# MAPieschl/PointCloudProcessing

Measured on AMD Instinct MI355X. Metric: points/sec PointNet fwd+bwd N=1024 B=32 at 1/2/4/8 MI355X vs CPU ref, higher is better.
Workload: dtype bf16; 1 GPU; PointNet-cls training step (fwd + losses + bwd + grad all-reduce + Adam), N=1024 points, batch 32 per GPU, profile classification_pretrain, 23 classes / 12 parts, random-init weights; global_batch=32, points_per_cloud=1024, parallelism=dp1, launch=hipgraph

## Files before the change

### include/pointnet_hip.h

```cpp
#ifndef POINTNET_HIP_H
#define POINTNET_HIP_H

#include <stddef.h>
#include <stdint.h>

#ifdef __cplusplus
extern "C" {
#endif

#define PN_ABI_VERSION 6

typedef enum {
  PN_OK = 0,
  PN_ERR_INVALID_ARGUMENT = -1,
  PN_ERR_LAUNCH = -2,
  PN_ERR_UNSUPPORTED = -3,
  PN_ERR_WORKSPACE = -4
} pn_status;

#define PN_PREC_BF16 1
#define PN_PREC_BF16X3 3
#define PN_STORE_BF16 0x100
#define PN_IO_KEEP_ACTIVATIONS 1

// ... 183 lines not shown

typedef struct pn_slot_info {
  char name[64];
  int64_t offset;
  int32_t rows, cols, kind, block;
} pn_slot_info;

#define PN_NUM_BLOCKS 15

typedef struct pn_model_io {
  const float* pc;
  int32_t B, N;
  float* params;
  float* grads;
  const uint8_t* trainable;
  int32_t training;
  int32_t zero_grads_in_forward;
  const uint8_t* keep1;
  const uint8_t* keep2;
  const int32_t* labels_cls;
  const int32_t* labels_seg;
  const float* se3;
  float loss_weights[3];
  float pad2_;
  float* out_cls;
  float* out_seg;
  float* out_R;
  float* scalars;
  void* workspace;
  size_t workspace_bytes;
  void** prof_events;
  void* aux_stream;
  int32_t bwd_phase;
  int32_t flags;
  uint64_t dropout_seed;
  uint32_t* dropout_step;
  int32_t sync_rank;
  int32_t pad3_;
  int (*sync_hook)(void* ctx, int op, const void* src, void* dst, int64_t n, int dtype, void* stream);
  void* sync_ctx;
} pn_model_io;

int pn_model_num_slots(const pn_model_desc* d);
int64_t pn_model_param_floats(const pn_model_desc* d);
int pn_model_slot_info(const pn_model_desc* d, int i, pn_slot_info* out);
size_t pn_model_workspace_bytes(const pn_model_desc* d, int B, int N, int training);
int pn_model_ws_lookup(const pn_model_desc* d, int B, int N, int training, const char* name, int64_t* offset, int64_t* bytes);

int pn_model_ws_entry(const pn_model_desc* d, int B, int N, int training, int index, char* name_out, int name_cap,
                      int64_t* offset, int64_t* bytes);

int64_t pn_model_plan_count(int which);
int64_t pn_model_wgrad_fused_count(void);

int pn_model_forward(const pn_model_desc* d, const pn_model_io* io, pn_stream stream);
int pn_model_backward(const pn_model_desc* d, const pn_model_io* io, const float* d_cls, const float* d_seg,
                      const float* d_R, pn_stream stream);

int pn_dropout_masks(uint8_t* keep1, int64_t n1, uint8_t* keep2, int64_t n2, float rate, uint64_t seed, uint32_t* step,
                     pn_stream stream);

int pn_adam_prepare(const int32_t* iterations, float* alpha_scratch, double lr0, double decay_rate, double decay_steps, double beta1,
                    double beta2, pn_stream stream);
int pn_adam_step(float* params, const float* grads, float* m, float* v, int64_t n, int32_t* iterations,
                 float* alpha_scratch, double lr0, double decay_rate, double decay_steps, double beta1, double beta2,
                 double eps, float grad_scale, pn_stream stream);

#ifdef __cplusplus
}
#endif
#endif
```

### pointcloudprocessing_amd/_lib.py

```python
from __future__ import annotations

import ctypes as C
import os
import subprocess

_HERE = os.path.dirname(os.path.abspath(__file__))
LIB_PATH = os.path.join(_HERE, "libpointnet_hip.so")
CSRC = os.path.join(_HERE, "csrc")

PN_PREC_BF16 = 1
PN_PREC_BF16X3 = 3
PN_STORE_BF16 = 0x100
PN_IO_KEEP_ACTIVATIONS = 1
ABI_VERSION = 6
PN_NUM_BLOCKS = 15
PREC = {"bf16": PN_PREC_BF16 | PN_STORE_BF16, "bf16_f32act": PN_PREC_BF16, "bf16x3": PN_PREC_BF16X3}

BLOCK_NAMES = ["input_transform", "mlp_1_1", "mlp_1_2", "feature_transform", "mlp_2_1", "mlp_2_2", "mlp_2_3",
               "mlp_cls_1", "mlp_cls_2", "mlp_cls_3", "mlp_seg_1", "mlp_seg_2", "mlp_seg_3", "mlp_seg_4",
               "mlp_seg_5"]


class PointNetHipError(RuntimeError):
    pass
# ... 70 lines not shown
    "pn_conv_bwd_data_wgrad": (_I, [_OP, _P, _I64, _I, _I, _I, _I, _P, _P, _P, _P, _P, _P, _OP, _I, _I, _P, _I, _P]),
    "pn_slab_reduce": (_I, [_P, _I, _I, _I64, _P, _P]),
    "pn_bn_finalize": (_I, [_P, _I, _I, _I64, _P, _P, _P, _P, _F, _F, _I, _I, _P, _P, _P, _P, _P]),
    "pn_bn_bwd_finalize": (_I, [_P, _I, _I, _I64, _P, _P, _P, _I, _P, _P, _P, _P, _P, _P]),
    "pn_sign": (_I, [_P, _I, _P, _P]),
    "pn_max_finalize": (_I, [_P, _P, _I, _I, _I, _P, _P, _P, _P, _P, _P, _P]),
    "pn_dense_workspace_floats": (C.c_size_t, [_I, _I, _I]),
    "pn_dense_layer": (_I, [_P, _I, _P, _I, _I, _I, _I, _I, _P, _P, _P, _P, _P, _P, _P, _F, _F, _I, _I, _P, _F, _P, _P, _P, _P, _P]),
    "pn_dense_bwd_step": (_I, [_P, _I, _P, _I, _I, _I, _I, _P, _P, _P, _P, _P]),
    "pn_dense_wgrad_batch": (_I, [_P, _I, _P]),
    "pn_dense_bwd": (_I, [_P, _P, _P, _I, _I, _I, _I, _P, _P, _P, _P, _I, _I, _P, _F, _P, _P, _P, _P, _P, _P]),
    "pn_softmax_xent": (_I, [_P, _I, _I, _P, _F, _P, _P, _P, _P, _P]),
    "pn_argmax_rows": (_I, [_P, _I64, _I, _P, _P]),
    "pn_seg_out_part_stride": (_I, []),
    "pn_seg_out_part_rows": (_I, []),
    "pn_seg_out_fwd": (_I, [_OP, _P, _P, _I64, _I, _I, _P, _F, _P, _P, _P, _P]),
    "pn_bmm": (_I, [_P, _P, _I, _I, _I, _P, _I, _P]),
    "pn_dropout_masks": (_I, [_P, _I64, _P, _I64, _F, C.c_uint64, _P, _P]),
    "pn_count_nonfinite": (_I, [_P, _I64, _I, _P, _P]),
    "pn_fps_workspace_bytes": (C.c_size_t, [_I, _I]),
    "pn_fps": (_I, [_P, _I, _I, _I, _I, _P, _P, _P, C.c_size_t, _P]),
    "pn_voxel_workspace_bytes": (C.c_size_t, [_I]),
    "pn_voxel_downsample": (_I, [_P, _P, _I, C.POINTER(C.c_float), C.POINTER(C.c_float), _I, _P, _P, _P, _P, _P,
                                 C.c_size_t, _P]),
    "pn_knn_propagate": (_I, [_P, _P, _I, _I, _I, _I, _P, _I, _P, _P, _P, _P, _P]),
    "pn_icp_workspace_bytes": (C.c_size_t, [_I, _I, _I, _I]),
    "pn_icp_correspond": (_I, [_P, _P, _I, _I, _P, C.POINTER(C.c_int32), _I, _I, _P, _F, _P, _P, _P, _P, C.c_size_t, _P]),
    "pn_icp_solve": (_I, [_P, _I, _P, _P, _P, _P]),
    "pn_semantic_icp": (_I, [_P, _P, _I, _I, _P, C.POINTER(C.c_int32), _I, _I, _P, _I, _F, _D, _D, _P, _P, _P, _P, _P, _P,
                             C.c_size_t, _P]),
    "pn_icp_normals": (_I, [_P, C.POINTER(C.c_int32), _I, _I, _I, _P, _P, _P, _P]),
    "pn_icp_plane_workspace_bytes": (C.c_size_t, [_I, _I, _I, _I]),
    "pn_icp_plane_sums": (_I, [_P, _P, _I, _I, _P, C.POINTER(C.c_int32), _I, _I, _P, _F, _P, _P, _P, _P, _P, _P, C.c_size_t, _P]),
    "pn_icp_plane_solve": (_I, [_P, _I, _P, _P, _P, _P]),
    "pn_semantic_icp_plane": (_I, [_P, _P, _I, _I, _P, C.POINTER(C.c_int32), _I, _I, _P, _I, _F, _D, _D, _P, _P, _P, _P, _P, _P, _P,
                                   C.c_size_t, _P]),
    "pn_icp_mesh_workspace_bytes": (C.c_size_t, [_I, _I, _I, _I]),
    "pn_icp_mesh_correspond": (_I, [_P, _P, _I, _I, _P, C.POINTER(C.c_int32), _I, _I, _P, _F, _I, _P, _P, _P, _P, _P, _P, _P, C.c_size_t,
                                    _P]),
    "pn_semantic_icp_mesh": (_I, [_P, _P, _I, _I, _P, C.POINTER(C.c_int32), _I, _I, _P, _I, _P, _I, _F, _D, _D, _P, _P, _P, _P, _P, _P,
                                  C.c_size_t, _P]),
    "pn_part_moments_workspace_bytes": (C.c_size_t, [_I, _I]),
    "pn_part_moments": (_I, [_P, _P, _I, _I, _I, _P, _P, C.c_size_t, _P]),
    "pn_icp_seed_poses": (_I, [_P, _P, _I, _I, _P, _I, _P, _P]),
    "pn_icp_score_workspace_bytes": (C.c_size_t, [_I, _I, _I]),
    "pn_icp_score_poses": (_I, [_P, _P, _I, _I, _P, C.POINTER(C.c_int32), _I, _I, _P, _I, _I, _F, _P, _P, _P, C.c_size_t, _P]),
    "pn_model_num_slots": (_I, [_DESC]),
    "pn_model_param_floats": (_I64, [_DESC]),
    "pn_model_slot_info": (_I, [_DESC, _I, C.POINTER(pn_slot_info)]),
    "pn_model_workspace_bytes": (C.c_size_t, [_DESC, _I, _I, _I]),
    "pn_model_ws_lookup": (_I, [_DESC, _I, _I, _I, C.c_char_p, C.POINTER(C.c_int64), C.POINTER(C.c_int64)]),
    "pn_model_ws_entry": (_I, [_DESC, _I, _I, _I, _I, C.c_char_p, _I, C.POINTER(C.c_int64), C.POINTER(C.c_int64)]),
    "pn_model_plan_count": (_I64, [_I]),
    "pn_model_wgrad_fused_count": (_I64, []),
    "pn_model_forward": (_I, [_DESC, _IO, _P]),
    "pn_model_backward": (_I, [_DESC, _IO, _P, _P, _P, _P]),
    "pn_adam_prepare": (_I, [_P, _P, _D, _D, _D, _D, _D, _P]),
    "pn_adam_step": (_I, [_P, _P, _P, _P, _I64, _P, _P, _D, _D, _D, _D, _D, _D, _F, _P]),
}

_lib = None


def build(verbose: bool = False) -> str:
    res = subprocess.run(["make", "-C", CSRC, "-j", str(min(8, os.cpu_count() or 1))], capture_output=True, text=True)
    if verbose or res.returncode != 0:
        print(res.stdout[-4000:])
        print(res.stderr[-4000:])
    if res.returncode != 0:
        raise PointNetHipError("building libpointnet_hip.so failed")
    return LIB_PATH


def lib():
    global _lib
    if _lib is None:
        if not os.path.exists(LIB_PATH):
            raise PointNetHipError(
                f"{LIB_PATH} is missing: run `python -c 'import __graft_entry__ as g; g.build()'` "
                f"(or `make -C {CSRC}`).  There is no CPU fallback for the PointNet hot path.")
        import torch
        try:
            l = C.CDLL(LIB_PATH)
        except OSError as e:
            raise PointNetHipError(f"cannot load {LIB_PATH}: {e}") from e
        for name, (res, args) in SIGNATURES.items():
            fn = getattr(l, name)
            fn.restype = res
            fn.argtypes = args
        if l.pn_abi_version() != ABI_VERSION:
            raise PointNetHipError("libpointnet_hip.so ABI version mismatch")
        _lib = l
    return _lib


def check(rc: int, what: str = "") -> None:
    if rc != 0:
        msg = lib().pn_last_error()
        raise PointNetHipError(f"{what} failed ({rc}): {msg.decode() if msg else ''}")


def ptr(t):
    if t is None:
        return None
    return C.c_void_p(t.data_ptr())

# ... 33 lines not shown
```

### pointcloudprocessing_amd/csrc/pn_dense.hip

```cpp
#include "pn_common.h"
#include "pn_dense_wgrad.h"
#include "pn_internal.h"
#include "pn_loss_bodies.h"
#include "pn_maxbwd_bodies.h"

namespace pn {

typedef __attribute__((ext_vector_type(8))) __bf16 bf16x8;
typedef __attribute__((ext_vector_type(16))) float f32x16;

constexpr int DL_COLS = 32;
constexpr int DL_SLICES = 8;
constexpr int DL_KPS = 16;
constexpr int DL_KSTEP = DL_SLICES * DL_KPS;
constexpr int DL_ROWS = 32;
constexpr int DL_MAX_SPLITS = 8;

struct DenseArgs {
  const float* x; int ldx;
  const float* w; int ldw;
  int R, K, C, split_len, nsplit;
  float* partial;
  unsigned* counters;
  const float *bias, *gamma, *beta;
  float *mm, *mv;
  float momentum, eps;
  int bn_mode, act;
  const unsigned char* keep; float keep_scale;
  float *z_out, *a_out, *mean_o, *invstd_o;
  const float *bt_z, *bt_gamma, *bt_beta, *bt_mean, *bt_invstd;
  const unsigned char* bt_keep; float bt_keep_scale;
  int bt_mode, bt_act;
  float *bt_dz, *bt_dgamma, *bt_dbeta, *bt_dbias;
};

static inline int dl_ksplit_env() {
  static const int v = (getenv("PN_DENSE_KSPLIT") && atoi(getenv("PN_DENSE_KSPLIT")) >= 1) ? atoi(getenv("PN_DENSE_KSPLIT")) : 0;
  return v;
}
static inline int dl_nsplit(int K) {
  const int env = dl_ksplit_env();
  const int per_split = env ? env : DL_KSTEP;
  const int s = cdiv(K, per_split);
  return s < 1 ? 1 : (s > DL_MAX_SPLITS ? DL_MAX_SPLITS : s);
}
static inline int dl_split_len(int K) { return cdiv(cdiv(K, dl_nsplit(K)), DL_KSTEP) * DL_KSTEP; }

template <bool TRANS, int DEPTH, bool VEC, bool CARRY = false>
__device__ __forceinline__ bool dense_layer_body(const DenseArgs& a, const unsigned bxi, const int ks, float* zr_out = nullptr) {
  __shared__ __attribute__((aligned(16))) float lds[4 * DL_ROWS * DL_COLS + 16 * 32 + 4];
  float* red = lds;
  float* fin = lds + 4 * DL_ROWS * DL_COLS;
  unsigned* flag = reinterpret_cast<unsigned*>(fin + 16 * 32);
  const int tid = threadIdx.x, c = tid & 31, s = tid >> 5;
  const int j = bxi * DL_COLS + c;
  const int jc = j < a.C ? j : a.C - 1;
  const int kbeg = ks * a.split_len, kend = min(a.K, kbeg + a.split_len);
  const bool single = a.nsplit == 1;
  const bool small = a.R <= DL_ROWS;
  float own[DL_ROWS / DL_SLICES];
  float pf_g = 1.f, pf_b = 0.f, pf_mm = 0.f, pf_mv = 1.f;
  const float pf_bias = a.bias ? a.bias[jc] : 0.f;
  unsigned char pf_kb[DL_ROWS / DL_SLICES] = {1, 1, 1, 1};
  if (a.bn_mode) { pf_g = a.gamma[jc]; pf_b = a.beta[jc]; pf_mm = a.mm[jc]; pf_mv = a.mv[jc]; }
  if (a.keep && a.a_out && a.R <= DL_ROWS) {
#pragma unroll
    for (int i = 0; i < DL_ROWS / DL_SLICES; ++i) pf_kb[i] = a.keep[(long long)min(s + DL_SLICES * i, a.R - 1) * a.C + jc];
  }
  float bt_zz[DL_ROWS / DL_SLICES], bt_mu = 0.f, bt_is = 1.f, bt_g = 1.f, bt_b = 0.f;
  unsigned char bt_kb[DL_ROWS / DL_SLICES] = {1, 1, 1, 1};
  if (TRANS && a.bt_dz) {
#pragma unroll
    for (int i = 0; i < DL_ROWS / DL_SLICES; ++i) bt_zz[i] = a.bt_z[(long long)min(s + DL_SLICES * i, a.R - 1) * a.C + jc];
    if (a.bt_keep) {
#pragma unroll
      for (int i = 0; i < DL_ROWS / DL_SLICES; ++i) bt_kb[i] = a.bt_keep[(long long)min(s + DL_SLICES * i, a.R - 1) * a.C + jc];
    }
    if (a.bt_mode) { bt_mu = a.bt_mean[jc]; bt_is = a.bt_invstd[jc]; bt_g = a.bt_gamma[jc]; bt_b = a.bt_beta[jc]; }
  }

  const int lane = tid & 63, wv = tid >> 6;
  const int lr = lane & 31, lg = lane >> 5;
  const int jw = bxi * DL_COLS + lr;
  const int jwc = jw < a.C ? jw : a.C - 1;
  for (int rc = 0; rc < a.R; rc += DL_ROWS) {
    const int nr = min(DL_ROWS, a.R - rc);
    f32x16 acc;
#pragma unroll
    for (int e = 0; e < 16; ++e) acc[e] = 0.f;
    const int xr = rc + (lr < nr ? lr : nr - 1);
    float xa[DEPTH][8], wb[DEPTH][8];
    auto issue = [&](float (&xv)[8], float (&wv_)[8], int k0) {
      const int kk = k0 + 8 * lg;
      if constexpr (VEC) {
        const int kc = min(kk, kend - 8);
        const float4 t0 = *reinterpret_cast<const float4*>(a.x + (long long)xr * a.ldx + kc);
        const float4 t1 = *reinterpret_cast<const float4*>(a.x + (long long)xr * a.ldx + kc + 4);
        xv[0] = t0.x; xv[1] = t0.y; xv[2] = t0.z; xv[3] = t0.w; xv[4] = t1.x; xv[5] = t1.y; xv[6] = t1.z; xv[7] = t1.w;
        if constexpr (TRANS) {
          const float4 u0 = *reinterpret_cast<const float4*>(a.w + (long long)jwc * a.ldw + kc);
          const float4 u1 = *reinterpret_cast<const float4*>(a.w + (long long)jwc * a.ldw + kc + 4);
          wv_[0] = u0.x; wv_[1] = u0.y; wv_[2] = u0.z; wv_[3] = u0.w; wv_[4] = u1.x; wv_[5] = u1.y; wv_[6] = u1.z; wv_[7] = u1.w;
        } else {
#pragma unroll
          for (int e = 0; e < 8; ++e) wv_[e] = a.w[(long long)(kc + e) * a.ldw + jwc];
        }
      } else {
#pragma unroll
        for (int e = 0; e < 8; ++e) {
          const int k = kk + e;
          const long long kc = k < kend ? k : kend - 1;
          xv[e] = a.x[(long long)xr * a.ldx + kc];
          wv_[e] = TRANS ? a.w[(long long)jwc * a.ldw + kc] : a.w[kc * a.ldw + jwc];
        }
      }
    };
    const int kw = kbeg + 16 * wv;
    const int nsteps = kw < kend ? (kend - kw + 63) / 64 : 0;
    for (int base = 0; base < nsteps; base += DEPTH) {
#pragma unroll
      for (int d = 0; d < DEPTH; ++d)
        if (base + d < nsteps) issue(xa[d], wb[d], kw + 64 * (base + d));
#pragma unroll
      for (int d = 0; d < DEPTH; ++d) {
        const int i = base + d;
        if (i >= nsteps) break;
        const int k0 = kw + 64 * i;
        bf16x8 ah, al, bh, bl;
#pragma unroll
        for (int e = 0; e < 8; ++e) {
          const bool kv = k0 + 8 * lg + e < kend;
          const float xv = (kv && lr < nr) ? xa[d][e] : 0.f;
          const float wvv = (kv && jw < a.C) ? wb[d][e] : 0.f;
          ah[e] = (__bf16)xv;
          al[e] = (__bf16)(xv - (float)ah[e]);
          bh[e] = (__bf16)wvv;
          bl[e] = (__bf16)(wvv - (float)bh[e]);
        }
        acc = __builtin_amdgcn_mfma_f32_32x32x16_bf16(al, bh, acc, 0, 0, 0);
        acc = __builtin_amdgcn_mfma_f32_32x32x16_bf16(ah, bl, acc, 0, 0, 0);
        acc = __builtin_amdgcn_mfma_f32_32x32x16_bf16(ah, bh, acc, 0, 0, 0);
      }
    }
    __syncthreads();
#pragma unroll
    for (int e = 0; e < 16; ++e) red[(wv * DL_ROWS + (e & 3) + 8 * (e >> 2) + 4 * lg) * DL_COLS + lr] = acc[e];
    __syncthreads();
#pragma unroll
    for (int i = 0; i < DL_ROWS / DL_SLICES; ++i) {
      const int r = s + DL_SLICES * i;
      const float t = (red[(0 * DL_ROWS + r) * DL_COLS + c] + red[(1 * DL_ROWS + r) * DL_COLS + c]) +
                      (red[(2 * DL_ROWS + r) * DL_COLS + c] + red[(3 * DL_ROWS + r) * DL_COLS + c]);
      own[i] = t;
      if (!(single && small) && r < nr && j < a.C)
        __hip_atomic_store(&a.partial[((long long)ks * a.R + rc + r) * a.C + j], t, __ATOMIC_RELAXED, __HIP_MEMORY_SCOPE_AGENT);
    }
  }

  if (!single) {
    asm volatile("s_waitcnt vmcnt(0)" ::: "memory");
    __syncthreads();
    if (tid == 0) {
      const unsigned t = __hip_atomic_fetch_add(a.counters + bxi, 1u, __ATOMIC_RELAXED, __HIP_MEMORY_SCOPE_AGENT);
      const unsigned last = (t == (unsigned)a.nsplit - 1u) ? 1u : 0u;
      if (last) __hip_atomic_store(a.counters + bxi, 0u, __ATOMIC_RELAXED, __HIP_MEMORY_SCOPE_AGENT);
      *flag = last;
    }
    __syncthreads();
    if (*flag == 0u) return false;
  } else {
    __syncthreads();
  }

  const int R = a.R, C = a.C, nks = a.nsplit;
  const int tx = c, ty = s;
  constexpr int RP = DL_SLICES;
  const bool jv = j < C;
  const float b = jv ? pf_bias : 0.f;
  float zr[DL_ROWS / RP];
  float s1 = 0.f;
  if (small && single) {
#pragma unroll
    for (int i = 0; i < DL_ROWS / RP; ++i) {
      const int r = ty + RP * i;
      const float z = own[i] + b;
      zr[i] = z;
      if (jv && r < R) {
        a.z_out[(long long)r * C + j] = z;
        s1 += z;
      }
    }
  } else if (small) {
    float pv[DL_ROWS / RP][DL_MAX_SPLITS];
#pragma unroll
    for (int i = 0; i < DL_ROWS / RP; ++i) {
      const int r = min(ty + RP * i, R - 1);
#pragma unroll
      for (int q = 0; q < DL_MAX_SPLITS; ++q)
        pv[i][q] = __hip_atomic_load(&a.partial[((long long)min(q, nks - 1) * R + r) * C + jc], __ATOMIC_RELAXED, __HIP_MEMORY_SCOPE_AGENT);
    }
#pragma unroll
    for (int i = 0; i < DL_ROWS / RP; ++i) {
      float z0 = 0.f, z1 = 0.f;
#pragma unroll
      for (int q = 0; q < DL_MAX_SPLITS; q += 2) {
        z0 += (q < nks) ? pv[i][q] : 0.f;
        z1 += (q + 1 < nks) ? pv[i][q + 1] : 0.f;
      }
      const int r = ty + RP * i;
      const float z = (z0 + z1) + b;
      zr[i] = z;
      if (jv && r < R) {
        a.z_out[(long long)r * C + j] = z;
        s1 += z;
      }
    }
  } else if (jv) {
    for (int r = ty; r < R; r += RP) {
      float z0 = 0.f, z1 = 0.f;
      int q = 0;
      for (; q + 1 < nks; q += 2) {
        z0 += __hip_atomic_load(&a.partial[((long long)q * R + r) * C + j], __ATOMIC_RELAXED, __HIP_MEMORY_SCOPE_AGENT);
        z1 += __hip_atomic_load(&a.partial[((long long)(q + 1) * R + r) * C + j], __ATOMIC_RELAXED, __HIP_MEMORY_SCOPE_AGENT);
      }
      if (q < nks) z0 += __hip_atomic_load(&a.partial[((long long)q * R + r) * C + j], __ATOMIC_RELAXED, __HIP_MEMORY_SCOPE_AGENT);
      const float z = (z0 + z1) + b;
      a.z_out[(long long)r * C + j] = z;
      s1 += z;
    }
  }
  float sc = 1.f, sh = 0.f;
  if (a.bn_mode) {
    float mean = 0.f, var = 1.f;
    if (a.bn_mode == 1) {
      __syncthreads();
      fin[ty * 32 + tx] = s1;
      __syncthreads();
      float t = 0.f;
      for (int q = 0; q < RP; ++q) t += fin[q * 32 + tx];
      mean = t / (float)R;
      float s2 = 0.f;
      if (small) {
#pragma unroll
        for (int i = 0; i < DL_ROWS / RP; ++i) {
          const float d = zr[i] - mean;
          s2 = (jv && ty + RP * i < R) ? fmaf(d, d, s2) : s2;
        }
      } else if (jv) {
        for (int r = ty; r < R; r += RP) {
          const float d = a.z_out[(long long)r * C + j] - mean;
          s2 = fmaf(d, d, s2);
        }
      }
      fin[(8 + ty) * 32 + tx] = s2;
      __syncthreads();
      t = 0.f;
      for (int q = 0; q < RP; ++q) t += fin[(8 + q) * 32 + tx];
      var = t / (float)R;
      if (ty == 0 && jv) {
        a.mm[j] = pf_mm * a.momentum + mean * (1.f - a.momentum);
        a.mv[j] = pf_mv * a.momentum + var * (1.f - a.momentum);
      }
    } else if (jv) {
      mean = pf_mm;
      var = pf_mv;
    }
    const float invstd = 1.0f / sqrtf(var + a.eps);
    if (jv) {
      sc = pf_g * invstd;
      sh = pf_b - mean * sc;
      if (ty == 0) {
        if (a.mean_o) a.mean_o[j] = mean;
        if (a.invstd_o) a.invstd_o[j] = invstd;
      }
    }
  }
  if (TRANS && a.bt_dz) {
    float bsc = 1.f, bsh = 0.f;
    const float mu = bt_mu, is = bt_is;
    if (a.bt_mode) {
      bsc = bt_g * is;
      bsh = bt_b - mu * bsc;
    }
    const float kscale = a.bt_keep ? a.bt_keep_scale : 1.f;
    float v[DL_ROWS / RP], zh[DL_ROWS / RP];
    const float (&zz)[DL_ROWS / DL_SLICES] = bt_zz;
    float S1 = 0.f, S2 = 0.f;
#pragma unroll
    for (int i = 0; i < DL_ROWS / RP; ++i) {
      const int r = ty + RP * i;
      float d = bt_kb[i] ? zr[i] * kscale : 0.f;
      if (a.bt_act == 1 && !(fmaf(bsc, zz[i], bsh) > 0.f)) d = 0.f;
      if (r >= R || !jv) d = 0.f;
      zh[i] = (zz[i] - mu) * is;
      v[i] = d;
      S1 += d;
      S2 = fmaf(d, zh[i], S2);
    }
    __syncthreads();
    fin[ty * 32 + tx] = S1;
    fin[(8 + ty) * 32 + tx] = S2;
    __syncthreads();
    S1 = 0.f; S2 = 0.f;
#pragma unroll
    for (int q = 0; q < RP; ++q) { S1 += fin[q * 32 + tx]; S2 += fin[(8 + q) * 32 + tx]; }
    const float invR = 1.f / (float)R;
    const float m1 = S1 * invR, m2 = S2 * invR;
#pragma unroll
    for (int i = 0; i < DL_ROWS / RP; ++i) {
      const int r = ty + RP * i;
      float d = v[i];
      if (a.bt_mode == 1) d = bsc * (d - m1 - zh[i] * m2);
      else if (a.bt_mode == 2) d *= bsc;
      if (jv && r < R) a.bt_dz[(long long)r * C + j] = d;
    }
    if (ty == 0 && jv) {
      if (a.bt_mode == 1) {
        if (a.bt_dgamma) a.bt_dgamma[j] = S2;
        if (a.bt_dbeta) a.bt_dbeta[j] = S1;
      } else if (a.bt_mode == 0 && a.bt_dbias) {
        a.bt_dbias[j] = S1;
      }
    }
  }
  if (a.a_out && jv) {
    if (small) {
#pragma unroll
      for (int i = 0; i < DL_ROWS / RP; ++i) {
        const int r = ty + RP * i;
        if (r < R) {
          float y = fmaf(sc, zr[i], sh);
          if (a.act == 1) y = clamp_lo(y, 0.f);
          if (a.keep) y = pf_kb[i] ? y * a.keep_scale : 0.f;
          a.a_out[(long long)r * C + j] = y;
        }
      }
    } else {
      for (int r = ty; r < R; r += RP) {
        float y = fmaf(sc, a.z_out[(long long)r * C + j], sh);
        if (a.act == 1) y = clamp_lo(y, 0.f);
        if (a.keep) y = a.keep[(long long)r * C + j] ? y * a.keep_scale : 0.f;
        a.a_out[(long long)r * C + j] = y;
      }
    }
  }
  if constexpr (CARRY) {
#pragma unroll
    for (int i = 0; i < DL_ROWS / RP; ++i) zr_out[i] = zr[i];
  }
  return true;
}

template <bool TRANS, int DEPTH, bool VEC>
__global__ __launch_bounds__(256) void dense_layer_kernel(const DenseArgs a0, const DenseArgs a1) {
  (void)dense_layer_body<TRANS, DEPTH, VEC>(blockIdx.z ? a1 : a0, blockIdx.x, blockIdx.y);
}

template <int NT>
__global__ __launch_bounds__(256) void dense_prep_carry_kernel(const DenseArgs a, int ncb, int n_dense, const PrepArgs pa, const pn_operand x,
                                                               const __bf16* __restrict__ wf_hi, const __bf16* __restrict__ wf_lo,
                                                               const int* __restrict__ argq, int N, int K, int C, int quarters_per_cloud,
                                                               int* __restrict__ arg) {
  const int lin = (int)blockIdx.x;
  if (lin >= n_dense) {
    max_resolve_body<NT>(x, wf_hi, wf_lo, argq, N, K, C, quarters_per_cloud, arg, lin - n_dense);
    return;
  }
  const int ks = lin / ncb, bx = lin - ks * ncb;
  PrepPre pre;
  maxbwd_prep_preload(pa, bx, pre);
  float zr[DL_ROWS / DL_SLICES];
  if (!dense_layer_body<true, 2, true, true>(a, (unsigned)bx, ks, zr)) return;
  maxbwd_prep_body<true>(pa, bx, &pre, zr);
}


struct LossCarryArgs {
  const int* labels; float grad_scale; float *probs, *dlogits, *loss_sum, *correct;
  const float* part; int n, stride, n_sum; float* sum_out;
  const float *Rm, *T; int n_mse; float* mse_out;
  float* scratch;
};
__global__ __launch_bounds__(256) void dense_loss_carry_kernel(const DenseArgs a, const DenseArgs t, const LossCarryArgs lc, int ncb) {
  __shared__ float rl[32], rc[32];
  __shared__ double wsum[16];
  int bx = blockIdx.x;
  if (bx >= ncb) {
    bx -= ncb;
    if (bx < lc.n_sum) { sum_partials_body_as1024(lc.part, lc.n, lc.stride, bx, lc.sum_out, wsum); return; }
    bx -= lc.n_sum;
    if (bx == 0 && lc.mse_out) mse_body(lc.Rm, lc.T, lc.n_mse, 0.f, nullptr, lc.mse_out, rl);
    return;
  }
  float *lg = a.z_out, *pr = lc.probs, *dl = lc.dlogits, *ls = lc.loss_sum, *cr = lc.correct;
  if (bx > 0) {
    const long long rc_ = (long long)a.R * a.C;
    lg = lc.scratch + (long long)(bx - 1) * 3 * rc_; pr = lg + rc_; dl = pr + rc_; ls = nullptr; cr = nullptr;
  }
  DenseArgs a2 = a, t2 = t;
  a2.z_out = lg;
  t2.x = dl;
  (void)dense_layer_body<false, 4, true>(a2, 0u, 0);
  __syncthreads();
  softmax_xent_rows_body<true>(lg, a.R, a.C, lc.labels, lc.grad_scale, pr, dl, ls, cr, rl, rc);
  __syncthreads();
  (void)dense_layer_body<true, 2, false>(t2, (unsigned)bx, 0);
}

constexpr int DB_TPW = 2;
constexpr int DB_KG = 4 * DB_TPW * 32;

__global__ __launch_bounds__(256) void dense_bwd_fused_kernel(const float* __restrict__ da, const float* __restrict__ z,
                                                              const float* __restrict__ x, int ldx, int R, int K, int C,
                                                              const float* __restrict__ gamma, const float* __restrict__ beta,
                                                              const float* __restrict__ mean, const float* __restrict__ invstd,
                                                              int bn_mode, int act, const unsigned char* __restrict__ keep,
                                                              float keep_scale, float* __restrict__ dz, float* __restrict__ dgamma,
                                                              float* __restrict__ dbeta, float* __restrict__ dbias,
                                                              float* __restrict__ dw) {
  const int lane = threadIdx.x & 63, wave = threadIdx.x >> 6;
  const int lr = lane & 31, lg = lane >> 5;
  const int j = blockIdx.x * 32 + lr;
  const bool jv = j < C;
  const int jc = jv ? j : C - 1;
  float sc = 1.f, sh = 0.f, mu = 0.f, is = 1.f;
  if (bn_mode) {
    mu = mean[jc]; is = invstd[jc];
    sc = gamma[jc] * is;
    sh = beta[jc] - mu * sc;
  }
  float d[16], zh[16];
  unsigned kmask = 0xffffu;
#pragma unroll
  for (int q = 0; q < 16; ++q) {
    const int r = (q >> 3) * 16 + 8 * lg + (q & 7);
    const long long o = (long long)min(r, R - 1) * C + jc;
    d[q] = da[o];
    zh[q] = z[o];
  }
  if (keep) {
    kmask = 0u;
#pragma unroll
    for (int q = 0; q < 16; ++q) {
      const int r = (q >> 3) * 16 + 8 * lg + (q & 7);
      kmask |= (keep[(long long)min(r, R - 1) * C + jc] ? 1u : 0u) << q;
    }
  }
  const int kbase = blockIdx.y * DB_KG + wave * (DB_TPW * 32);
  float xa[16];
  auto issue_x = [&](int k0) {
    const int kk = min(k0 + lr, K - 1);
#pragma unroll
    for (int q = 0; q < 16; ++q) {
      const int r = (q >> 3) * 16 + 8 * lg + (q & 7);
      xa[q] = x[(long long)min(r, R - 1) * ldx + kk];
    }
  };
  if (dw && kbase < K) issue_x(kbase);
  const float kscale = keep ? keep_scale : 1.f;
// ... 220 lines not shown
__global__ __launch_bounds__(1024) void softmax_xent_rows_kernel(const float* __restrict__ logits, int R, int C,
                                                                const int* __restrict__ labels, float grad_scale,
                                                                float* __restrict__ probs, float* __restrict__ dlogits,
                                                                float* __restrict__ loss_sum, float* __restrict__ correct) {
  __shared__ float rl[32], rc[32];
  softmax_xent_rows_body(logits, R, C, labels, grad_scale, probs, dlogits, loss_sum, correct, rl, rc);
}

__global__ __launch_bounds__(256) void softmax_bwd_rows_kernel(const float* __restrict__ probs, const float* __restrict__ dprobs,
                                                               long long R, int C, float* __restrict__ dlogits) {
  const long long r = (long long)blockIdx.x * 256 + threadIdx.x;
  if (r >= R) return;
  const float* p = probs + r * C;
  const float* dp = dprobs + r * C;
  float dot = 0.f;
  for (int c = 0; c < C; ++c) dot = fmaf(p[c], dp[c], dot);
  float* d = dlogits + r * C;
  for (int c = 0; c < C; ++c) d[c] = p[c] * (dp[c] - dot);
}

__global__ __launch_bounds__(256) void argmax_rows_kernel(const float* __restrict__ v, long long R, int C, int* __restrict__ out) {
  const long long r = (long long)blockIdx.x * 256 + threadIdx.x;
  if (r >= R) return;
  const float* p = v + r * C;
  float best = p[0];
  int bi = 0;
  for (int c = 1; c < C; ++c) {
    const float x = p[c];
    if (x > best) { best = x; bi = c; }
  }
  out[r] = bi;
}

size_t dense_partial_floats(int R, int K, int C) { return (size_t)dl_nsplit(K) * R * C; }

static int dense_args(DenseArgs& a, const float* x, int ldx, const float* w, int ldw, int R, int K, int C, float* partial, unsigned* counters,
                      const float* bias, const float* gamma, const float* beta, float* mm, float* mv, float momentum, float eps, int bn_mode,
                      int act, const unsigned char* keep, float keep_scale, float* z_out, float* a_out, float* mean_o, float* invstd_o) {
  PN_CHECK_ARG(x && w && partial && counters && z_out && R > 0 && K > 0 && C > 0, "dense_layer: bad arguments");
  PN_CHECK_ARG(cdiv(C, DL_COLS) <= DENSE_MAX_COUNTERS, "dense_layer: C=%d needs more than %d counters", C, DENSE_MAX_COUNTERS);
  PN_CHECK_ARG(!bn_mode || (gamma && beta && mm && mv), "dense_layer: BatchNormalization needs gamma/beta/moving statistics");
  a.x = x; a.ldx = ldx; a.w = w; a.ldw = ldw; a.R = R; a.K = K; a.C = C;
  a.nsplit = dl_nsplit(K); a.split_len = dl_split_len(K);
  if (cdiv(C, DL_COLS) == 1 && K <= 512) { a.nsplit = 1; a.split_len = cdiv(K, DL_KSTEP) * DL_KSTEP; }
  a.partial = partial; a.counters = counters;
  a.bias = bias; a.gamma = gamma; a.beta = beta; a.mm = mm; a.mv = mv; a.momentum = momentum; a.eps = eps;
  a.bn_mode = bn_mode; a.act = act; a.keep = keep; a.keep_scale = keep_scale;
  a.z_out = z_out; a.a_out = a_out; a.mean_o = mean_o; a.invstd_o = invstd_o;
  a.bt_z = a.bt_gamma = a.bt_beta = a.bt_mean = a.bt_invstd = nullptr;
  a.bt_keep = nullptr; a.bt_keep_scale = 1.f; a.bt_mode = 0; a.bt_act = 0;
  a.bt_dz = a.bt_dgamma = a.bt_dbeta = a.bt_dbias = nullptr;
  return PN_OK;
}
template <bool TRANS>
static void launch_dense(const DenseArgs& a, const DenseArgs& b, dim3 grid, hipStream_t st) {
  const int steps = cdiv(a.split_len, 64);
  const int depth = steps <= 2 ? 2 : (steps <= 4 ? 4 : 8);
  auto aligned = [](const DenseArgs& q) {
    return q.K % 16 == 0 && q.ldx % 4 == 0 && (reinterpret_cast<uintptr_t>(q.x) & 15) == 0 &&
           (!TRANS || (q.ldw % 4 == 0 && (reinterpret_cast<uintptr_t>(q.w) & 15) == 0));
  };
  const bool vec = aligned(a) && aligned(b);
#define PN_DENSE_CASE(D, V) hipLaunchKernelGGL((dense_layer_kernel<TRANS, D, V>), grid, dim3(256), 0, st, a, b)
  if (vec) { if (depth == 2) PN_DENSE_CASE(2, true); else if (depth == 4) PN_DENSE_CASE(4, true); else PN_DENSE_CASE(8, true); }
  else PN_DENSE_CASE(2, false);
#undef PN_DENSE_CASE
}

int dense_layer(const float* x, int ldx, const float* w, int ldw, bool trans, int R, int K, int C, float* partial, unsigned* counters,
                const float* bias, const float* gamma, const float* beta, float* mm, float* mv, float momentum, float eps, int bn_mode,
                int act, const unsigned char* keep, float keep_scale, float* z_out, float* a_out, float* mean_o, float* invstd_o,
                hipStream_t st) {
  DenseArgs a;
  PN_TRY(dense_args(a, x, ldx, w, ldw, R, K, C, partial, counters, bias, gamma, beta, mm, mv, momentum, eps, bn_mode, act, keep, keep_scale,
                    z_out, a_out, mean_o, invstd_o));
  const dim3 grid(cdiv(C, DL_COLS), a.nsplit);
  if (trans) launch_dense<true>(a, a, grid, st);
  else launch_dense<false>(a, a, grid, st);
  PN_CHECK_LAUNCH();
  return PN_OK;
}
int dense_layer_with_plain(const float* x, int ldx, const float* w, int ldw, int R, int K, int C, float* partial, unsigned* counters,
                           const float* bias, const float* gamma, const float* beta, float* mm, float* mv, float momentum, float eps,
                           int bn_mode, int act, const unsigned char* keep, float keep_scale, float* z_out, float* a_out, float* mean_o,
                           float* invstd_o, const float* w2, int ldw2, float* out2, hipStream_t st) {
  PN_CHECK_ARG(2 * cdiv(C, DL_COLS) <= DENSE_MAX_COUNTERS, "dense_layer_with_plain: C=%d needs more than %d counters", C, DENSE_MAX_COUNTERS);
  DenseArgs a, b;
  PN_TRY(dense_args(a, x, ldx, w, ldw, R, K, C, partial, counters, bias, gamma, beta, mm, mv, momentum, eps, bn_mode, act, keep, keep_scale,
                    z_out, a_out, mean_o, invstd_o));
  PN_TRY(dense_args(b, x, ldx, w2, ldw2, R, K, C, partial + dense_partial_floats(R, K, C), counters + cdiv(C, DL_COLS), nullptr, nullptr, nullptr,
                    nullptr, nullptr, 0.f, 0.f, 0, 0, nullptr, 1.f, out2, nullptr, nullptr, nullptr));
  launch_dense<false>(a, b, dim3(cdiv(C, DL_COLS), a.nsplit, 2), st);
  PN_CHECK_LAUNCH();
  return PN_OK;
}

int dense_trans_tail(const float* dz, int lddz, const float* w, int ldw, int R, int K, int C, float* partial, unsigned* counters, float* dx,
                     const DenseTail* tail, hipStream_t st) {
  DenseArgs a;
  PN_TRY(dense_args(a, dz, lddz, w, ldw, R, K, C, partial, counters, nullptr, nullptr, nullptr, nullptr, nullptr, 0.f, 0.f, 0, 0, nullptr, 1.f,
                    dx, nullptr, nullptr, nullptr));
  if (tail) {
    PN_CHECK_ARG(R <= DL_ROWS, "dense_trans_tail: the backward tail needs R <= %d (R=%d)", DL_ROWS, R);
    PN_CHECK_ARG(tail->z && tail->dz, "dense_trans_tail: null pointer in the tail");
    PN_CHECK_ARG(!tail->mode || (tail->gamma && tail->beta && tail->mean && tail->invstd), "dense_trans_tail: BatchNormalization needs gamma/beta/mean/invstd");
    a.bt_z = tail->z; a.bt_gamma = tail->gamma; a.bt_beta = tail->beta; a.bt_mean = tail->mean; a.bt_invstd = tail->invstd;
    a.bt_keep = tail->keep; a.bt_keep_scale = tail->keep_scale; a.bt_mode = tail->mode; a.bt_act = tail->act;
    a.bt_dz = tail->dz; a.bt_dgamma = tail->dgamma; a.bt_dbeta = tail->dbeta; a.bt_dbias = tail->dbias;
  }
  launch_dense<true>(a, a, dim3(cdiv(C, DL_COLS), a.nsplit), st);
  PN_CHECK_LAUNCH();
  return PN_OK;
}

int dense_trans_prep_carry(const float* dz, int lddz, const float* w, int ldw, int R, int K, int C, float* partial, unsigned* counters, float* dx,
                           const PrepCarry* pc, hipStream_t st, bool* carried) {
  *carried = false;
  DenseArgs a;
  PN_TRY(dense_args(a, dz, lddz, w, ldw, R, K, C, partial, counters, nullptr, nullptr, nullptr, nullptr, nullptr, 0.f, 0.f, 0, 0, nullptr, 1.f,
                    dx, nullptr, nullptr, nullptr));
  const int prec = pc ? (pc->prec & ~PN_STORE_BF16) : 0;
  const bool vec = K % 16 == 0 && lddz % 4 == 0 && ldw % 4 == 0 && (reinterpret_cast<uintptr_t>(dz) & 15) == 0 && (reinterpret_cast<uintptr_t>(w) & 15) == 0;
  const bool fits = pc && R <= DL_ROWS && cdiv(a.split_len, 64) <= 2 && vec && C % 32 == 0 && pc->W && pc->Wt && pc->We && pc->K <= RS_KMAX &&
                    pc->K % 16 == 0 && (!pc->pm_slabs || pc->K == 128) && pc->x.s1 && !pc->x.s2 && (reinterpret_cast<uintptr_t>(pc->x.s1) & 15) == 0 &&
                    pc->x.ld % (pc->x.h16 ? 8 : 4) == 0 && (prec == PN_PREC_BF16 || (prec == PN_PREC_BF16X3 && pc->wf_lo)) && pc->N > 0;
  if (!fits) {
    launch_dense<true>(a, a, dim3(cdiv(C, DL_COLS), a.nsplit), st);
    PN_CHECK_LAUNCH();
    return PN_OK;
  }
  PN_CHECK_ARG(pc->g && pc->zstar && pc->mean && pc->invstd && pc->scale && pc->hs && pc->e && pc->nege && pc->f && pc->wf_hi && pc->argq && pc->arg,
               "dense_trans_prep_carry: null pointer");
  const PrepArgs pa = make_prep(dx, pc->dg2, pc->g, pc->zstar, R, C, pc->mean, pc->invstd, pc->scale, pc->batch_stats, pc->count, pc->hs, pc->e, pc->nege,
                                pc->f, pc->dgamma, pc->dbeta, pc->W, pc->K, pc->Wt, pc->We, pc->pm_slabs);
  const int ncb = cdiv(C, DL_COLS), n_dense = ncb * a.nsplit, qpc = cdiv(pc->N, 32);
  const __bf16* wh = reinterpret_cast<const __bf16*>(pc->wf_hi);
  const __bf16* wl = reinterpret_cast<const __bf16*>(pc->wf_lo);
  if (prec == PN_PREC_BF16X3)
    hipLaunchKernelGGL((dense_prep_carry_kernel<2>), dim3(n_dense + R * qpc), dim3(256), 0, st, a, ncb, n_dense, pa, pc->x, wh, wl, pc->argq, pc->N, pc->K, C, qpc, pc->arg);
  else
    hipLaunchKernelGGL((dense_prep_carry_kernel<1>), dim3(n_dense + R * qpc), dim3(256), 0, st, a, ncb, n_dense, pa, pc->x, wh, wl, pc->argq, pc->N, pc->K, C, qpc, pc->arg);
  PN_CHECK_LAUNCH();
  *carried = true;
  return PN_OK;
}

bool dense_loss_carry_fits(const float* x, int ldx, int R, int K, int C, int C2) {
  if (R < 1 || R > DL_ROWS || C < 1 || C2 < 1 || cdiv(C, DL_COLS) != 1 || K > 512 || K % 16 != 0 || ldx % 4 != 0 || (reinterpret_cast<uintptr_t>(x) & 15) != 0) return false;
  const int steps_a = cdiv(cdiv(K, DL_KSTEP) * DL_KSTEP, 64);
  if (steps_a <= 2 || steps_a > 4) return false;
  if (C % 16 == 0 || dl_nsplit(C) != 1 || cdiv(dl_split_len(C), 64) > 2) return false;
  return cdiv(C2, DL_COLS) <= DENSE_MAX_COUNTERS;
}
int dense_loss_carry(const float* x, int ldx, const float* w, int ldw, int R, int K, int C, const float* bias, float* logits, float* partial,
                     unsigned* counters, const LossCarry* lc, int C2, float* dx, const DenseTail* tail, hipStream_t st) {
  PN_CHECK_ARG(dense_loss_carry_fits(x, ldx, R, K, C, C2), "dense_loss_carry: shapes do not fit the carried launch (R=%d K=%d C=%d C2=%d)", R, K, C, C2);
  PN_CHECK_ARG(lc && lc->labels && lc->probs && lc->dlogits && dx && tail && tail->z && tail->dz, "dense_loss_carry: null pointer");
  PN_CHECK_ARG(!tail->mode || (tail->gamma && tail->beta && tail->mean && tail->invstd), "dense_loss_carry: BatchNormalization needs gamma/beta/mean/invstd");
  PN_CHECK_ARG(lc->n_sum == 0 || (lc->part && lc->sum_out && lc->n > 0), "dense_loss_carry: bad partial-sum arguments");
  PN_CHECK_ARG(!lc->mse_out || (lc->Rm && lc->T && lc->n_mse > 0), "dense_loss_carry: bad rotation-loss arguments");
  DenseArgs a, t;
  PN_TRY(dense_args(a, x, ldx, w, ldw, R, K, C, partial, counters, bias, nullptr, nullptr, nullptr, nullptr, 0.f, 0.f, 0, 0, nullptr, 1.f, logits,
                    nullptr, nullptr, nullptr));
  PN_TRY(dense_args(t, lc->dlogits, C, w, ldw, R, C, C2, partial, counters, nullptr, nullptr, nullptr, nullptr, nullptr, 0.f, 0.f, 0, 0, nullptr, 1.f,
                    dx, nullptr, nullptr, nullptr));
  PN_CHECK_ARG(a.nsplit == 1 && t.nsplit == 1, "dense_loss_carry: both products must be single splits");
  t.bt_z = tail->z; t.bt_gamma = tail->gamma; t.bt_beta = tail->beta; t.bt_mean = tail->mean; t.bt_invstd = tail->invstd;
  t.bt_keep = tail->keep; t.bt_keep_scale = tail->keep_scale; t.bt_mode = tail->mode; t.bt_act = tail->act;
  t.bt_dz = tail->dz; t.bt_dgamma = tail->dgamma; t.bt_dbeta = tail->dbeta; t.bt_dbias = tail->dbias;
  const int ncb = cdiv(C2, DL_COLS);
  PN_CHECK_ARG(dense_partial_floats(R, 1024, C2) >= (size_t)(ncb - 1) * 3 * R * C, "dense_loss_carry: the partial-tile buffer is too small for the copies");
  const LossCarryArgs la{lc->labels, lc->grad_scale, lc->probs, lc->dlogits, lc->loss_sum, lc->correct, lc->part, lc->n, lc->stride, lc->n_sum,
                         lc->sum_out, lc->Rm, lc->T, lc->n_mse, lc->mse_out, partial};
  hipLaunchKernelGGL(dense_loss_carry_kernel, dim3(ncb + lc->n_sum + (lc->mse_out ? 1 : 0)), dim3(256), 0, st, a, t, la, ncb);
  PN_CHECK_LAUNCH();
  return PN_OK;
}

__global__ __launch_bounds__(256) void dense_wgrad_batch_kernel(const DenseWgradBatch b) {
  __shared__ float xs[16][32];
  dense_wgrad_batch_body(b, (int)blockIdx.x, xs);
}
int dense_wgrad_batch(const DenseWgradJob* jobs, int n, hipStream_t st) {
  DenseWgradBatch b;
  int blocks = 0;
  PN_TRY(make_dense_wgrad_batch(jobs, n, b, blocks));
  hipLaunchKernelGGL(dense_wgrad_batch_kernel, dim3(blocks), dim3(256), 0, st, b);
  PN_CHECK_LAUNCH();
  return PN_OK;
}

// ... 68 lines not shown
```

### pointcloudprocessing_amd/csrc/pn_internal.h

```cpp
#pragma once
#include "pn_common.h"

namespace pn {

int conv_fwd(const pn_operand* x, const float* w, long long wcs, int B, int N, int K, int C, const float* cloud_bias, float* z,
             float* stat_partials, int prec, hipStream_t st, const void* w16 = nullptr);
int conv_fwd_max(const pn_operand* x, const float* w, int B, int N, int K, int C, const float* sgn, float* pmax, int* pidx,
                 float* stat_partials, int prec, hipStream_t st);
struct WgradFuse {
  pn_operand a;
  int Ci, slab_rows;
  float* slabs;
};
int conv_bwd_data(const pn_operand* dz, const float* w, long long wcs, int B, int N, int K, int C, const float* addend,
                  const float* zmask, const float* msc, const float* msh, float* out, float* stat_partials, int prec,
                  hipStream_t st, const void* w16 = nullptr, const float* col_bias = nullptr,
                  const WgradFuse* wf = nullptr);
int conv_bwd_data_reduce(const pn_operand* dz, const float* w, long long wcs, int B, int N, int K, int C, float* out, int prec, hipStream_t st,
                         const float* slabs, int n_slabs, int per_group, long long elems, float* red_out, bool* rode);
struct WgradDesc {
  pn_operand a, b;
  int B, N, Ci, Cj, slab_rows;
  float* slabs;
  int prec, colsum;
// ... 47 lines not shown
  long long elems;
  int n_slabs;
};
int slab_reduce_batch(const SlabJob* jobs, int n_jobs, hipStream_t st);
int slab_reduce_q(const float* slabs, int n_slabs, long long elems, float* out, const float* w, const float* f, int K, int C, float* q,
                  hipStream_t st);
int bn_finalize(const float* part, int n_tiles, int C, long long count, const float* gamma, const float* beta, float* mm,
                float* mv, float momentum, float eps, int use_batch, int update, float* mean, float* invstd, float* scale,
                float* shift, hipStream_t st);
int bn_bwd_finalize(const float* part, int n_tiles, int C, long long count, const float* gamma, const float* mean,
                    const float* invstd, int batch_stats, float* dgamma, float* dbeta, float* ca, float* cb, float* cc,
                    hipStream_t st);
int sign_of(const float* gamma, int C, float* sgn, hipStream_t st);
int max_finalize(const float* pmax, const int* pidx, int B, int tpc, int C, int n_rows, const float* sgn, const float* scale,
                 const float* shift, float* g, float* zstar, int* arg, hipStream_t st);

constexpr int DENSE_MAX_COUNTERS = 256;
size_t dense_partial_floats(int R, int K, int C);
int dense_layer(const float* x, int ldx, const float* w, int ldw, bool trans, int R, int K, int C, float* partial, unsigned* counters,
                const float* bias, const float* gamma, const float* beta, float* mm, float* mv, float momentum, float eps, int bn_mode,
                int act, const unsigned char* keep, float keep_scale, float* z_out, float* a_out, float* mean_o, float* invstd_o,
                hipStream_t st);
int dense_layer_with_plain(const float* x, int ldx, const float* w, int ldw, int R, int K, int C, float* partial, unsigned* counters,
                           const float* bias, const float* gamma, const float* beta, float* mm, float* mv, float momentum, float eps,
                           int bn_mode, int act, const unsigned char* keep, float keep_scale, float* z_out, float* a_out, float* mean_o,
                           float* invstd_o, const float* w2, int ldw2, float* out2, hipStream_t st);
int dense_bwd_fused(const float* da, const float* z, const float* x, int ldx, int R, int K, int C, const float* gamma, const float* beta,
                    const float* mean, const float* invstd, int bn_mode, int act, const unsigned char* keep, float keep_scale, float* dz,
                    float* dgamma, float* dbeta, float* dbias, float* dw, hipStream_t st);
int dense_bwd_pre(const float* da, const float* z, int R, int C, const float* gamma, const float* beta, const float* mean,
                  const float* invstd, int bn_mode, int act, const unsigned char* keep, float keep_scale, float* dz, float* dgamma,
                  float* dbeta, float* dbias, hipStream_t st);
int dense_wgrad(const float* x, int ldx, const float* dz, int R, int K, int C, float* dw, hipStream_t st, float* db = nullptr);
struct DenseTail {
  const float *z, *gamma, *beta, *mean, *invstd;
  const unsigned char* keep; float keep_scale;
  int mode, act;
  float *dz, *dgamma, *dbeta, *dbias;
};
static_assert(sizeof(DenseTail) == sizeof(pn_dense_tail), "DenseTail mirrors pn_dense_tail");
int dense_trans_tail(const float* dz, int lddz, const float* w, int ldw, int R, int K, int C, float* partial, unsigned* counters, float* dx,
                     const DenseTail* tail, hipStream_t st);
struct PrepCarry {
  const float *dg2, *g, *zstar, *mean, *invstd, *scale;
  int batch_stats; long long count;
  float *hs, *e, *nege, *f, *dgamma, *dbeta;
  const float* W; int K;
  float *Wt, *We;
  pn_operand x;
  const void *wf_hi, *wf_lo;
  int prec;
  const int* argq; int N; int* arg;
  float* pm_slabs;
};
int dense_trans_prep_carry(const float* dz, int lddz, const float* w, int ldw, int R, int K, int C, float* partial, unsigned* counters, float* dx,
                           const PrepCarry* pc, hipStream_t st, bool* carried);
struct LossCarry {
  const int* labels; float grad_scale; float *probs, *dlogits, *loss_sum, *correct;
  const float* part; int n, stride, n_sum; float* sum_out;
  const float *Rm, *T; int n_mse; float* mse_out;
};
bool dense_loss_carry_fits(const float* x, int ldx, int R, int K, int C, int C2);
int dense_loss_carry(const float* x, int ldx, const float* w, int ldw, int R, int K, int C, const float* bias, float* logits, float* partial,
                     unsigned* counters, const LossCarry* lc, int C2, float* dx, const DenseTail* tail, hipStream_t st);
constexpr int DENSE_WGRAD_MAX_JOBS = 12;
struct DenseWgradJob { const float* x; int ldx; const float* dz; int R, K, C; float* dw; float* db; };
static_assert(sizeof(DenseWgradJob) == sizeof(pn_dense_wgrad_job), "DenseWgradJob mirrors pn_dense_wgrad_job");
int dense_wgrad_batch(const DenseWgradJob* jobs, int n, hipStream_t st);
int transpose(const float* in, int R, int C, float* out, hipStream_t st);
int transpose2(const float* in, int R, int C, const float* rowscale, float* out, float* out2, hipStream_t st);
int softmax_xent_rows(const float* logits, int R, int C, const int* labels, float grad_scale, float* probs, float* dlogits,
                      float* loss_sum, float* correct, hipStream_t st);
int softmax_bwd_rows(const float* probs, const float* dprobs, long long R, int C, float* dlogits, hipStream_t st);
int argmax_rows(const float* values, long long R, int C, int* index, hipStream_t st);

int bmm3(const float* x, const float* R, int B, int N, float* out, hipStream_t st);

int seg_out_fwd(const pn_operand* x, const float* w, const float* bias, long long M, int K, int C, const int* labels,
                float grad_scale, float* probs, float* dlogits, float* part, hipStream_t st);
int seg_head_fused_rows();
int seg_head_fused(const pn_operand* x, const float* gb, const void* w1t, const void* w2t, const void* w3t, const void* w4t, const float* sc1,
                   const float* sh1, const float* sc2, const float* sh2, const float* sc3, const float* sh3, const float* sc4, const float* sh4,
                   const float* w5, const float* b5, int B, int N, int C, int s16, const int* labels, float grad_scale, float* probs,
                   float* dlogits, float* part, hipStream_t st);
int seg_out_part_stride();
int seg_out_part_rows();
int seg_out_bwd(const pn_operand* x, const float* w, const float* dlogits, int B, int N, int K, int C, float* dyhat, float* stat_part,
                float* wslab, hipStream_t st, int store16 = 0);
int sum_partials(const float* part, int n, int stride, int elems, float* out, hipStream_t st);
int loss_tail(const float* logits, int R, int C, const int* labels, float grad_scale, float* probs, float* dlogits, float* loss_sum,
              float* correct, const float* part, int n, int stride, int n_sum, float* sum_out, const float* Rm, const float* T, int n_mse,
              float* mse_out, hipStream_t st);

int maxbwd_prep(const float* dg, const float* dg2, const float* g, const float* zstar, int B, int C, const float* mean, const float* invstd,
                const float* scale, int batch_stats, long long count, float* hs, float* e, float* nege, float* f, float* dgamma,
                float* dbeta, const float* W, int K, float* Wt, float* We, hipStream_t st, float* pm_slabs = nullptr);
int colsum_lazy(const pn_operand* x, int B, int N, int C, float* part, hipStream_t st);
struct DwJob {
  pn_operand x;
  const int* arg;
  const float* hs;
  const float* a1;
  const float* f;
  const float* e;
  const float* GW;
  float* dW;
};
int maxbwd_dw_batch(const DwJob* jobs, int n_jobs, int B, int N, int K, int C, hipStream_t st);
int maxbwd_dw(const pn_operand* x, const int* arg, const float* hs, int B, int N, int K, int C, const float* a1, const float* f,
              const float* e, const float* GW, float* dW, hipStream_t st);
int maxbwd_q(const float* w, const float* f, int K, int C, float* q, hipStream_t st);
int maxbwd_scatter(const int* arg, const float* hs, const float* wt, const float* q, int B, int N, int K, int C, float* D,
                   int store16, hipStream_t st);
int maxbwd_scatter_reduce(const int* arg, const float* hs, const float* wt, int B, int N, int K, int C, float* D, int store16,
                          const float* slabs, int n_slabs, long long elems, float* pm, const float* w, const float* f, float* q, hipStream_t st);
int maxbwd_prep_resolve(const float* dg, const float* dg2, const float* g, const float* zstar, int B, int C, const float* mean,
                        const float* invstd, const float* scale, int batch_stats, long long count, float* hs, float* e, float* nege,
                        float* f, float* dgamma, float* dbeta, const float* W, int K, float* Wt, float* We, const pn_operand* x,
                        const void* wf_hi, const void* wf_lo, int prec, const int* argq, int N, int* arg, hipStream_t st, float* pm_slabs = nullptr);
int max_resolve(const pn_operand* x, const void* wf_hi, const void* wf_lo, int prec, const int* argq, int B, int N, int K, int C, int* arg,
                hipStream_t st);

size_t fps_workspace_bytes(int B, int N);
int fps(const float* xyz, int B, int N, int M, int start_idx, int* idx_out, float* mindist, void* ws, size_t ws_bytes,
        hipStream_t st);
size_t voxel_workspace_bytes(int N);
int voxel_downsample(const float* xyz, const int* labels, int N, const float* leaf, const float* origin, int n_labels,
                     float* centroids, int* counts, int* majority, int* n_out, void* ws, size_t ws_bytes, hipStream_t st);
int knn_propagate(const float* query, const float* ref, int B, int Nq, int M, int k, const float* values, int C, int* idx_out,
                  float* d2_out, float* values_out, int* arg_out, hipStream_t st);
size_t icp_workspace_bytes(int B, int N, int M, int n_parts);
int icp_correspond(const float* scan, const int* labels, int B, int N, const float* ref, const int* ref_seg, int M, int n_parts,
                   const float* pose32, float max_d2, int* idx_out, float* d2_out, double* sums_out, void* ws, size_t ws_bytes,
                   hipStream_t st);
int icp_solve(const double* sums, int B, double* pose, double* rmse, int* status, hipStream_t st);
int semantic_icp(const float* scan, const int* labels, int B, int N, const float* ref, const int* ref_seg, int M, int n_parts,
                 const double* init_pose, int max_iters, float max_d2, double tol_rot, double tol_t, double* pose_out,
// ... 59 lines not shown
```

### pointcloudprocessing_amd/csrc/pn_model.hip

```cpp
#include <algorithm>
#include <atomic>
#include <cstdlib>
#include <functional>
#include <cstring>
#include <string>
#include <vector>
#include "pn_internal.h"

namespace pn {

static std::atomic<long long> g_plan_count[3];
static std::atomic<long long> g_wgrad_fused_count;

enum { BLK_IT = 0, BLK_M11, BLK_M12, BLK_FT, BLK_M21, BLK_M22, BLK_M23, BLK_C1, BLK_C2, BLK_C3, BLK_S1, BLK_S2, BLK_S3, BLK_S4,
       BLK_S5, N_BLOCKS };

struct Slot {
  std::string name;
  long long off;
  int rows, cols, kind, block;
};
struct LRef {
  long long kernel = -1, gamma = -1, beta = -1, mm = -1, mv = -1, bias = -1;
  int cin = 0, cout = 0, block = 0;
  bool has_bn = false;
};
struct TRef {
  LRef c1, c2, c3, d1, d2;
  long long w = -1, b = -1;
  int K = 0;
};
struct Layout {
  std::vector<Slot> slots;
  TRef iT, fT;
  LRef m11, m12, m21, m22, m23, c1, c2, c3, s1, s2, s3, s4, s5;
  long long total = 0;
};

static long long add_slot(Layout& L, const std::string& name, int rows, int cols, int kind, int block) {
  Slot s;
  s.name = name; s.rows = rows; s.cols = cols; s.kind = kind; s.block = block;
  s.off = L.total;
  L.total += ((long long)rows * cols + 63) / 64 * 64;
  L.slots.push_back(s);
  return s.off;
}
static LRef add_layer(Layout& L, const std::string& prefix, int cin, int cout, bool has_bn, int block) {
  LRef r;
  r.cin = cin; r.cout = cout; r.block = block; r.has_bn = has_bn;
  r.kernel = add_slot(L, prefix + ".kernel", cin, cout, 0, block);
  if (has_bn) {
    r.gamma = add_slot(L, prefix + ".bn.gamma", 1, cout, 1, block);
    r.beta = add_slot(L, prefix + ".bn.beta", 1, cout, 2, block);
    r.mm = add_slot(L, prefix + ".bn.moving_mean", 1, cout, 3, block);
    r.mv = add_slot(L, prefix + ".bn.moving_var", 1, cout, 4, block);
  } else {
    r.bias = add_slot(L, prefix + ".bias", 1, cout, 5, block);
  }
  return r;
}
static TRef add_tnet(Layout& L, const std::string& name, int K, int block) {
  TRef t;
  t.K = K;
  t.c1 = add_layer(L, name + ".conv1", K, 64, true, block);
// ... 7 lines not shown
}

static Layout make_layout(const pn_model_desc& d) {
  Layout L;
  if (!d.vanilla) L.iT = add_tnet(L, "input_transform", 3, BLK_IT);
  L.m11 = add_layer(L, "mlp_1_1", 3, 64, true, BLK_M11);
  L.m12 = add_layer(L, "mlp_1_2", 64, 64, true, BLK_M12);
  if (!d.vanilla) L.fT = add_tnet(L, "feature_transform", 64, BLK_FT);
  L.m21 = add_layer(L, "mlp_2_1", 64, 64, true, BLK_M21);
  L.m22 = add_layer(L, "mlp_2_2", 64, 128, true, BLK_M22);
  L.m23 = add_layer(L, "mlp_2_3", 128, 1024, true, BLK_M23);
  L.c1 = add_layer(L, "mlp_cls_1", 1024, 512, true, BLK_C1);
  L.c2 = add_layer(L, "mlp_cls_2", 512, 256, true, BLK_C2);
  L.c3 = add_layer(L, "mlp_cls_3", 256, d.ccls, false, BLK_C3);
  L.s1 = add_layer(L, "mlp_seg_1", 1088, 512, true, BLK_S1);
  L.s2 = add_layer(L, "mlp_seg_2", 512, 256, true, BLK_S2);
  L.s3 = add_layer(L, "mlp_seg_3", 256, 128, true, BLK_S3);
  L.s4 = add_layer(L, "mlp_seg_4", 128, 128, true, BLK_S4);
  L.s5 = add_layer(L, "mlp_seg_5", 128, d.cseg, false, BLK_S5);
  return L;
}

struct Arena {
  char* base = nullptr;
  size_t off = 0;
  size_t guard = ws_guard_bytes();
  std::vector<std::pair<std::string, std::pair<size_t, size_t>>>* dir = nullptr;
  static size_t ws_guard_bytes() {
    const char* e = getenv("PN_WS_GUARD");
    return e ? ((size_t)atoll(e) + 255) & ~(size_t)255 : 0;
  }
  template <class T>
  T* get(const char* name, size_t count) {
    const size_t bytes = ((count * sizeof(T) + 255) & ~(size_t)255) + guard;
    const size_t o = off;
    off += bytes;
    if (dir) dir->push_back({name, {o, count * sizeof(T)}});
    return base ? reinterpret_cast<T*>(base + o) : nullptr;
  }
};

struct CL {
  float *Z = nullptr, *part = nullptr, *mean = nullptr, *invstd = nullptr, *scale = nullptr, *shift = nullptr;
  float *ca = nullptr, *cb = nullptr, *cc = nullptr, *dy = nullptr;
  unsigned short *w16 = nullptr, *wt16 = nullptr;
  int C = 0, K = 0;
};
struct ML {
  long long* pa1;
  float *g_all = nullptr, *zstar_all = nullptr;
  float *pmax, *sumsq, *g, *zstar, *hs, *e, *nege, *f, *a1part, *a1, *gram, *GW, *Pm, *q, *D, *Wt, *We, *dG;
  float* gram_slabs = nullptr;
  int gram_rows = 0, gram_spc = 0;
  int *pq, *argq, *arg;
  unsigned short *wb_hi, *wb_lo;
  int T64, tpc64, rows;
};
struct DLs {
  float *z, *a, *mean, *invstd, *dz, *din;
  int K, C;
};
struct TN {
  CL c1, c2, c3;
  ML m3;
  DLs d1, d2;
  float *R, *dR, *da2;
};

struct WS {
  float *pcn, *cent, *scl;
  TN iT, fT;
  CL m11, m12, m21, m22, m23, s1, s2, s3, s4;
  ML mm23;
  DLs c1, c2, c3;
  float *Weff1, *dWeff1, *X64, *dX64, *tmpA12, *gb, *dgb, *dGseg, *dGcls;
  float *cls_logits, *cls_dlogits, *seg_dlogits, *seg_part, *dense_part, *slabs, *slabs_main, *bpart, *s5slab, *R3eye, *regpart;
  float* sync_part = nullptr;
  float* pm_slabs = nullptr;
  size_t slab_floats, slab_main_floats;
  float* slab_pool;
  size_t slab_pool_floats;
  unsigned* dcount;
};

static long long wgrad_slab_rows(int B, int N, int Ci, int Cj, int* spc_out, int target_override = 0) {
  const int bm = (Ci % 128 == 0 && Cj % 128 == 0) ? 128 : 64, bn = (Cj % 128 == 0) ? 128 : 64;
  const int n_out = (Ci / bm) * (Cj / bn);
  static const int target_blocks = getenv("PN_WGRAD_TARGET") ? atoi(getenv("PN_WGRAD_TARGET")) : 256;
  int target = (target_override > 0 ? target_override : target_blocks) / n_out;
  if (target < 1) target = 1;
  int spc = cdiv(target, B);
  const int max_spc = cdiv(N, 64);
  if (spc > max_spc) spc = max_spc;
  if (spc < 1) spc = 1;
  int rows = cdiv(cdiv(N, spc), 64) * 64;
  spc = cdiv(N, rows);
  *spc_out = spc;
  return rows;
}
static size_t wgrad_slab_floats(int B, int N, int Ci, int Cj) {
  int spc;
  wgrad_slab_rows(B, N, Ci, Cj, &spc);
  return (size_t)B * spc * Ci * Cj;
}

static float* plan_act(Arena& A, const std::string& name, size_t elems, bool s16) {
// ... 356 lines not shown
  }
  bool gram_rides(const ML& m, const LRef& r) const {
    static const bool on = getenv("PN_GRAM_RIDE") && atoi(getenv("PN_GRAM_RIDE")) == 1;
    return on && training && tr(r.block) && G && W == 1 && !aux && m.gram_slabs && r.cin == 128 && s16 && (prec & ~PN_STORE_BF16) == PN_PREC_BF16;
  }
  int fwd_max(CL& l, ML& m, const LRef& r, const pn_operand& x, int prof_slot) {
    const int ub = bn_batch(r.block) ? 1 : 0;
    void** ev = io.prof_events;
    if (ev && ev[2 * prof_slot]) (void)hipEventRecord(reinterpret_cast<hipEvent_t>(ev[2 * prof_slot]), st);
    PN_TRY(conv_fwd_max_panel(&x, m.wb_hi, m.wb_lo, B, N, r.cin, r.cout, m.pmax, m.pq, ub ? m.sumsq : nullptr, ub ? m.pa1 : nullptr, prec, st));
    if (ev && ev[2 * prof_slot + 1]) (void)hipEventRecord(reinterpret_cast<hipEvent_t>(ev[2 * prof_slot + 1]), st);
    if (W > 1 && ub) {
      PN_TRY(sync_sum(m.sumsq, m.sumsq, (long long)m.T64 * r.cout));
      PN_TRY(sync_sum(m.pa1, m.pa1, (long long)B * r.cin * ((prec & ~PN_STORE_BF16) == PN_PREC_BF16X3 ? 2 : 1), 1));
    }
    WgradDesc gram{x, x, B, N, r.cin, r.cin, m.gram_rows, m.gram_slabs, prec, 1, 0};
    PN_TRY(panel_finalize(m.pmax, m.pq, m.sumsq, m.pa1, m.wb_hi, m.wb_lo, prec, B, N, r.cin, r.cout, p(r.gamma), p(r.beta), p(r.mm), p(r.mv), d.bn_momentum, d.bn_eps, ub,
                          ub, l.mean, l.invstd, l.scale, l.shift, W > 1 ? loc(m.g_all, r.cout) : m.g, W > 1 ? loc(m.zstar_all, r.cout) : m.zstar, m.argq, st, W,
                          gram_rides(m, r) ? &gram : nullptr));
    if (W > 1) {
      PN_TRY(sync_gather_rows(m.g_all, (long long)B * r.cout));
      PN_TRY(sync_gather_rows(m.zstar_all, (long long)B * r.cout));
    }
    return PN_OK;
  }
  const float* pooled(const ML& m) const { return W > 1 ? m.g_all : m.g; }
  const float* pooled_local(const ML& m, int C) const { return W > 1 ? loc(m.g_all, C) : m.g; }
  const float* zstar_local(const ML& m, int C) const { return W > 1 ? loc(m.zstar_all, C) : m.zstar; }
  bool fused_chain(const CL& c2) const {
    static const bool on = !(getenv("PN_CHAIN_FUSE") && atoi(getenv("PN_CHAIN_FUSE")) == 0);
    return on && !training && s16 && (prec & ~PN_STORE_BF16) == PN_PREC_BF16 && !(io.flags & PN_IO_KEEP_ACTIVATIONS) && c2.wt16 != nullptr;
  }
  int fwd_chain(const pn_operand* x, const float* w1f, CL& c1, CL& c2, CL& c3, ML& m, const LRef& r3) {
    PN_TRY(chain_fwd_max(x, x ? nullptr : w.pcn, w1f, x ? c1.wt16 : nullptr, c1.scale, c1.shift, c2.wt16, c2.scale, c2.shift, m.wb_hi, B, N,
                         m.pmax, m.pq, st));
    return panel_finalize(m.pmax, m.pq, nullptr, nullptr, m.wb_hi, m.wb_lo, prec, B, N, r3.cin, r3.cout, p(r3.gamma), p(r3.beta), p(r3.mm), p(r3.mv),
                          d.bn_momentum, d.bn_eps, 0, 0, c3.mean, c3.invstd, c3.scale, c3.shift, m.g, m.zstar, m.argq, st);
  }
  int dense_plain(const float* x, int ldx, const float* Wk, int ldw, bool trans, int K, int C, const float* bias, float* out, int rows = -1) {
    return dense_layer(x, ldx, Wk, ldw, trans, rows < 0 ? Bd : rows, K, C, w.dense_part, w.dcount, bias, nullptr, nullptr, nullptr, nullptr, 0.f, 0.f, 0, 0,
                       nullptr, 1.f, out, nullptr, nullptr, nullptr, st);
  }
  int fwd_dense(DLs& dl, const LRef& r, const float* x, int act, const unsigned char* keep) {
    const int mode = r.has_bn ? (bn_batch(r.block) ? 1 : 2) : 0;
    const float ks = 1.f / (1.f - d.dropout_rate);
    return dense_layer(x, r.cin, p(r.kernel), r.cout, false, Bd, r.cin, r.cout, w.dense_part, w.dcount, p(r.bias), p(r.gamma), p(r.beta),
                       p(r.mm), p(r.mv), d.bn_momentum, d.bn_eps, mode, act, keep, ks, dl.z, dl.a, dl.mean, dl.invstd, st);
  }
  bool loss_carries() const {
    static const bool on = getenv("PN_LOSS_CARRY") && atoi(getenv("PN_LOSS_CARRY")) == 1;
    return on && training && G && io.zero_grads_in_forward && io.labels_cls && io.loss_weights[0] != 0.f && W == 1 && chain_ok() &&
           dense_loss_carry_fits(w.c2.a, L.c3.cin, Bd, L.c3.cin, d.ccls, L.c2.cout);
  }
  struct ChainLayer { DLs* dl; const LRef* r; const float* xin; int act; const unsigned char* keep; };
  DenseTail chain_tail(const ChainLayer& cl) const {
    const DLs& dl = *cl.dl;
    const LRef& r = *cl.r;
    const int mode = r.has_bn ? (bn_batch(r.block) ? 1 : 2) : 0;
    const bool wg = tr(r.block) && G;
    DenseTail t;
    memset(&t, 0, sizeof(t));
    t.z = dl.z; t.gamma = p(r.gamma); t.beta = p(r.beta); t.mean = dl.mean; t.invstd = dl.invstd;
    t.keep = cl.keep; t.keep_scale = 1.f / (1.f - d.dropout_rate); t.mode = mode; t.act = cl.act;
    t.dz = dl.dz;
    t.dgamma = (wg && mode == 1) ? gr(r.gamma) : nullptr;
    t.dbeta = (wg && mode == 1) ? gr(r.beta) : nullptr;
    t.dbias = (wg && mode == 0) ? gr(r.bias) : nullptr;
    return t;
  }
  int fwd_tnet(TN& t, const TRef& r, const pn_operand* x) {
    if (fused_chain(t.c2) && (r.K == 3 || t.c1.wt16)) {
      PN_TRY(fwd_chain(r.K == 3 ? nullptr : x, r.K == 3 ? p(r.c1.kernel) : nullptr, t.c1, t.c2, t.c3, t.m3, r.c3));
      PN_TRY(fwd_dense(t.d1, r.d1, pooled(t.m3), 1, nullptr));
      PN_TRY(fwd_dense(t.d2, r.d2, t.d1.a, 1, nullptr));
      return dense_plain(t.d2.a, 256, p(r.w), r.K * r.K, false, 256, r.K * r.K, p(r.b), t.R);
    }
    if (r.K == 3) {
      PN_TRY(conv3_fwd(w.pcn, p(r.c1.kernel), 0, B, N, 64, t.c1.Z, bn_batch(r.c1.block) ? t.c1.part : nullptr, st, s16));
      PN_TRY(bn_fin(t.c1, r.c1));
    } else {
      PN_TRY(fwd_conv(t.c1, r.c1, *x, p(r.c1.kernel), 0, nullptr));
    }
    PN_TRY(fwd_conv(t.c2, r.c2, lazy(t.c1), p(r.c2.kernel), 0, nullptr));
    PN_TRY(fwd_max(t.c3, t.m3, r.c3, lazy(t.c2), r.K == 3 ? 0 : 1));
    PN_TRY(fwd_dense(t.d1, r.d1, pooled(t.m3), 1, nullptr));
    PN_TRY(fwd_dense(t.d2, r.d2, t.d1.a, 1, nullptr));
    return dense_plain(t.d2.a, 256, p(r.w), r.K * r.K, false, 256, r.K * r.K, p(r.b), t.R);
  }

  pn_operand x64op() const { return d.vanilla ? lazy(w.m12) : plain_act(w.X64, 64); }

  int forward() {
    {
      const bool x3 = prec == PN_PREC_BF16X3;
      const float* ws[3] = {d.vanilla ? nullptr : p(L.iT.c3.kernel), d.vanilla ? nullptr : p(L.fT.c3.kernel), p(L.m23.kernel)};
      const int Ks[3] = {128, 128, 128}, Cs[3] = {1024, 1024, 1024};
      void* his[3] = {d.vanilla ? nullptr : w.iT.m3.wb_hi, d.vanilla ? nullptr : w.fT.m3.wb_hi, w.mm23.wb_hi};
      void* los[3] = {(x3 && !d.vanilla) ? w.iT.m3.wb_lo : nullptr, (x3 && !d.vanilla) ? w.fT.m3.wb_lo : nullptr, x3 ? w.mm23.wb_lo : nullptr};
      const float* sgs[3] = {d.vanilla ? nullptr : p(L.iT.c3.gamma), d.vanilla ? nullptr : p(L.fT.c3.gamma), p(L.m23.gamma)};
      WCopyDesc wc[PN_WCOPY_MAX];
      int nwc = 0;
      bool dropped = false;
      auto add_wc = [&](const CL& l, const float* Wk, int frag = 0) {
        if (!l.w16) return;
        if (nwc < PN_WCOPY_MAX) wc[nwc++] = WCopyDesc{Wk, l.w16, l.wt16, l.K, l.C, frag};
        else dropped = true;
// ... 21 lines not shown
      if (dropped) {
        set_error("pn_model_forward: more per-point layers than fwd_prologue's tables hold (PN_WCOPY_MAX %d, PN_FROZEN_MAX %d)", PN_WCOPY_MAX,
                  PN_FROZEN_MAX);
        return PN_ERR_INVALID_ARGUMENT;
      }
      const bool zg = training && G && io.zero_grads_in_forward;
      const bool dm = training && io.dropout_step && io.keep1 && io.keep2 && d.dropout_rate > 0.f;
      PN_TRY(fwd_prologue(io.pc, B, N, w.pcn, w.cent, w.scl, ws, sgs, Ks, Cs, his, los, w.dcount, DENSE_MAX_COUNTERS + 3 * B * 512, zg ? G : nullptr,
                          zg ? L.total : 0, dm ? const_cast<unsigned char*>(io.keep1) : nullptr, dm ? (long long)Bd * 512 : 0,
                          dm ? const_cast<unsigned char*>(io.keep2) : nullptr, dm ? (long long)Bd * 256 : 0, d.dropout_rate, io.dropout_seed,
                          dm ? io.dropout_step : nullptr, wc, nwc, fz, nfz, d.bn_eps, st));
    }
    if (!d.vanilla) {
      PN_TRY(fwd_tnet(w.iT, L.iT, nullptr));
      PN_TRY(conv3_fwd(w.pcn, p(L.m11.kernel), 0, B, N, 64, w.m11.Z, bn_batch(BLK_M11) ? w.m11.part : nullptr, st, s16, loc(w.iT.R, 9), w.Weff1,
                       io.out_R));
    } else {
      PN_TRY(conv3_fwd(w.pcn, p(L.m11.kernel), 0, B, N, 64, w.m11.Z, bn_batch(BLK_M11) ? w.m11.part : nullptr, st, s16));
    }
    PN_TRY(bn_fin(w.m11, L.m11));
    PN_TRY(fwd_conv(w.m12, L.m12, lazy(w.m11), p(L.m12.kernel), 0, nullptr));
    if (!d.vanilla) {
      const pn_operand a12 = lazy(w.m12);
      PN_TRY(fwd_tnet(w.fT, L.fT, &a12));
      PN_TRY(conv_fwd(&a12, loc(w.fT.R, 4096), 4096, B, N, 64, 64, nullptr, w.X64, nullptr, prec, st));
    }
    const pn_operand x64 = x64op();
    if (fused_chain(w.m22) && w.m21.wt16) {
      PN_TRY(fwd_chain(&x64, nullptr, w.m21, w.m22, w.m23, w.mm23, L.m23));
    } else {
      PN_TRY(fwd_conv(w.m21, L.m21, x64, p(L.m21.kernel), 0, nullptr));
      PN_TRY(fwd_conv(w.m22, L.m22, lazy(w.m21), p(L.m22.kernel), 0, nullptr));
      PN_TRY(fwd_max(w.m23, w.mm23, L.m23, lazy(w.m22), 2));
    }
    const float* Gf = pooled(w.mm23);

    {
      const LRef& r = L.c1;
      const int mode = r.has_bn ? (bn_batch(r.block) ? 1 : 2) : 0;
      PN_TRY(dense_layer_with_plain(Gf, r.cin, p(r.kernel), r.cout, Bd, r.cin, r.cout, w.dense_part, w.dcount, p(r.bias), p(r.gamma), p(r.beta),
                                    p(r.mm), p(r.mv), d.bn_momentum, d.bn_eps, mode, 1, training ? io.keep1 : nullptr,
                                    1.f / (1.f - d.dropout_rate), w.c1.z, w.c1.a, w.c1.mean, w.c1.invstd, p(L.s1.kernel) + 64 * 512, 512, w.gb,
                                    st));
    }
    const bool lcar = loss_carries();
    const bool fused = io.labels_cls != nullptr;
    const bool fseg = io.labels_seg != nullptr;
    int seg_parts = (int)cdivll(M, seg_out_part_rows());
    auto cls_rest = [&]() -> int {
      PN_TRY(fwd_dense(w.c2, L.c2, w.c1.a, 1, training ? io.keep2 : nullptr));
      if (!lcar) PN_TRY(dense_plain(w.c2.a, 256, p(L.c3.kernel), d.ccls, false, 256, d.ccls, p(L.c3.bias), w.cls_logits));
      return PN_OK;
    };
    if (!lcar) PN_TRY(cls_rest());

    if (fused_seg_head()) {
      seg_parts = B * cdiv(N, seg_head_fused_rows());
      PN_TRY(seg_head_fused(&x64, loc(w.gb, 512), w.s1.wt16, w.s2.wt16, w.s3.wt16, w.s4.wt16, w.s1.scale, w.s1.shift, w.s2.scale, w.s2.shift, w.s3.scale,
                            w.s3.shift, w.s4.scale, w.s4.shift, p(L.s5.kernel), p(L.s5.bias), B, N, d.cseg, s16, io.labels_seg,
                            fseg ? io.loss_weights[1] / (float)M : 0.f, io.out_seg, nullptr, fseg ? w.seg_part : nullptr, st));
    } else {
    const float* Ws1 = p(L.s1.kernel);
    PN_TRY(conv_fwd(&x64, Ws1, 0, B, N, 64, 512, loc(w.gb, 512), w.s1.Z, w.s1.part, prec, st, w.s1.wt16));
    PN_TRY(bn_fin(w.s1, L.s1));
    PN_TRY(fwd_conv(w.s2, L.s2, lazy(w.s1), p(L.s2.kernel), 0, nullptr));
    PN_TRY(fwd_conv(w.s3, L.s3, lazy(w.s2), p(L.s3.kernel), 0, nullptr));
    PN_TRY(fwd_conv(w.s4, L.s4, lazy(w.s3), p(L.s4.kernel), 0, nullptr));
    const pn_operand a4 = lazy(w.s4);
    PN_TRY(seg_out_fwd(&a4, p(L.s5.kernel), p(L.s5.bias), M, 128, d.cseg, io.labels_seg, fseg ? io.loss_weights[1] / (float)M : 0.f,
                       io.out_seg, (fseg && training) ? w.seg_dlogits : nullptr, fseg ? w.seg_part : nullptr, st));
    }
    if (io.out_R) {
      if (d.vanilla) {
        PN_TRY(fill_eye3(io.out_R, B, st));
      }
    }
    if (lcar) PN_TRY(cls_rest());
    {
      const float* Rp = (io.se3 && io.scalars) ? (d.vanilla ? io.out_R : loc(w.iT.R, 9)) : nullptr;
      const bool sums = fseg && io.scalars;
      if (lcar) {
        const LossCarry lc{io.labels_cls, io.loss_weights[0] / (float)B, io.out_cls, w.cls_dlogits, io.scalars ? io.scalars + 0 : nullptr,
                           io.scalars ? io.scalars + 1 : nullptr, sums ? w.seg_part : nullptr, sums ? seg_parts : 0, seg_out_part_stride(),
                           sums ? 2 : 0, sums ? io.scalars + 2 : nullptr, Rp, io.se3, B * 9, Rp ? io.scalars + 4 : nullptr};
        const ChainLayer below{&w.c2, &L.c2, w.c1.a, 1, io.keep2};
        const DenseTail t = chain_tail(below);
        PN_TRY(dense_loss_carry(w.c2.a, 256, p(L.c3.kernel), d.ccls, Bd, 256, d.ccls, p(L.c3.bias), w.cls_logits, w.dense_part, w.dcount, &lc,
                                L.c2.cout, w.c3.din, &t, st));
        ++g_plan_count[1];
      } else
      PN_TRY(loss_tail(loc(w.cls_logits, d.ccls), B, d.ccls, io.labels_cls, fused ? io.loss_weights[0] / (float)B : 0.f, io.out_cls,
                       (fused && training) ? loc(w.cls_dlogits, d.ccls) : nullptr, io.scalars ? io.scalars + 0 : nullptr,
                       io.scalars ? io.scalars + 1 : nullptr, sums ? w.seg_part : nullptr, sums ? seg_parts : 0,
                       seg_out_part_stride(), sums ? 2 : 0, sums ? io.scalars + 2 : nullptr, Rp, io.se3, B * 9, Rp ? io.scalars + 4 : nullptr,
                       st));
    }
    if (io.scalars && !d.vanilla) {
      if (d.reg_in) {
        PN_TRY(orth_reg(loc(w.iT.R, 9), B, 3, 1e-3f, nullptr, w.regpart, st));
        PN_TRY(sum_partials(w.regpart, B, 1, 1, io.scalars + 5, st));
      }
      if (d.reg_feat) {
        PN_TRY(orth_reg(loc(w.fT.R, 4096), B, 64, 1e-3f, nullptr, w.regpart + B, st));
        PN_TRY(sum_partials(w.regpart + B, B, 1, 1, io.scalars + 6, st));
      }
    }
    return PN_OK;
  }

  int wgrad_to(const pn_operand& a, const pn_operand& b, int Ci, int Cj, float* out, bool per_cloud, bool deferrable = false) {
    return wgrad_general(a, b, B, N, Ci, Cj, out, per_cloud, prec, false, deferrable);
  }
  int wgrad3_to(const pn_operand& dz, float* out) {
    float* sl = pool_take((size_t)T * 3 * 64);
    if (sl) {
      PN_TRY(conv3_wgrad(w.pcn, &dz, B, N, 64, sl, st));
      jobs.push_back(SlabJob{sl, out, 3 * 64, T});
      return PN_OK;
    }
    PN_TRY(conv3_wgrad(w.pcn, &dz, B, N, 64, cur_slabs(), st));
    return slab_reduce(cur_slabs(), T, T, 3 * 64, out, st);
  }
  int wgrad_general(const pn_operand& a, const pn_operand& b, int Bq, int Nq, int Ci, int Cj, float* out, bool per_cloud, int pr,
                    bool colsum = false, bool deferrable = false) {
    static const int t_gram = getenv("PN_WGRAD_TARGET_GRAM") ? atoi(getenv("PN_WGRAD_TARGET_GRAM")) : 128;
    const int t_over = (deferrable && colsum) ? t_gram : 0;
    int spc;
    const int rows = (int)wgrad_slab_rows(Bq, Nq, Ci, Cj, &spc, t_over);
    const size_t elems = (size_t)Ci * Cj + (colsum ? Ci : 0);
    last_deferred = false;
    if (deferrable && !per_cloud) {
      if (float* ps = pool_take((size_t)Bq * spc * elems)) {
        static const bool batch_gemm = !(getenv("PN_WGRAD_BATCH") && atoi(getenv("PN_WGRAD_BATCH")) == 0);
        if (batch_gemm) wg_jobs.push_back(WgradDesc{a, b, Bq, Nq, Ci, Cj, rows, ps, pr, colsum ? 1 : 0, 0});
        else PN_TRY(conv_wgrad(&a, &b, Bq, Nq, Ci, Cj, rows, ps, pr, st, colsum ? 1 : 0));
        jobs.push_back(SlabJob{ps, out, (long long)elems, Bq * spc});
        last_deferred = true;
        return PN_OK;
      }
    }
    float* sl = cur_slabs();
    if ((size_t)Bq * spc * elems > (sl == w.slabs ? w.slab_floats : w.slab_main_floats)) {
      set_error("wgrad: slab scratch too small");
      return PN_ERR_WORKSPACE;
    }
    PN_TRY(conv_wgrad(&a, &b, Bq, Nq, Ci, Cj, rows, sl, pr, st, colsum ? 1 : 0));
    return slab_reduce(sl, Bq * spc, per_cloud ? spc : Bq * spc, (long long)elems, out, st);
  }
  bool wgrad_fuse_take(const pn_operand& a, int cin, int cout, float* out, WgradFuse& wf) {
    static const int mode = getenv("PN_WGRAD_FUSE") ? atoi(getenv("PN_WGRAD_FUSE")) : 1;
    if (mode == 0 || aux || W != 1 || !out || prec != (PN_PREC_BF16 | PN_STORE_BF16) || cin != 64 || (cout != 64 && cout != 128)) return false;
    if (!a.h16 || a.s2) return false;
    int spc;
    const int rows = (int)wgrad_slab_rows(B, N, cin, cout, &spc);
    if (rows != 64 && rows != 128) return false;
    const size_t elems = (size_t)cin * cout;
    float* ps = pool_take((size_t)B * spc * elems);
    if (!ps) return false;
    jobs.push_back(SlabJob{ps, out, (long long)elems, B * spc});
    wf = WgradFuse{a, cin, rows, ps};
    ++g_wgrad_fused_count;
    return true;
  }
  int bn_bwd_fin(const CL& l, const LRef& r, const float* part) {
    const int bs = bn_batch(r.block) ? 1 : 0;
    if (W > 1 && bs) {
      PN_TRY(sync_sum(part, w.sync_part, (long long)T * 2 * r.cout));
      part = w.sync_part;
    }
    return bn_bwd_finalize(part, T, r.cout, M * W, p(r.gamma), l.mean, l.invstd, bs, bs ? gr(r.gamma) : nullptr, bs ? gr(r.beta) : nullptr,
                           l.ca, l.cb, l.cc, st);
  }
  int bwd_step(CL& cur, const LRef& rc, CL& prev, const pn_operand& prev_act) {
    PN_TRY(bn_bwd_fin(cur, rc, w.bpart));
    const pn_operand dz = dzop(cur);
    WgradFuse wf;
    bool fz = false;
    if (tr(rc.block) && G) {
      float* out = gr(rc.kernel);
      const int ci = rc.cin, cj = rc.cout;
      fz = wgrad_fuse_take(prev_act, ci, cj, out, wf);
      if (!fz) {
        PN_TRY(side([=] { return wgrad_to(prev_act, dz, ci, cj, out, false, true); }));
        PN_TRY(flush());
      }
    }
    return conv_bwd_data(&dz, p(rc.kernel), 0, B, N, rc.cout, rc.cin, nullptr, prev.Z, prev.scale, prev.shift, prev.dy, w.bpart, prec, st,
                         cur.w16, nullptr, fz ? &wf : nullptr);
  }
  float* pm_slabs_of(int K, int C) const {
    static const bool pm_in_prep = !(getenv("PN_PM_IN_PREP") && atoi(getenv("PN_PM_IN_PREP")) == 0);
    return (pm_in_prep && K == 128 && C % 32 == 0 && C / 32 <= 32) ? w.pm_slabs : nullptr;
  }
  bool prep_carries(const LRef& r) const {
    static const bool on = !(getenv("PN_PREP_CARRY") && atoi(getenv("PN_PREP_CARRY")) == 0);
    return on && training && W == 1 && chain_ok() && r.cin == 128 && pm_slabs_of(r.cin, r.cout) != nullptr;
  }
  PrepCarry prep_carry(const CL& l, const ML& m, const LRef& r, const pn_operand& xop, const float* dG2) const {
    const bool wg = tr(r.block) && G;
    PrepCarry c;
    memset(&c, 0, sizeof(c));
    c.dg2 = dG2; c.g = m.g; c.zstar = m.zstar; c.mean = l.mean; c.invstd = l.invstd; c.scale = l.scale;
    c.batch_stats = bn_batch(r.block) ? 1 : 0; c.count = M;
    c.hs = m.hs; c.e = m.e; c.nege = m.nege; c.f = m.f; c.dgamma = wg ? gr(r.gamma) : nullptr; c.dbeta = wg ? gr(r.beta) : nullptr;
    c.W = p(r.kernel); c.K = r.cin; c.Wt = m.Wt; c.We = m.We;
    c.x = xop; c.wf_hi = m.wb_hi; c.wf_lo = m.wb_lo; c.prec = prec; c.argq = m.argq; c.N = N; c.arg = m.arg;
    c.pm_slabs = pm_slabs_of(r.cin, r.cout);
    return c;
  }
  int bwd_max(CL& l, ML& m, const LRef& r, const pn_operand& xop, CL& prev, const float* dG, const float* dG2 = nullptr, bool carried = false) {
    const int K = r.cin, C = r.cout;
    const int bs = bn_batch(r.block) ? 1 : 0;
    const bool wg = tr(r.block) && G;
    float* pms = pm_slabs_of(K, C);
    if (carried) {
      ++g_plan_count[0];
    } else if (W > 1) {
      PN_TRY(maxbwd_prep(dG, dG2, m.g_all, m.zstar_all, Bd, C, l.mean, l.invstd, l.scale, bs, M * W, m.hs, m.e, m.nege, m.f, wg ? gr(r.gamma) : nullptr,
                         wg ? gr(r.beta) : nullptr, p(r.kernel), K, m.Wt, m.We, st, pms));
      PN_TRY(max_resolve(&xop, m.wb_hi, m.wb_lo, prec, m.argq, B, N, K, C, m.arg, st));
    } else {
    PN_TRY(maxbwd_prep_resolve(dG, dG2, m.g, m.zstar, B, C, l.mean, l.invstd, l.scale, bs, M, m.hs, m.e, m.nege, m.f, wg ? gr(r.gamma) : nullptr,
                               wg ? gr(r.beta) : nullptr, p(r.kernel), K, m.Wt, m.We, &xop, m.wb_hi, m.wb_lo, prec, m.argq, N, m.arg, st, pms));
    }
    const float* hs_loc = W > 1 ? loc(m.hs, C) : m.hs;
    if (wg) {
      ML mm = m;
      mm.hs = const_cast<float*>(hs_loc);
      float* dw = gr(r.kernel);
      const float* Wk = p(r.kernel);
      PN_TRY(side([=] {
        if (gram_rides(mm, r)) {
          jobs.push_back(SlabJob{mm.gram_slabs, mm.gram, (long long)K * K + K, B * mm.gram_spc});
          last_deferred = true;
        } else
        PN_TRY(wgrad_general(xop, xop, B, N, K, K, mm.gram, false, prec, true, true));
        const WgradDesc gwd{plain(mm.gram, K), plain(Wk, C), 1, K, K, C, K, mm.GW, PN_PREC_BF16X3, 0, 1};
        auto gw_alone = [=] { return conv_wgrad_batch(&gwd, 1, st); };
        auto rest = [=] {
          PN_TRY(gw_alone());
          return maxbwd_dw(&xop, mm.arg, mm.hs, B, N, K, C, mm.a1, mm.f, mm.e, mm.GW, dw, st);
        };
        if (!last_deferred) return rest();
        if (!dw_jobs.empty() && (dw_K != K || dw_C != C)) {
          after_jobs.push_back(rest);
          return (int)PN_OK;
        }
        static const bool gw_batch = !(getenv("PN_GW_BATCH") && atoi(getenv("PN_GW_BATCH")) == 0);
        if (gw_batch) gw_jobs.push_back(gwd);
        else after_jobs.push_back(gw_alone);
        dw_K = K; dw_C = C;
        dw_jobs.push_back(DwJob{xop, mm.arg, mm.hs, mm.a1, mm.f, mm.e, mm.GW, dw});
        return (int)PN_OK;
      }));
      PN_TRY(flush());
    }
    if (pms) {
      PN_TRY(maxbwd_scatter_reduce(m.arg, hs_loc, m.Wt, B, N, K, C, m.D, s16, pms, C / 32, (long long)K * K, m.Pm, p(r.kernel), m.f, m.q, st));
      return conv_bwd_data(&xop, m.Pm, 0, B, N, K, K, m.D, prev.Z, prev.scale, prev.shift, prev.dy, w.bpart, prec, st, nullptr, m.q);
    } else {
      int spc;
      const int rows = (int)wgrad_slab_rows(1, C, K, K, &spc);
      float* sl = cur_slabs();
      if ((size_t)spc * K * K > (sl == w.slabs ? w.slab_floats : w.slab_main_floats)) {
        set_error("wgrad: slab scratch too small");
        return PN_ERR_WORKSPACE;
      }
      const pn_operand we = plain(m.We, K), wt = plain(m.Wt, K);
      static const bool pm_small = !(getenv("PN_PM_SMALL") && atoi(getenv("PN_PM_SMALL")) == 0);
      const WgradDesc pmd{we, wt, 1, C, K, K, rows, sl, PN_PREC_BF16X3, 0, pm_small ? 1 : 0};
      PN_TRY(conv_wgrad_batch(&pmd, 1, st));
      PN_TRY(slab_reduce_q(sl, spc, (long long)K * K, m.Pm, p(r.kernel), m.f, K, C, m.q, st));
    }
    PN_TRY(maxbwd_scatter(m.arg, hs_loc, m.Wt, m.q, B, N, K, C, m.D, s16, st));
    PN_TRY(conv_bwd_data(&xop, m.Pm, 0, B, N, K, K, m.D, prev.Z, prev.scale, prev.shift, prev.dy, w.bpart, prec, st));
    return PN_OK;
  }
  int bwd_dense(DLs& dl, const LRef& r, const float* xin, const float* da, int act, const unsigned char* keep, float* dx_out) {
    const int mode = r.has_bn ? (bn_batch(r.block) ? 1 : 2) : 0;
    const bool wg = tr(r.block) && G;
    const float ks = 1.f / (1.f - d.dropout_rate);
    float* dgam = (wg && mode == 1) ? gr(r.gamma) : nullptr;
    float* dbet = (wg && mode == 1) ? gr(r.beta) : nullptr;
    float* dbia = (wg && mode == 0) ? gr(r.bias) : nullptr;
    if (Bd <= 32) {
      PN_TRY(dense_bwd_fused(da, dl.z, xin, r.cin, Bd, r.cin, r.cout, p(r.gamma), p(r.beta), dl.mean, dl.invstd, mode, act, keep, ks, dl.dz,
                             dgam, dbet, dbia, wg ? gr(r.kernel) : nullptr, st));
    } else {
      PN_TRY(dense_bwd_pre(da, dl.z, Bd, r.cout, p(r.gamma), p(r.beta), dl.mean, dl.invstd, mode, act, keep, ks, dl.dz, dgam, dbet, dbia, st));
      if (wg) {
        const float* dzp = dl.dz;
        float* out = gr(r.kernel);
        const int ci = r.cin, cj = r.cout;
        const int rows = Bd;
        PN_TRY(side([=] { return dense_wgrad(xin, ci, dzp, rows, ci, cj, out, st); }));
        PN_TRY(flush());
      }
    }
    if (dx_out) PN_TRY(dense_plain(dl.dz, r.cout, p(r.kernel), r.cout, true, r.cout, r.cin, nullptr, dx_out));
    return PN_OK;
  }
  bool chain_ok() const { return Bd <= 32; }
  int bwd_chain(const float* dtop, int Ctop, const float* Wtop, const float* a_below_top, float* dWtop, float* dbtop, float* da_top,
                ChainLayer* ls, int n, float* dx_out, const PrepCarry* carry = nullptr, bool* carried = nullptr, bool top_done = false) {
    if (dWtop) dense_jobs.push_back(DenseWgradJob{a_below_top, ls[0].r->cout, dtop, Bd, ls[0].r->cout, Ctop, dWtop, dbtop});
    const float* dz_above = dtop;
    int c_above = Ctop;
    const float* w_above = Wtop;
    float* dx_above = da_top;
    for (int q = 0; q < n; ++q) {
      DLs& dl = *ls[q].dl;
      const LRef& r = *ls[q].r;
      const bool wg = tr(r.block) && G;
      const DenseTail t = chain_tail(ls[q]);
      if (!(q == 0 && top_done))
      PN_TRY(dense_trans_tail(dz_above, c_above, w_above, c_above, Bd, c_above, r.cout, w.dense_part, w.dcount, dx_above, &t, st));
      if (wg) dense_jobs.push_back(DenseWgradJob{ls[q].xin, r.cin, dl.dz, Bd, r.cin, r.cout, gr(r.kernel), nullptr});
      dz_above = dl.dz; c_above = r.cout; w_above = p(r.kernel); dx_above = dl.din;
    }
    if (carry)
      return dense_trans_prep_carry(dz_above, c_above, w_above, c_above, Bd, c_above, ls[n - 1].r->cin, w.dense_part, w.dcount, dx_out, carry, st, carried);
    return dense_trans_tail(dz_above, c_above, w_above, c_above, Bd, c_above, ls[n - 1].r->cin, w.dense_part, w.dcount, dx_out, nullptr, st);
  }
  int bwd_tnet(TN& t, const TRef& r, const pn_operand* x, WgradFuse* wf = nullptr, bool* fused = nullptr) {
    if (fused) *fused = false;
    const int KK = r.K * r.K;
    const bool wg = tr(r.c1.block) && G;
    PN_TRY(sync_gather_rows(t.dR, (long long)B * KK));
    bool prep_carried = false;
    if (chain_ok()) {
      ChainLayer ls[2] = {{&t.d2, &r.d2, t.d1.a, 1, nullptr}, {&t.d1, &r.d1, pooled(t.m3), 1, nullptr}};
      const bool pcar = prep_carries(r.c3);
      const PrepCarry pc = prep_carry(t.c3, t.m3, r.c3, lazy(t.c2), nullptr);
      PN_TRY(bwd_chain(t.dR, KK, p(r.w), t.d2.a, wg ? gr(r.w) : nullptr, wg ? gr(r.b) : nullptr, t.da2, ls, 2, t.m3.dG, pcar ? &pc : nullptr, &prep_carried));
    } else {
    if (wg) {
      const float *dR = t.dR, *a2 = t.d2.a;
      float *gb = gr(r.b), *gw = gr(r.w);
      const int rows = Bd;
      PN_TRY(side([=] {
        return dense_wgrad(a2, 256, dR, rows, 256, KK, gw, st, gb);
      }));
      PN_TRY(flush());
    }
    PN_TRY(dense_plain(t.dR, KK, p(r.w), KK, true, KK, 256, nullptr, t.da2));
    PN_TRY(bwd_dense(t.d2, r.d2, t.d1.a, t.da2, 1, nullptr, t.d2.din));
    PN_TRY(bwd_dense(t.d1, r.d1, pooled(t.m3), t.d2.din, 1, nullptr, t.m3.dG));
    }
    PN_TRY(bwd_max(t.c3, t.m3, r.c3, lazy(t.c2), t.c2, t.m3.dG, nullptr, prep_carried));
    PN_TRY(bwd_step(t.c2, r.c2, t.c1, lazy(t.c1)));
    PN_TRY(bn_bwd_fin(t.c1, r.c1, w.bpart));
    const pn_operand dz1 = dzop(t.c1);
    if (wg) {
      float* out = gr(r.c1.kernel);
      if (r.K == 3) {
        PN_TRY(side([=] { return wgrad3_to(dz1, out); }));
      } else {
        const pn_operand xin = *x;
        const bool fz = wf && fused && wgrad_fuse_take(xin, 64, 64, out, *wf);
        if (fz) *fused = true;
        else PN_TRY(side([=] { return wgrad_to(xin, dz1, 64, 64, out, false, true); }));
      }
      PN_TRY(flush());
    }
    return PN_OK;
  }

  int backward(const float* d_cls, const float* d_seg, const float* d_R) {
    const int rc = backward_body(d_cls, d_seg, d_R);
    if (rc != PN_OK) return rc;
    return flush_jobs();
  }
  int backward_body(const float* d_cls, const float* d_seg, const float* d_R) {
    if (!G) {
      set_error("pn_model_backward: grads buffer is NULL");
      return PN_ERR_INVALID_ARGUMENT;
    }
    const pn_operand x64 = x64op();
    const float* Ws1 = p(L.s1.kernel);
    const bool fused = io.labels_cls != nullptr || io.labels_seg != nullptr;
    bool has_seg = d_seg != nullptr || (io.labels_seg != nullptr && io.loss_weights[1] != 0.f);
    if (has_seg && fused_seg_head()) {
      set_error("pn_model_backward: a gradient through the segmentation head was asked for, but the forward pass ran the head fused "
                "(frozen, loss weight 0) and kept none of its activations; set PN_IO_KEEP_ACTIVATIONS in pn_model_io.flags");
      return PN_ERR_INVALID_ARGUMENT;
    }
    bool has_cls = d_cls != nullptr || (io.labels_cls != nullptr && io.loss_weights[0] != 0.f);
    (void)fused;
    const bool have_R_grad = !d.vanilla && (d_R != nullptr || (io.se3 != nullptr && io.loss_weights[2] != 0.f) || d.reg_in);
    const bool trunk = has_seg || has_cls || (!d.vanilla && d.reg_feat);
    const int phase = io.bwd_phase;
    if (phase != 2) {
    if (!io.zero_grads_in_forward) PN_TRY(zero_fill2(G, L.total, reinterpret_cast<float*>(w.dcount), DENSE_MAX_COUNTERS, st));

    bool have_dx64 = false;
    bool have_dGseg = false;
    if (has_seg) {
      if (d_seg) PN_TRY(softmax_bwd_rows(io.out_seg, d_seg, M, d.cseg, w.seg_dlogits, st));
      const pn_operand a4 = lazy(w.s4);
      PN_TRY(seg_out_bwd(&a4, p(L.s5.kernel), w.seg_dlogits, B, N, 128, d.cseg, w.s4.dy, w.bpart, w.s5slab, st, s16));
      if (tr(BLK_S5)) {
        PN_TRY(side([=] {
          if (!aux) jobs.push_back(SlabJob{w.s5slab, gr(L.s5.kernel), (long long)128 * d.cseg, T});
          else PN_TRY(slab_reduce(w.s5slab, T, T, (long long)128 * d.cseg, gr(L.s5.kernel), st));
          if (!d_seg) return sum_partials(w.seg_part + 2, (int)cdivll(M, seg_out_part_rows()), seg_out_part_stride(), d.cseg, gr(L.s5.bias), st);
          return sum_partials(w.seg_dlogits, (int)M, d.cseg, d.cseg, gr(L.s5.bias), st);
        }));
        PN_TRY(flush());
      }
      PN_TRY(bwd_step(w.s4, L.s4, w.s3, lazy(w.s3)));
      PN_TRY(bwd_step(w.s3, L.s3, w.s2, lazy(w.s2)));
      PN_TRY(bwd_step(w.s2, L.s2, w.s1, lazy(w.s1)));
      PN_TRY(bn_bwd_fin(w.s1, L.s1, w.bpart));
      const pn_operand dz1 = dzop(w.s1);
      PN_TRY(cloud_bias_grad(w.bpart, w.s1.part, B, tpc, N, 512, w.s1.ca, w.s1.cb, w.s1.cc, w.dgb, st));
      if (tr(BLK_S1)) {
        PN_TRY(side([=] {
          PN_TRY(wgrad_to(x64, dz1, 64, 512, gr(L.s1.kernel), false, true));
          return dense_wgrad(pooled_local(w.mm23, 1024), 1024, w.dgb, B, 1024, 512, gr(L.s1.kernel) + 64 * 512, st);
        }));
        PN_TRY(flush());
      }
      PN_TRY(dense_plain(w.dgb, 512, Ws1 + 64 * 512, 512, true, 512, 1024, nullptr, loc(w.dGseg, 1024), B));
      PN_TRY(sync_gather_rows(w.dGseg, (long long)B * 1024));
      have_dGseg = true;
      PN_TRY(conv_bwd_data(&dz1, Ws1, 0, B, N, 512, 64, nullptr, nullptr, nullptr, nullptr, w.dX64, nullptr, prec, st, w.s1.w16));
      have_dx64 = true;
    }

    bool have_dGcls = false, cls_prep_carried = false;
    if (has_cls) {
      if (d_cls) PN_TRY(softmax_bwd_rows(io.out_cls, d_cls, B, d.ccls, loc(w.cls_dlogits, d.ccls), st));
      PN_TRY(sync_gather_rows(w.cls_dlogits, (long long)B * d.ccls));
      if (chain_ok()) {
        const bool wg3 = tr(BLK_C3) && G;
        ChainLayer ls[2] = {{&w.c2, &L.c2, w.c1.a, 1, io.keep2}, {&w.c1, &L.c1, pooled(w.mm23), 1, io.keep1}};
        const bool pcar = prep_carries(L.m23);
        const PrepCarry pc = prep_carry(w.m23, w.mm23, L.m23, lazy(w.m22), have_dGseg ? w.dGseg : nullptr);
        PN_TRY(bwd_chain(w.cls_dlogits, d.ccls, p(L.c3.kernel), w.c2.a, wg3 ? gr(L.c3.kernel) : nullptr, wg3 ? gr(L.c3.bias) : nullptr,
                         w.c3.din, ls, 2, w.dGcls, pcar ? &pc : nullptr, &cls_prep_carried, loss_carries() && !d_cls));
      } else {
      PN_TRY(bwd_dense(w.c3, L.c3, w.c2.a, w.cls_dlogits, 0, nullptr, w.c3.din));
      PN_TRY(bwd_dense(w.c2, L.c2, w.c1.a, w.c3.din, 1, io.keep2, w.c2.din));
      PN_TRY(bwd_dense(w.c1, L.c1, pooled(w.mm23), w.c2.din, 1, io.keep1, w.dGcls));
      }
      have_dGcls = true;
    }
    const float* dGa = have_dGcls ? w.dGcls : nullptr;
    const float* dGb = have_dGseg ? w.dGseg : nullptr;

    if (!trunk && !have_R_grad) return PN_OK;

    if (has_seg || has_cls) {
      PN_TRY(bwd_max(w.m23, w.mm23, L.m23, lazy(w.m22), w.m22, dGa, dGb, cls_prep_carried));
      PN_TRY(bwd_step(w.m22, L.m22, w.m21, lazy(w.m21)));
      PN_TRY(bn_bwd_fin(w.m21, L.m21, w.bpart));
      const pn_operand dz21 = dzop(w.m21);
      WgradFuse wf21;
      bool fz21 = false;
      if (tr(BLK_M21)) {
        fz21 = wgrad_fuse_take(x64, 64, 64, gr(L.m21.kernel), wf21);
        if (!fz21) {
          PN_TRY(side([=] { return wgrad_to(x64, dz21, 64, 64, gr(L.m21.kernel), false, true); }));
          PN_TRY(flush());
        }
      }
      if (d.vanilla) {
        PN_TRY(conv_bwd_data(&dz21, p(L.m21.kernel), 0, B, N, 64, 64, have_dx64 ? w.dX64 : nullptr, w.m12.Z, w.m12.scale, w.m12.shift,
                             w.m12.dy, w.bpart, prec, st, w.m21.w16, nullptr, fz21 ? &wf21 : nullptr));
      } else {
        PN_TRY(conv_bwd_data(&dz21, p(L.m21.kernel), 0, B, N, 64, 64, have_dx64 ? w.dX64 : nullptr, nullptr, nullptr, nullptr, w.dX64,
                             nullptr, prec, st, w.m21.w16, nullptr, fz21 ? &wf21 : nullptr));
      }
    }
    if (!d.vanilla) {
      const pn_operand a12 = lazy(w.m12);
      const bool have_dx = has_seg || has_cls;
      float* fdR = loc(w.fT.dR, 4096);
      const float* fR = loc(w.fT.R, 4096);
      if (!have_dx) PN_TRY(zero_fill(fdR, (long long)B * 4096, st));
      if (have_dx) {
        const pn_operand dx = plain_act(w.dX64, 64);
        static const bool dr64_ride = !(getenv("PN_DR64_RIDE") && atoi(getenv("PN_DR64_RIDE")) == 0);
        int spc;
        const int rows = (int)wgrad_slab_rows(B, N, 64, 64, &spc);
        float* sl = cur_slabs();
        if ((size_t)B * spc * 4096 > (sl == w.slabs ? w.slab_floats : w.slab_main_floats)) {
          set_error("wgrad: slab scratch too small");
          return PN_ERR_WORKSPACE;
        }
        PN_TRY(conv_wgrad(&a12, &dx, B, N, 64, 64, rows, sl, prec, st, 0));
        bool rode = false;
        if (dr64_ride && W == 1)
// ... 99 lines not shown
}
int pn_model_slot_info(const pn_model_desc* d, int i, pn_slot_info* out) {
  PN_TRY(check_desc(d));
  const Layout L = make_layout(*d);
  PN_CHECK_ARG(out && i >= 0 && i < (int)L.slots.size(), "pn_model_slot_info: index %d out of range", i);
  const Slot& s = L.slots[i];
  memset(out, 0, sizeof(*out));
  strncpy(out->name, s.name.c_str(), sizeof(out->name) - 1);
  out->offset = s.off; out->rows = s.rows; out->cols = s.cols; out->kind = s.kind; out->block = s.block;
  return PN_OK;
}
size_t pn_model_workspace_bytes(const pn_model_desc* d, int B, int N, int training) {
  if (check_desc(d) != PN_OK || B <= 0 || N <= 0) return 0;
  Arena A;
  WS w;
  plan_ws(A, w, *d, B, N, training != 0);
  return A.off;
}
int pn_model_ws_lookup(const pn_model_desc* d, int B, int N, int training, const char* name, int64_t* offset, int64_t* bytes) {
  PN_TRY(check_desc(d));
  PN_CHECK_ARG(name && offset && bytes && B > 0 && N > 0, "pn_model_ws_lookup: bad arguments");
  Arena A;
  WS w;
  std::vector<std::pair<std::string, std::pair<size_t, size_t>>> dir;
  A.dir = &dir;
  plan_ws(A, w, *d, B, N, training != 0);
  for (auto& e : dir)
    if (e.first == name) {
      *offset = (int64_t)e.second.first;
      *bytes = (int64_t)e.second.second;
      return PN_OK;
    }
  set_error("pn_model_ws_lookup: no workspace buffer named '%s'", name);
  return PN_ERR_INVALID_ARGUMENT;
}
int pn_model_ws_entry(const pn_model_desc* d, int B, int N, int training, int index, char* name_out, int name_cap, int64_t* offset,
                      int64_t* bytes) {
  PN_TRY(check_desc(d));
  PN_CHECK_ARG(name_out && name_cap > 0 && offset && bytes && B > 0 && N > 0, "pn_model_ws_entry: bad arguments");
  Arena A;
  WS w;
  std::vector<std::pair<std::string, std::pair<size_t, size_t>>> dir;
  A.dir = &dir;
  plan_ws(A, w, *d, B, N, training != 0);
  if (index < 0 || index >= (int)dir.size()) return 1;
  strncpy(name_out, dir[index].first.c_str(), name_cap - 1);
  name_out[name_cap - 1] = 0;
  *offset = (int64_t)dir[index].second.first;
  *bytes = (int64_t)dir[index].second.second;
  return PN_OK;
}
int64_t pn_model_wgrad_fused_count(void) { return (int64_t)g_wgrad_fused_count.load(); }
int64_t pn_model_plan_count(int which) { return (which >= 0 && which < 3) ? (int64_t)g_plan_count[which].load() : -1; }
int pn_model_forward(const pn_model_desc* d, const pn_model_io* io, pn_stream stream) {
  Run* r = nullptr;
  PN_TRY(make_run(d, io, reinterpret_cast<hipStream_t>(stream), r));
  const int rc = r->forward();
  delete r;
  return rc;
}
int pn_model_backward(const pn_model_desc* d, const pn_model_io* io, const float* d_cls, const float* d_seg, const float* d_R,
                      pn_stream stream) {
  Run* r = nullptr;
  PN_TRY(make_run(d, io, reinterpret_cast<hipStream_t>(stream), r));
  int rc;
  if (!r->training) {
    set_error("pn_model_backward: the forward pass must have run with training=1");
    rc = PN_ERR_INVALID_ARGUMENT;
  } else {
    rc = r->backward(d_cls, d_seg, d_R);
    const int rj = r->join();
    if (rc == PN_OK) rc = rj;
  }
  delete r;
  return rc;
}
int pn_adam_prepare(const int32_t* iterations, float* alpha_scratch, double lr0, double decay_rate, double decay_steps, double beta1, double beta2,
                    pn_stream stream) {
  return adam_prepare(iterations, lr0, decay_rate, decay_steps, beta1, beta2, alpha_scratch, reinterpret_cast<hipStream_t>(stream));
}
int pn_adam_step(float* params, const float* grads, float* m, float* v, int64_t n, int32_t* iterations, float* alpha_scratch, double lr0,
                 double decay_rate, double decay_steps, double beta1, double beta2, double eps, float grad_scale, pn_stream stream) {
  hipStream_t st = reinterpret_cast<hipStream_t>(stream);
  PN_CHECK_ARG(iterations && alpha_scratch, "pn_adam_step: null pointer");
  return adam_fused(params, grads, m, v, n, iterations, lr0, decay_rate, decay_steps, beta1, beta2, eps, grad_scale, alpha_scratch, st);
}

}
```

### pointcloudprocessing_amd/csrc/pn_segout.hip

```cpp
#include "pn_common.h"
#include "pn_loss_bodies.h"

namespace pn {

constexpr int SEG_CM = 16;
constexpr int SEG_RPB = 128;

typedef __attribute__((ext_vector_type(8))) __bf16 seg_bf16x8;
typedef __attribute__((ext_vector_type(16))) float seg_f32x16;
constexpr int SEG_WP = 128 + 8;

__device__ __forceinline__ void seg_row_probs(const float (&acc)[SEG_CM], int C, float (&p)[SEG_CM], int& am) {
    float mx = -INFINITY;
    am = 0;
#pragma unroll
    for (int c = 0; c < SEG_CM; ++c)
      if (c < C && acc[c] > mx) { mx = acc[c]; am = c; }
    float sum = 0.f;
#pragma unroll
    for (int c = 0; c < SEG_CM; ++c) {
      p[c] = c < C ? expf(acc[c] - mx) : 0.f;
      sum += p[c];
    }
    const float inv = 1.f / sum;
#pragma unroll
    for (int c = 0; c < SEG_CM; ++c) p[c] *= inv;
}
__device__ __forceinline__ void seg_row_loss(const float (&p)[SEG_CM], int C, int y, int am, float& loss, float& corr, float& qs) {
    float py = 1.f;
    qs = 0.f;
#pragma unroll
    for (int c = 0; c < SEG_CM; ++c)
      if (c < C) {
        const float pc = clip_nan(p[c], 1e-7f, 1.f - 1e-7f);
        qs += pc;
        if (c == y) py = pc;
      }
    loss = -(logf(py) - logf(qs));
    corr = (am == y) ? 1.f : 0.f;
}
__device__ __forceinline__ void seg_row_tail(const float (&acc)[SEG_CM], int C, long long row, const int* __restrict__ labels, float grad_scale,
                                             float* __restrict__ probs, float* __restrict__ dlogits, float& loss, float& corr,
                                             float (&dl)[SEG_CM]) {
    float p[SEG_CM];
    int am;
    seg_row_probs(acc, C, p, am);
    if (probs) {
      float* po = probs + row * C;
#pragma unroll
      for (int c = 0; c < SEG_CM; ++c)
        if (c < C) po[c] = p[c];
    }
    if (labels) {
// ... 195 lines not shown
__device__ __forceinline__ float sh_bnrelu(float z, float sc, float sh, int s16) {
  const float zq = s16 ? bf16_bits_f32(f32_bf16_bits(z)) : z;
  return clamp_lo(fmaf(sc, zq, sh), 0.f);
}
struct sh_coef { float4 v[4]; };
__device__ __forceinline__ sh_coef sh_load_coef(const float* __restrict__ p, int c0, int h) {
  sh_coef c;
#pragma unroll
  for (int g = 0; g < 4; ++g) c.v[g] = *reinterpret_cast<const float4*>(p + c0 + 8 * g + 4 * h);
  return c;
}
__device__ __forceinline__ float sh_c(const sh_coef& c, int g, int q) { return q == 0 ? c.v[g].x : (q == 1 ? c.v[g].y : (q == 2 ? c.v[g].z : c.v[g].w)); }
typedef __attribute__((ext_vector_type(2))) float seg_f32x2;
typedef __attribute__((ext_vector_type(2))) __bf16 seg_bf16x2;
template <bool S16, bool BIAS>
__device__ __forceinline__ void sh_bnrelu16(const seg_f32x16& acc, const sh_coef& bias, const sh_coef& sc, const sh_coef& sh, float (&y)[16]) {
#pragma unroll
  for (int g = 0; g < 4; ++g)
#pragma unroll
    for (int q = 0; q < 4; q += 2) {
      float z0 = acc[4 * g + q], z1 = acc[4 * g + q + 1];
      if (BIAS) { z0 += sh_c(bias, g, q); z1 += sh_c(bias, g, q + 1); }
      if (S16) {
        const seg_f32x2 zz = {z0, z1};
        const unsigned u = __builtin_bit_cast(unsigned, __builtin_convertvector(zz, seg_bf16x2));
        z0 = __builtin_bit_cast(float, u << 16);
        z1 = __builtin_bit_cast(float, u & 0xffff0000u);
      }
      y[4 * g + q] = clamp_lo(fmaf(sh_c(sc, g, q), z0, sh_c(sh, g, q)), 0.f);
      y[4 * g + q + 1] = clamp_lo(fmaf(sh_c(sc, g, q + 1), z1, sh_c(sh, g, q + 1)), 0.f);
    }
}
__device__ __forceinline__ void sh_store16(__bf16* img, int pitch, int row, int c0, int h, const float (&y)[16]) {
#pragma unroll
  for (int g = 0; g < 4; ++g) {
    const seg_f32x2 a = {y[4 * g], y[4 * g + 1]}, b = {y[4 * g + 2], y[4 * g + 3]};
    uint2 w;
    w.x = __builtin_bit_cast(unsigned, __builtin_convertvector(a, seg_bf16x2));
    w.y = __builtin_bit_cast(unsigned, __builtin_convertvector(b, seg_bf16x2));
    *reinterpret_cast<uint2*>(img + row * pitch + c0 + 8 * g + 4 * h) = w;
  }
}
#define SH_KEEP_ABOVE() asm volatile("" ::: "memory")
#define SH_BARRIER() asm volatile("s_waitcnt lgkmcnt(0)\n\ts_barrier" ::: "memory")
#define SH_STAMP(i) do { if (DBG) stamp[i] = (unsigned)__builtin_amdgcn_s_memtime(); } while (0)
constexpr int SH_CO_GB = 0, SH_CO_SC1 = 512, SH_CO_SH1 = 1024, SH_CO_SC2 = 1536, SH_CO_SH2 = 1792, SH_CO_SC3 = 2048, SH_CO_SH3 = 2176, SH_CO_SC4 = 2304,
              SH_CO_SH4 = 2432, SH_CO_B5 = 2560, SH_CO_FLOATS = 2560 + SEG_CM;
constexpr int sh_region_c(int) { return 2 * SEG_CM * SEG_WP * 2; }
static_assert((32 - SEG_CM) * SEG_WP * 2 <= SH_CO_FLOATS * 4, "the unused class rows of the lo image stay inside the allocation");
constexpr int sh_region_d() { return SH_CO_FLOATS * 4; }
constexpr int sh_lds_bytes(int rows) { return sh_region_a(rows) + sh_region_b(rows) + sh_region_c(rows) + sh_region_d(); }
static_assert(sh_lds_bytes(128) <= 160 * 1024 && 2 * sh_lds_bytes(64) <= 160 * 1024, "one 128-row workgroup or two 64-row workgroups per CU");
template <int MB, bool S16, bool DBG = false>
__global__ __launch_bounds__(256, MB == 2 ? 2 : 1) void seg_head_fused_kernel(const SegHeadArgs a) {
  constexpr int ROWS = 32 * MB, SH_REGION_A = sh_region_a(ROWS), SH_REGION_B = sh_region_b(ROWS), SH_REGION_C = sh_region_c(ROWS);
  unsigned stamp[DBG ? 24 : 1];
  SH_STAMP(0);
  extern __shared__ __attribute__((aligned(16))) unsigned char sh_sm[];
  __bf16* Ain = reinterpret_cast<__bf16*>(sh_sm);
  __bf16* S1c = Ain + ROWS * SH_P64;
  __bf16* S3 = reinterpret_cast<__bf16*>(sh_sm);
  __bf16* S2 = reinterpret_cast<__bf16*>(sh_sm + SH_REGION_A);
  float* S4f = reinterpret_cast<float*>(sh_sm + SH_REGION_A);
  float* prob_s = reinterpret_cast<float*>(sh_sm + SH_REGION_A);
  __bf16* W5hi = reinterpret_cast<__bf16*>(sh_sm + SH_REGION_A + SH_REGION_B);
  __bf16* W5lo = W5hi + SEG_CM * SEG_WP;
  float* lgt = reinterpret_cast<float*>(sh_sm);
  float* coef = reinterpret_cast<float*>(sh_sm + SH_REGION_A + SH_REGION_B + SH_REGION_C);
  const int tid = threadIdx.x, lane = tid & 63, wave = tid >> 6;
  const int r = lane & 31, h = lane >> 5;
  const int cloud = blockIdx.x / a.tiles_per_cloud, tin = blockIdx.x - cloud * a.tiles_per_cloud;
  const int r0 = tin * ROWS, nrows = min(ROWS, a.N - r0);
  const long long row0 = (long long)cloud * a.N + r0;

  auto afrag = [&](const __bf16* img, int pitch, int m, int k0) {
    return *reinterpret_cast<const seg_bf16x8*>(img + (m * 32 + r) * pitch + k0 + 8 * h);
  };
  auto bfrag = [&](const unsigned short* wt, int K, int cb, int ks) {
    return __builtin_bit_cast(seg_bf16x8, *reinterpret_cast<const uint4*>(wt + (((long long)cb * (K >> 4) + ks) * 64 + lane) * 8));
  };

  seg_bf16x8 b1[4], b2[8][2];
#pragma unroll
  for (int ks = 0; ks < 4; ++ks) { b1[ks] = bfrag(a.w1t, 64, wave, ks); }
#pragma unroll
  for (int ks = 0; ks < 8; ++ks)
#pragma unroll
    for (int n = 0; n < 2; ++n) b2[ks][n] = bfrag(a.w2t, 512, 2 * wave + n, ks);
  float4 cf[3];
#pragma unroll
  for (int q = 0; q < 3; ++q) {
    const int i = tid + 256 * q;
    const float* src = a.gb + (long long)cloud * 512;
    int off = i;
    if (i >= 128) { src = a.sc1; off = i - 128; }
    if (i >= 256) { src = a.sh1; off = i - 256; }
    if (i >= 384) { src = a.sc2; off = i - 384; }
    if (i >= 448) { src = a.sh2; off = i - 448; }
    if (i >= 512) { src = a.sc3; off = i - 512; }
    if (i >= 544) { src = a.sh3; off = i - 544; }
    if (i >= 576) { src = a.sc4; off = i - 576; }
    if (i >= 608) { src = a.sh4; off = i - 608; }
    cf[q] = i < 640 ? *reinterpret_cast<const float4*>(src + 4 * off) : make_float4(0.f, 0.f, 0.f, 0.f);
  }
  const float b5v = (tid < SEG_CM && tid < a.C && a.b5) ? a.b5[tid] : 0.f;
  const int prow = 64 * wave + lane;
  const int ylab = (a.labels && wave < MB / 2 && prow < nrows) ? a.labels[row0 + prow] : 0;
  float w5v[SEG_CM * 128 / 256];
#pragma unroll
  for (int q = 0; q < SEG_CM * 64 / 256; ++q) {
    const int t = tid + 256 * q, c = t >> 6, k = 2 * (t & 63);
    w5v[2 * q] = c < a.C ? a.w5[(long long)k * a.C + c] : 0.f;
    w5v[2 * q + 1] = c < a.C ? a.w5[(long long)(k + 1) * a.C + c] : 0.f;
  }
  SH_KEEP_ABOVE();
  SH_STAMP(22);

#pragma unroll
  for (int pass = 0; pass < ROWS / 64; ++pass) {
    const int row = pass * 64 + (tid >> 2), c0 = (tid & 3) * 16;
    float v[16];
    const long long src = (row0 + min(row, nrows - 1)) * a.x.ld + c0;
    if (a.x.h16) {
      bf16x8_unpack(act_load8_raw(a.x.s1, src), *reinterpret_cast<float(*)[8]>(v));
// ... 183 lines not shown
      acc = __builtin_amdgcn_mfma_f32_32x32x16_bf16(ah, bl, acc, 0, 0, 0);
      acc = __builtin_amdgcn_mfma_f32_32x32x16_bf16(ah, bh, acc, 0, 0, 0);
    }
    if (r < SEG_CM) {
#pragma unroll
      for (int e = 0; e < 16; ++e) lgt[(wave * 32 + (e & 3) + 8 * (e >> 2) + 4 * h) * (SEG_CM + 1) + r] = acc[e];
    }
  }
  SH_STAMP(19);
  SH_BARRIER();
  SH_STAMP(20);
  if (wave < MB / 2) {
    float loss = 0.f, corr = 0.f;
    if (prow < nrows) {
      float acc[SEG_CM], p[SEG_CM];
#pragma unroll
      for (int c = 0; c < SEG_CM; ++c) {
        acc[c] = (c < a.C && a.b5) ? coef[SH_CO_B5 + c] : 0.f;
        acc[c] += lgt[prow * (SEG_CM + 1) + c];
      }
      int am;
      seg_row_probs(acc, a.C, p, am);
#pragma unroll
      for (int c = 0; c < SEG_CM; ++c)
        if (c < a.C) prob_s[prow * a.C + c] = p[c];
      if (a.labels) {
        float qs;
        seg_row_loss(p, a.C, ylab, am, loss, corr, qs);
      }
    }
    if (a.part && r0 + 64 * wave < a.N) {
      float* pp = a.part + ((long long)cloud * ((a.N + 63) / 64) + (r0 >> 6) + wave) * (2 + SEG_CM);
      const float l = wave_sum(loss), cr = wave_sum(corr);
      if (lane == 0) { pp[0] = l; pp[1] = cr; }
    }
  }
  if (a.probs) {
    SH_BARRIER();
    const int n = nrows * a.C;
    float* dst = a.probs + row0 * a.C;
    for (int i = 4 * tid; i + 3 < n; i += 1024) *reinterpret_cast<float4*>(dst + i) = *reinterpret_cast<const float4*>(prob_s + i);
    if (tid < (n & 3)) dst[(n & ~3) + tid] = prob_s[(n & ~3) + tid];
  }
  if (DBG) {
    SH_STAMP(21);
    __syncthreads();
    if (tid == 0 && a.probs && nrows * a.C >= 24) {
      unsigned* p = reinterpret_cast<unsigned*>(a.probs + row0 * a.C);
#pragma unroll
      for (int i = 0; i < 24; ++i) p[i] = stamp[i];
    }
  }
}
#undef SH_STAMP
#undef SH_KEEP_ABOVE
#undef SH_BARRIER
int seg_head_fused_rows() { return SH_ROWS; }
int seg_head_fused(const pn_operand* x, const float* gb, const void* w1t, const void* w2t, const void* w3t, const void* w4t, const float* sc1,
                   const float* sh1, const float* sc2, const float* sh2, const float* sc3, const float* sh3, const float* sc4, const float* sh4,
                   const float* w5, const float* b5, int B, int N, int C, int s16, const int* labels, float grad_scale, float* probs,
                   float* dlogits, float* part, hipStream_t st) {
  PN_CHECK_ARG(x && x->s1 && !x->s2 && gb && w1t && w2t && w3t && w4t && sc1 && sh1 && sc2 && sh2 && sc3 && sh3 && sc4 && sh4 && w5,
               "seg_head_fused: null pointer");
  PN_CHECK_ARG(B > 0 && N > 0 && C >= 1 && C <= SEG_CM, "seg_head_fused: bad sizes (B=%d N=%d C=%d)", B, N, C);
  PN_CHECK_ARG(x->ld >= 64 && x->ld % 8 == 0 && (reinterpret_cast<uintptr_t>(x->s1) & 15) == 0, "seg_head_fused: operand alignment");
  SegHeadArgs a;
  memset(&a, 0, sizeof(a));
  a.x = *x; a.gb = gb;
  a.w1t = reinterpret_cast<const unsigned short*>(w1t); a.w2t = reinterpret_cast<const unsigned short*>(w2t);
  a.w3t = reinterpret_cast<const unsigned short*>(w3t); a.w4t = reinterpret_cast<const unsigned short*>(w4t);
  a.sc1 = sc1; a.sh1 = sh1; a.sc2 = sc2; a.sh2 = sh2; a.sc3 = sc3; a.sh3 = sh3; a.sc4 = sc4; a.sh4 = sh4;
  a.w5 = w5; a.b5 = b5; a.N = N; a.C = C; a.s16 = s16;
  a.labels = labels; a.grad_scale = grad_scale; a.probs = probs; a.dlogits = dlogits; a.part = part;
  static const int force_mb = getenv("PN_SEGHEAD_MB") ? atoi(getenv("PN_SEGHEAD_MB")) : 0;
  static const bool dbg = getenv("PN_SEGHEAD_DBG") && atoi(getenv("PN_SEGHEAD_DBG")) == 16;
  const bool tall = force_mb == 4;
  if (tall) {
    static const hipError_t attr1 = hipFuncSetAttribute(reinterpret_cast<const void*>(&seg_head_fused_kernel<4, true>), hipFuncAttributeMaxDynamicSharedMemorySize,
                                                        sh_lds_bytes(128));
    static const hipError_t attr0 = hipFuncSetAttribute(reinterpret_cast<const void*>(&seg_head_fused_kernel<4, false>), hipFuncAttributeMaxDynamicSharedMemorySize,
                                                        sh_lds_bytes(128));
    PN_CHECK_ARG(attr1 == hipSuccess && attr0 == hipSuccess, "seg_head_fused: dynamic LDS attribute");
    a.tiles_per_cloud = cdiv(N, 128);
    if (dbg && s16 && N % 128 == 0) {
      static const hipError_t attrd = hipFuncSetAttribute(reinterpret_cast<const void*>(&seg_head_fused_kernel<4, true, true>), hipFuncAttributeMaxDynamicSharedMemorySize,
                                                          sh_lds_bytes(128));
      PN_CHECK_ARG(attrd == hipSuccess, "seg_head_fused: dynamic LDS attribute");
      hipLaunchKernelGGL((seg_head_fused_kernel<4, true, true>), dim3(B * a.tiles_per_cloud), dim3(256), sh_lds_bytes(128), st, a);
    } else
    if (s16) hipLaunchKernelGGL((seg_head_fused_kernel<4, true>), dim3(B * a.tiles_per_cloud), dim3(256), sh_lds_bytes(128), st, a);
    else hipLaunchKernelGGL((seg_head_fused_kernel<4, false>), dim3(B * a.tiles_per_cloud), dim3(256), sh_lds_bytes(128), st, a);
  } else {
    a.tiles_per_cloud = cdiv(N, 64);
    static const hipError_t attr3 = hipFuncSetAttribute(reinterpret_cast<const void*>(&seg_head_fused_kernel<2, true>), hipFuncAttributeMaxDynamicSharedMemorySize,
                                                        sh_lds_bytes(64));
    static const hipError_t attr2 = hipFuncSetAttribute(reinterpret_cast<const void*>(&seg_head_fused_kernel<2, false>), hipFuncAttributeMaxDynamicSharedMemorySize,
                                                        sh_lds_bytes(64));
    PN_CHECK_ARG(attr3 == hipSuccess && attr2 == hipSuccess, "seg_head_fused: dynamic LDS attribute");
    if (dbg && s16 && N % 64 == 0) {
      static const hipError_t attrd = hipFuncSetAttribute(reinterpret_cast<const void*>(&seg_head_fused_kernel<2, true, true>), hipFuncAttributeMaxDynamicSharedMemorySize,
                                                          sh_lds_bytes(64));
      PN_CHECK_ARG(attrd == hipSuccess, "seg_head_fused: dynamic LDS attribute");
      hipLaunchKernelGGL((seg_head_fused_kernel<2, true, true>), dim3(B * a.tiles_per_cloud), dim3(256), sh_lds_bytes(64), st, a);
    } else
    if (s16) hipLaunchKernelGGL((seg_head_fused_kernel<2, true>), dim3(B * a.tiles_per_cloud), dim3(256), sh_lds_bytes(64), st, a);
    else hipLaunchKernelGGL((seg_head_fused_kernel<2, false>), dim3(B * a.tiles_per_cloud), dim3(256), sh_lds_bytes(64), st, a);
  }
  PN_CHECK_LAUNCH();
  return PN_OK;
}

__global__ __launch_bounds__(256) void seg_out_bwd_kernel(const pn_operand x, const float* __restrict__ w,
                                                          const float* __restrict__ dlogits, int N, int C, int tiles_per_cloud,
                                                          float* __restrict__ dyhat, float* __restrict__ stat_part,
                                                          float* __restrict__ wslab, int store16) {
  constexpr int K = 128;
  __shared__ float red[128][2 + SEG_CM];
  __shared__ __attribute__((aligned(16))) float out_s[128 * SEG_CM];
  const int bx = blockIdx.x, cloud = bx / tiles_per_cloud, tin = bx - cloud * tiles_per_cloud;
  const int k = threadIdx.x & 127, stream = threadIdx.x >> 7;
  float wk[SEG_CM], gw[SEG_CM];
#pragma unroll
  for (int c = 0; c < SEG_CM; ++c) {
    wk[c] = c < C ? w[(long long)k * C + c] : 0.f;
    gw[c] = 0.f;
  }
  const float ca = x.ca ? x.ca[k] : 1.f, cc = x.cc ? x.cc[k] : 0.f, lo = x.lo;
  const int r0 = tin * 128 + stream * 64, r1 = min(N, r0 + 64);
// ... 140 lines not shown
```

Baseline: 48.07 million points/s.

## Co-launch small dense layers with seg-head tiles and wgrad gram tiles

Moves the dense layer body into a shared header that takes its LDS buffer from the caller, so it can run inside other kernels. Adds a fill kernel that runs a small dense layer's blocks alongside segmentation-head tiles in one grid, and a prep-carry kernel that also runs wgrad gram tiles. The goal is to fill idle CUs during small, latency-bound launches and to cut the number of kernel launches. In exchange, shared LDS sizing and dispatch logic grow more complex, and the heterogeneous blocks may balance load poorly.

```diff
diff --git a/include/pointnet_hip.h b/include/pointnet_hip.h
--- a/include/pointnet_hip.h
+++ b/include/pointnet_hip.h
@@ -259,6 +259,7 @@
 
 int64_t pn_model_plan_count(int which);
 int64_t pn_model_wgrad_fused_count(void);
+int64_t pn_model_fill_count(int which);
 
 int pn_model_forward(const pn_model_desc* d, const pn_model_io* io, pn_stream stream);
 int pn_model_backward(const pn_model_desc* d, const pn_model_io* io, const float* d_cls, const float* d_seg,
diff --git a/pointcloudprocessing_amd/_lib.py b/pointcloudprocessing_amd/_lib.py
--- a/pointcloudprocessing_amd/_lib.py
+++ b/pointcloudprocessing_amd/_lib.py
@@ -146,6 +146,7 @@
     "pn_model_ws_lookup": (_I, [_DESC, _I, _I, _I, C.c_char_p, C.POINTER(C.c_int64), C.POINTER(C.c_int64)]),
     "pn_model_ws_entry": (_I, [_DESC, _I, _I, _I, _I, C.c_char_p, _I, C.POINTER(C.c_int64), C.POINTER(C.c_int64)]),
     "pn_model_plan_count": (_I64, [_I]),
+    "pn_model_fill_count": (_I64, [_I]),
     "pn_model_wgrad_fused_count": (_I64, []),
     "pn_model_forward": (_I, [_DESC, _IO, _P]),
     "pn_model_backward": (_I, [_DESC, _IO, _P, _P, _P, _P]),
diff --git a/pointcloudprocessing_amd/csrc/pn_dense.hip b/pointcloudprocessing_amd/csrc/pn_dense.hip
--- a/pointcloudprocessing_amd/csrc/pn_dense.hip
+++ b/pointcloudprocessing_amd/csrc/pn_dense.hip
@@ -1,38 +1,12 @@
 #include "pn_common.h"
+#include "pn_dense_body.h"
 #include "pn_dense_wgrad.h"
+#include "pn_gemm_core.h"
 #include "pn_internal.h"
 #include "pn_loss_bodies.h"
 #include "pn_maxbwd_bodies.h"
 
 namespace pn {
-
-typedef __attribute__((ext_vector_type(8))) __bf16 bf16x8;
-typedef __attribute__((ext_vector_type(16))) float f32x16;
-
-constexpr int DL_COLS = 32;
-constexpr int DL_SLICES = 8;
-constexpr int DL_KPS = 16;
-constexpr int DL_KSTEP = DL_SLICES * DL_KPS;
-constexpr int DL_ROWS = 32;
-constexpr int DL_MAX_SPLITS = 8;
-
-struct DenseArgs {
-  const float* x; int ldx;
-  const float* w; int ldw;
-  int R, K, C, split_len, nsplit;
-  float* partial;
-  unsigned* counters;
-  const float *bias, *gamma, *beta;
-  float *mm, *mv;
-  float momentum, eps;
-  int bn_mode, act;
-  const unsigned char* keep; float keep_scale;
-  float *z_out, *a_out, *mean_o, *invstd_o;
-  const float *bt_z, *bt_gamma, *bt_beta, *bt_mean, *bt_invstd;
-  const unsigned char* bt_keep; float bt_keep_scale;
-  int bt_mode, bt_act;
-  float *bt_dz, *bt_dgamma, *bt_dbeta, *bt_dbias;
-};
 
 static inline int dl_ksplit_env() {
   static const int v = (getenv("PN_DENSE_KSPLIT") && atoi(getenv("PN_DENSE_KSPLIT")) >= 1) ? atoi(getenv("PN_DENSE_KSPLIT")) : 0;
@@ -46,314 +20,10 @@
 }
 static inline int dl_split_len(int K) { return cdiv(cdiv(K, dl_nsplit(K)), DL_KSTEP) * DL_KSTEP; }
 
-template <bool TRANS, int DEPTH, bool VEC, bool CARRY = false>
-__device__ __forceinline__ bool dense_layer_body(const DenseArgs& a, const unsigned bxi, const int ks, float* zr_out = nullptr) {
-  __shared__ __attribute__((aligned(16))) float lds[4 * DL_ROWS * DL_COLS + 16 * 32 + 4];
-  float* red = lds;
-  float* fin = lds + 4 * DL_ROWS * DL_COLS;
-  unsigned* flag = reinterpret_cast<unsigned*>(fin + 16 * 32);
-  const int tid = threadIdx.x, c = tid & 31, s = tid >> 5;
-  const int j = bxi * DL_COLS + c;
-  const int jc = j < a.C ? j : a.C - 1;
-  const int kbeg = ks * a.split_len, kend = min(a.K, kbeg + a.split_len);
-  const bool single = a.nsplit == 1;
-  const bool small = a.R <= DL_ROWS;
-  float own[DL_ROWS / DL_SLICES];
-  float pf_g = 1.f, pf_b = 0.f, pf_mm = 0.f, pf_mv = 1.f;
-  const float pf_bias = a.bias ? a.bias[jc] : 0.f;
-  unsigned char pf_kb[DL_ROWS / DL_SLICES] = {1, 1, 1, 1};
-  if (a.bn_mode) { pf_g = a.gamma[jc]; pf_b = a.beta[jc]; pf_mm = a.mm[jc]; pf_mv = a.mv[jc]; }
-  if (a.keep && a.a_out && a.R <= DL_ROWS) {
-#pragma unroll
-    for (int i = 0; i < DL_ROWS / DL_SLICES; ++i) pf_kb[i] = a.keep[(long long)min(s + DL_SLICES * i, a.R - 1) * a.C + jc];
-  }
-  float bt_zz[DL_ROWS / DL_SLICES], bt_mu = 0.f, bt_is = 1.f, bt_g = 1.f, bt_b = 0.f;
-  unsigned char bt_kb[DL_ROWS / DL_SLICES] = {1, 1, 1, 1};
-  if (TRANS && a.bt_dz) {
-#pragma unroll
-    for (int i = 0; i < DL_ROWS / DL_SLICES; ++i) bt_zz[i] = a.bt_z[(long long)min(s + DL_SLICES * i, a.R - 1) * a.C + jc];
-    if (a.bt_keep) {
-#pragma unroll
-      for (int i = 0; i < DL_ROWS / DL_SLICES; ++i) bt_kb[i] = a.bt_keep[(long long)min(s + DL_SLICES * i, a.R - 1) * a.C + jc];
-    }
-    if (a.bt_mode) { bt_mu = a.bt_mean[jc]; bt_is = a.bt_invstd[jc]; bt_g = a.bt_gamma[jc]; bt_b = a.bt_beta[jc]; }
-  }
-
-  const int lane = tid & 63, wv = tid >> 6;
-  const int lr = lane & 31, lg = lane >> 5;
-  const int jw = bxi * DL_COLS + lr;
-  const int jwc = jw < a.C ? jw : a.C - 1;
-  for (int rc = 0; rc < a.R; rc += DL_ROWS) {
-    const int nr = min(DL_ROWS, a.R - rc);
-    f32x16 acc;
-#pragma unroll
-    for (int e = 0; e < 16; ++e) acc[e] = 0.f;
-    const int xr = rc + (lr < nr ? lr : nr - 1);
-    float xa[DEPTH][8], wb[DEPTH][8];
-    auto issue = [&](float (&xv)[8], float (&wv_)[8], int k0) {
-      const int kk = k0 + 8 * lg;
-      if constexpr (VEC) {
-        const int kc = min(kk, kend - 8);
-        const float4 t0 = *reinterpret_cast<const float4*>(a.x + (long long)xr * a.ldx + kc);
-        const float4 t1 = *reinterpret_cast<const float4*>(a.x + (long long)xr * a.ldx + kc + 4);
-        xv[0] = t0.x; xv[1] = t0.y; xv[2] = t0.z; xv[3] = t0.w; xv[4] = t1.x; xv[5] = t1.y; xv[6] = t1.z; xv[7] = t1.w;
-        if constexpr (TRANS) {
-          const float4 u0 = *reinterpret_cast<const float4*>(a.w + (long long)jwc * a.ldw + kc);
-          const float4 u1 = *reinterpret_cast<const float4*>(a.w + (long long)jwc * a.ldw + kc + 4);
-          wv_[0] = u0.x; wv_[1] = u0.y; wv_[2] = u0.z; wv_[3] = u0.w; wv_[4] = u1.x; wv_[5] = u1.y; wv_[6] = u1.z; wv_[7] = u1.w;
-        } else {
-#pragma unroll
-          for (int e = 0; e < 8; ++e) wv_[e] = a.w[(long long)(kc + e) * a.ldw + jwc];
-        }
-      } else {
-#pragma unroll
-        for (int e = 0; e < 8; ++e) {
-          const int k = kk + e;
-          const long long kc = k < kend ? k : kend - 1;
-          xv[e] = a.x[(long long)xr * a.ldx + kc];
-          wv_[e] = TRANS ? a.w[(long long)jwc * a.ldw + kc] : a.w[kc * a.ldw + jwc];
-        }
-      }
-    };
-    const int kw = kbeg + 16 * wv;
-    const int nsteps = kw < kend ? (kend - kw + 63) / 64 : 0;
-    for (int base = 0; base < nsteps; base += DEPTH) {
-#pragma unroll
-      for (int d = 0; d < DEPTH; ++d)
-        if (base + d < nsteps) issue(xa[d], wb[d], kw + 64 * (base + d));
-#pragma unroll
-      for (int d = 0; d < DEPTH; ++d) {
-        const int i = base + d;
-        if (i >= nsteps) break;
-        const int k0 = kw + 64 * i;
-        bf16x8 ah, al, bh, bl;
-#pragma unroll
-        for (int e = 0; e < 8; ++e) {
-          const bool kv = k0 + 8 * lg + e < kend;
-          const float xv = (kv && lr < nr) ? xa[d][e] : 0.f;
-          const float wvv = (kv && jw < a.C) ? wb[d][e] : 0.f;
-          ah[e] = (__bf16)xv;
-          al[e] = (__bf16)(xv - (float)ah[e]);
-          bh[e] = (__bf16)wvv;
-          bl[e] = (__bf16)(wvv - (float)bh[e]);
-        }
-        acc = __builtin_amdgcn_mfma_f32_32x32x16_bf16(al, bh, acc, 0, 0, 0);
-        acc = __builtin_amdgcn_mfma_f32_32x32x16_bf16(ah, bl, acc, 0, 0, 0);
-        acc = __builtin_amdgcn_mfma_f32_32x32x16_bf16(ah, bh, acc, 0, 0, 0);
-      }
-    }
-    __syncthreads();
-#pragma unroll
-    for (int e = 0; e < 16; ++e) red[(wv * DL_ROWS + (e & 3) + 8 * (e >> 2) + 4 * lg) * DL_COLS + lr] = acc[e];
-    __syncthreads();
-#pragma unroll
-    for (int i = 0; i < DL_ROWS / DL_SLICES; ++i) {
-      const int r = s + DL_SLICES * i;
-      const float t = (red[(0 * DL_ROWS + r) * DL_COLS + c] + red[(1 * DL_ROWS + r) * DL_COLS + c]) +
-                      (red[(2 * DL_ROWS + r) * DL_COLS + c] + red[(3 * DL_ROWS + r) * DL_COLS + c]);
-      own[i] = t;
-      if (!(single && small) && r < nr && j < a.C)
-        __hip_atomic_store(&a.partial[((long long)ks * a.R + rc + r) * a.C + j], t, __ATOMIC_RELAXED, __HIP_MEMORY_SCOPE_AGENT);
-    }
-  }
-
-  if (!single) {
-    asm volatile("s_waitcnt vmcnt(0)" ::: "memory");
-    __syncthreads();
-    if (tid == 0) {
-      const unsigned t = __hip_atomic_fetch_add(a.counters + bxi, 1u, __ATOMIC_RELAXED, __HIP_MEMORY_SCOPE_AGENT);
-      const unsigned last = (t == (unsigned)a.nsplit - 1u) ? 1u : 0u;
-      if (last) __hip_atomic_store(a.counters + bxi, 0u, __ATOMIC_RELAXED, __HIP_MEMORY_SCOPE_AGENT);
-      *flag = last;
-    }
-    __syncthreads();
-    if (*flag == 0u) return false;
-  } else {
-    __syncthreads();
-  }
-
-  const int R = a.R, C = a.C, nks = a.nsplit;
-  const int tx = c, ty = s;
-  constexpr int RP = DL_SLICES;
-  const bool jv = j < C;
-  const float b = jv ? pf_bias : 0.f;
-  float zr[DL_ROWS / RP];
-  float s1 = 0.f;
-  if (small && single) {
-#pragma unroll
-    for (int i = 0; i < DL_ROWS / RP; ++i) {
-      const int r = ty + RP * i;
-      const float z = own[i] + b;
-      zr[i] = z;
-      if (jv && r < R) {
-        a.z_out[(long long)r * C + j] = z;
-        s1 += z;
-      }
-    }
-  } else if (small) {
-    float pv[DL_ROWS / RP][DL_MAX_SPLITS];
-#pragma unroll
-    for (int i = 0; i < DL_ROWS / RP; ++i) {
-      const int r = min(ty + RP * i, R - 1);
-#pragma unroll
-      for (int q = 0; q < DL_MAX_SPLITS; ++q)
-        pv[i][q] = __hip_atomic_load(&a.partial[((long long)min(q, nks - 1) * R + r) * C + jc], __ATOMIC_RELAXED, __HIP_MEMORY_SCOPE_AGENT);
-    }
-#pragma unroll
-    for (int i = 0; i < DL_ROWS / RP; ++i) {
-      float z0 = 0.f, z1 = 0.f;
-#pragma unroll
-      for (int q = 0; q < DL_MAX_SPLITS; q += 2) {
-        z0 += (q < nks) ? pv[i][q] : 0.f;
-        z1 += (q + 1 < nks) ? pv[i][q + 1] : 0.f;
-      }
-      const int r = ty + RP * i;
-      const float z = (z0 + z1) + b;
-      zr[i] = z;
-      if (jv && r < R) {
-        a.z_out[(long long)r * C + j] = z;
-        s1 += z;
-      }
-    }
-  } else if (jv) {
-    for (int r = ty; r < R; r += RP) {
-      float z0 = 0.f, z1 = 0.f;
-      int q = 0;
-      for (; q + 1 < nks; q += 2) {
-        z0 += __hip_atomic_load(&a.partial[((long long)q * R + r) * C + j], __ATOMIC_RELAXED, __HIP_MEMORY_SCOPE_AGENT);
-        z1 += __hip_atomic_load(&a.partial[((long long)(q + 1) * R + r) * C + j], __ATOMIC_RELAXED, __HIP_MEMORY_SCOPE_AGENT);
-      }
-      if (q < nks) z0 += __hip_atomic_load(&a.partial[((long long)q * R + r) * C + j], __ATOMIC_RELAXED, __HIP_MEMORY_SCOPE_AGENT);
-      const float z = (z0 + z1) + b;
-      a.z_out[(long long)r * C + j] = z;
-      s1 += z;
-    }
-  }
-  float sc = 1.f, sh = 0.f;
-  if (a.bn_mode) {
-    float mean = 0.f, var = 1.f;
-    if (a.bn_mode == 1) {
-      __syncthreads();
-      fin[ty * 32 + tx] = s1;
-      __syncthreads();
-      float t = 0.f;
-      for (int q = 0; q < RP; ++q) t += fin[q * 32 + tx];
-      mean = t / (float)R;
-      float s2 = 0.f;
-      if (small) {
-#pragma unroll
-        for (int i = 0; i < DL_ROWS / RP; ++i) {
-          const float d = zr[i] - mean;
-          s2 = (jv && ty + RP * i < R) ? fmaf(d, d, s2) : s2;
-        }
-      } else if (jv) {
-        for (int r = ty; r < R; r += RP) {
-          const float d = a.z_out[(long long)r * C + j] - mean;
-          s2 = fmaf(d, d, s2);
-        }
-      }
-      fin[(8 + ty) * 32 + tx] = s2;
-      __syncthreads();
-      t = 0.f;
-      for (int q = 0; q < RP; ++q) t += fin[(8 + q) * 32 + tx];
-      var = t / (float)R;
-      if (ty == 0 && jv) {
-        a.mm[j] = pf_mm * a.momentum + mean * (1.f - a.momentum);
-        a.mv[j] = pf_mv * a.momentum + var * (1.f - a.momentum);
-      }
-    } else if (jv) {
-      mean = pf_mm;
-      var = pf_mv;
-    }
-    const float invstd = 1.0f / sqrtf(var + a.eps);
-    if (jv) {
-      sc = pf_g * invstd;
-      sh = pf_b - mean * sc;
-      if (ty == 0) {
-        if (a.mean_o) a.mean_o[j] = mean;
-        if (a.invstd_o) a.invstd_o[j] = invstd;
-      }
-    }
-  }
-  if (TRANS && a.bt_dz) {
-    float bsc = 1.f, bsh = 0.f;
-    const float mu = bt_mu, is = bt_is;
-    if (a.bt_mode) {
-      bsc = bt_g * is;
-      bsh = bt_b - mu * bsc;
-    }
-    const float kscale = a.bt_keep ? a.bt_keep_scale : 1.f;
-    float v[DL_ROWS / RP], zh[DL_ROWS / RP];
-    const float (&zz)[DL_ROWS / DL_SLICES] = bt_zz;
-    float S1 = 0.f, S2 = 0.f;
-#pragma unroll
-    for (int i = 0; i < DL_ROWS / RP; ++i) {
-      const int r = ty + RP * i;
-      float d = bt_kb[i] ? zr[i] * kscale : 0.f;
-      if (a.bt_act == 1 && !(fmaf(bsc, zz[i], bsh) > 0.f)) d = 0.f;
-      if (r >= R || !jv) d = 0.f;
-      zh[i] = (zz[i] - mu) * is;
-      v[i] = d;
-      S1 += d;
-      S2 = fmaf(d, zh[i], S2);
-    }
-    __syncthreads();
-    fin[ty * 32 + tx] = S1;
-    fin[(8 + ty) * 32 + tx] = S2;
-    __syncthreads();
-    S1 = 0.f; S2 = 0.f;
-#pragma unroll
-    for (int q = 0; q < RP; ++q) { S1 += fin[q * 32 + tx]; S2 += fin[(8 + q) * 32 + tx]; }
-    const float invR = 1.f / (float)R;
-    const float m1 = S1 * invR, m2 = S2 * invR;
-#pragma unroll
-    for (int i = 0; i < DL_ROWS / RP; ++i) {
-      const int r = ty + RP * i;
-      float d = v[i];
-      if (a.bt_mode == 1) d = bsc * (d - m1 - zh[i] * m2);
-      else if (a.bt_mode == 2) d *= bsc;
-      if (jv && r < R) a.bt_dz[(long long)r * C + j] = d;
-    }
-    if (ty == 0 && jv) {
-      if (a.bt_mode == 1) {
-        if (a.bt_dgamma) a.bt_dgamma[j] = S2;
-        if (a.bt_dbeta) a.bt_dbeta[j] = S1;
-      } else if (a.bt_mode == 0 && a.bt_dbias) {
-        a.bt_dbias[j] = S1;
-      }
-    }
-  }
-  if (a.a_out && jv) {
-    if (small) {
-#pragma unroll
-      for (int i = 0; i < DL_ROWS / RP; ++i) {
-        const int r = ty + RP * i;
-        if (r < R) {
-          float y = fmaf(sc, zr[i], sh);
-          if (a.act == 1) y = clamp_lo(y, 0.f);
-          if (a.keep) y = pf_kb[i] ? y * a.keep_scale : 0.f;
-          a.a_out[(long long)r * C + j] = y;
-        }
-      }
-    } else {
-      for (int r = ty; r < R; r += RP) {
-        float y = fmaf(sc, a.z_out[(long long)r * C + j], sh);
-        if (a.act == 1) y = clamp_lo(y, 0.f);
-        if (a.keep) y = a.keep[(long long)r * C + j] ? y * a.keep_scale : 0.f;
-        a.a_out[(long long)r * C + j] = y;
-      }
-    }
-  }
-  if constexpr (CARRY) {
-#pragma unroll
-    for (int i = 0; i < DL_ROWS / RP; ++i) zr_out[i] = zr[i];
-  }
-  return true;
-}
-
 template <bool TRANS, int DEPTH, bool VEC>
 __global__ __launch_bounds__(256) void dense_layer_kernel(const DenseArgs a0, const DenseArgs a1) {
-  (void)dense_layer_body<TRANS, DEPTH, VEC>(blockIdx.z ? a1 : a0, blockIdx.x, blockIdx.y);
+  __shared__ __attribute__((aligned(16))) float lds[DL_LDS_FLOATS];
+  (void)dense_layer_body<TRANS, DEPTH, VEC>(blockIdx.z ? a1 : a0, blockIdx.x, blockIdx.y, lds);
 }
 
 template <int NT>
@@ -361,6 +31,7 @@
                                                                const __bf16* __restrict__ wf_hi, const __bf16* __restrict__ wf_lo,
                                                                const int* __restrict__ argq, int N, int K, int C, int quarters_per_cloud,
                                                                int* __restrict__ arg) {
+  __shared__ __attribute__((aligned(16))) float lds[DL_LDS_FLOATS];
   const int lin = (int)blockIdx.x;
   if (lin >= n_dense) {
     max_resolve_body<NT>(x, wf_hi, wf_lo, argq, N, K, C, quarters_per_cloud, arg, lin - n_dense);
@@ -370,10 +41,30 @@
   PrepPre pre;
   maxbwd_prep_preload(pa, bx, pre);
   float zr[DL_ROWS / DL_SLICES];
-  if (!dense_layer_body<true, 2, true, true>(a, (unsigned)bx, ks, zr)) return;
+  if (!dense_layer_body<true, 2, true, true>(a, (unsigned)bx, ks, lds, zr)) return;
   maxbwd_prep_body<true>(pa, bx, &pre, zr);
 }
-
+__global__ __launch_bounds__(256) void dense_prep_carry_gram_kernel(const DenseArgs a, int ncb, int n_dense, const PrepArgs pa, const pn_operand x,
+                                                                    const __bf16* __restrict__ wf_hi, const int* __restrict__ argq, int N, int K, int C,
+                                                                    int quarters_per_cloud, int* __restrict__ arg, const WgradBatch wb, int n_gram) {
+  constexpr int RAW = GemmLds<128, 128, 1>::BYTES > DL_LDS_FLOATS * 4 ? GemmLds<128, 128, 1>::BYTES : DL_LDS_FLOATS * 4;
+  __shared__ __attribute__((aligned(16))) unsigned char raw[RAW];
+  const int lin = (int)blockIdx.x;
+  if (lin >= n_dense + n_gram) {
+    max_resolve_body<1>(x, wf_hi, nullptr, argq, N, K, C, quarters_per_cloud, arg, lin - n_dense - n_gram);
+    return;
+  }
+  if (lin >= n_dense) {
+    wgrad_batch_tile<128, 128, 1, false>(wb, lin - n_dense, raw);
+    return;
+  }
+  const int ks = lin / ncb, bx = lin - ks * ncb;
+  PrepPre pre;
+  maxbwd_prep_preload(pa, bx, pre);
+  float zr[DL_ROWS / DL_SLICES];
+  if (!dense_layer_body<true, 2, true, true>(a, (unsigned)bx, ks, reinterpret_cast<float*>(raw), zr)) return;
+  maxbwd_prep_body<true>(pa, bx, &pre, zr);
+}
 
 struct LossCarryArgs {
   const int* labels; float grad_scale; float *probs, *dlogits, *loss_sum, *correct;
@@ -384,6 +75,7 @@
 __global__ __launch_bounds__(256) void dense_loss_carry_kernel(const DenseArgs a, const DenseArgs t, const LossCarryArgs lc, int ncb) {
   __shared__ float rl[32], rc[32];
   __shared__ double wsum[16];
+  __shared__ __attribute__((aligned(16))) float lds_a[DL_LDS_FLOATS], lds_t[DL_LDS_FLOATS];
   int bx = blockIdx.x;
   if (bx >= ncb) {
     bx -= ncb;
@@ -400,11 +92,11 @@
   DenseArgs a2 = a, t2 = t;
   a2.z_out = lg;
   t2.x = dl;
-  (void)dense_layer_body<false, 4, true>(a2, 0u, 0);
+  (void)dense_layer_body<false, 4, true>(a2, 0u, 0, lds_a);
   __syncthreads();
   softmax_xent_rows_body<true>(lg, a.R, a.C, lc.labels, lc.grad_scale, pr, dl, ls, cr, rl, rc);
   __syncthreads();
-  (void)dense_layer_body<true, 2, false>(t2, (unsigned)bx, 0);
+  (void)dense_layer_body<true, 2, false>(t2, (unsigned)bx, 0, lds_t);
 }
 
 constexpr int DB_TPW = 2;
@@ -731,15 +423,26 @@
   a.bt_dz = a.bt_dgamma = a.bt_dbeta = a.bt_dbias = nullptr;
   return PN_OK;
 }
+static int dense_depth(const DenseArgs& a) {
+  const int steps = cdiv(a.split_len, 64);
+  return steps <= 2 ? 2 : (steps <= 4 ? 4 : 8);
+}
+template <bool TRANS>
+static bool dense_aligned(const DenseArgs& q) {
+  return q.K % 16 == 0 && q.ldx % 4 == 0 && (reinterpret_cast<uintptr_t>(q.x) & 15) == 0 &&
+         (!TRANS || (q.ldw % 4 == 0 && (reinterpret_cast<uintptr_t>(q.w) & 15) == 0));
+}
+int dense_call_args(const DenseCall& d, DenseArgs& a, int* depth, bool* vec) {
+  PN_TRY(dense_args(a, d.x, d.ldx, d.w, d.ldw, d.R, d.K, d.C, d.partial, d.counters, d.bias, d.gamma, d.beta, d.mm, d.mv, d.momentum, d.eps, d.bn_mode,
+                    d.act, d.keep, d.keep_scale, d.z_out, d.a_out, d.mean_o, d.invstd_o));
+  *depth = dense_depth(a);
+  *vec = dense_aligned<false>(a);
+  return PN_OK;
+}
 template <bool TRANS>
 static void launch_dense(const DenseArgs& a, const DenseArgs& b, dim3 grid, hipStream_t st) {
-  const int steps = cdiv(a.split_len, 64);
-  const int depth = steps <= 2 ? 2 : (steps <= 4 ? 4 : 8);
-  auto aligned = [](const DenseArgs& q) {
-    return q.K % 16 == 0 && q.ldx % 4 == 0 && (reinterpret_cast<uintptr_t>(q.x) & 15) == 0 &&
-           (!TRANS || (q.ldw % 4 == 0 && (reinterpret_cast<uintptr_t>(q.w) & 15) == 0));
-  };
-  const bool vec = aligned(a) && aligned(b);
+  const int depth = dense_depth(a);
+  const bool vec = dense_aligned<TRANS>(a) && dense_aligned<TRANS>(b);
 #define PN_DENSE_CASE(D, V) hipLaunchKernelGGL((dense_layer_kernel<TRANS, D, V>), grid, dim3(256), 0, st, a, b)
   if (vec) { if (depth == 2) PN_DENSE_CASE(2, true); else if (depth == 4) PN_DENSE_CASE(4, true); else PN_DENSE_CASE(8, true); }
   else PN_DENSE_CASE(2, false);
@@ -793,8 +496,9 @@
 }
 
 int dense_trans_prep_carry(const float* dz, int lddz, const float* w, int ldw, int R, int K, int C, float* partial, unsigned* counters, float* dx,
-                           const PrepCarry* pc, hipStream_t st, bool* carried) {
+                           const PrepCarry* pc, hipStream_t st, bool* carried, bool* gram_rode) {
   *carried = false;
+  if (gram_rode) *gram_rode = false;
   DenseArgs a;
   PN_TRY(dense_args(a, dz, lddz, w, ldw, R, K, C, partial, counters, nullptr, nullptr, nullptr, nullptr, nullptr, 0.f, 0.f, 0, 0, nullptr, 1.f,
                     dx, nullptr, nullptr, nullptr));
@@ -815,7 +519,16 @@
   const int ncb = cdiv(C, DL_COLS), n_dense = ncb * a.nsplit, qpc = cdiv(pc->N, 32);
   const __bf16* wh = reinterpret_cast<const __bf16*>(pc->wf_hi);
   const __bf16* wl = reinterpret_cast<const __bf16*>(pc->wf_lo);
-  if (prec == PN_PREC_BF16X3)
+  const WgradDesc* gq = pc->gram;
+  if (gq && gram_rode && prec == PN_PREC_BF16 && (gq->prec & ~PN_STORE_BF16) == PN_PREC_BF16 && !gq->b.s2 && gq->Ci % 128 == 0 && gq->Cj % 128 == 0 &&
+      !gq->small_tiles) {
+    WgradBatch wb;
+    int n_gram = 0;
+    PN_TRY(wgrad_batch_one(*gq, 128, 128, wb, n_gram));
+    hipLaunchKernelGGL(dense_prep_carry_gram_kernel, dim3(n_dense + n_gram + R * qpc), dim3(256), 0, st, a, ncb, n_dense, pa, pc->x, wh, pc->argq, pc->N,
+                       pc->K, C, qpc, pc->arg, wb, n_gram);
+    *gram_rode = true;
+  } else if (prec == PN_PREC_BF16X3)
     hipLaunchKernelGGL((dense_prep_carry_kernel<2>), dim3(n_dense + R * qpc), dim3(256), 0, st, a, ncb, n_dense, pa, pc->x, wh, wl, pc->argq, pc->N, pc->K, C, qpc, pc->arg);
   else
     hipLaunchKernelGGL((dense_prep_carry_kernel<1>), dim3(n_dense + R * qpc), dim3(256), 0, st, a, ncb, n_dense, pa, pc->x, wh, wl, pc->argq, pc->N, pc->K, C, qpc, pc->arg);
diff --git a/pointcloudprocessing_amd/csrc/pn_dense_body.h b/pointcloudprocessing_amd/csrc/pn_dense_body.h
--- /dev/null
+++ b/pointcloudprocessing_amd/csrc/pn_dense_body.h
@@ -0,0 +1,342 @@
+#pragma once
+#include "pn_common.h"
+#include "pn_internal.h"
+
+namespace pn {
+
+typedef __attribute__((ext_vector_type(8))) __bf16 bf16x8;
+typedef __attribute__((ext_vector_type(16))) float f32x16;
+
+constexpr int DL_COLS = 32;
+constexpr int DL_SLICES = 8;
+constexpr int DL_KPS = 16;
+constexpr int DL_KSTEP = DL_SLICES * DL_KPS;
+constexpr int DL_ROWS = 32;
+constexpr int DL_MAX_SPLITS = 8;
+
+struct DenseArgs {
+  const float* x; int ldx;
+  const float* w; int ldw;
+  int R, K, C, split_len, nsplit;
+  float* partial;
+  unsigned* counters;
+  const float *bias, *gamma, *beta;
+  float *mm, *mv;
+  float momentum, eps;
+  int bn_mode, act;
+  const unsigned char* keep; float keep_scale;
+  float *z_out, *a_out, *mean_o, *invstd_o;
+  const float *bt_z, *bt_gamma, *bt_beta, *bt_mean, *bt_invstd;
+  const unsigned char* bt_keep; float bt_keep_scale;
+  int bt_mode, bt_act;
+  float *bt_dz, *bt_dgamma, *bt_dbeta, *bt_dbias;
+};
+constexpr int DL_LDS_FLOATS = 4 * DL_ROWS * DL_COLS + 16 * 32 + 4;
+
+template <bool TRANS, int DEPTH, bool VEC, bool CARRY = false>
+__device__ __forceinline__ bool dense_layer_body(const DenseArgs& a, const unsigned bxi, const int ks, float* lds, float* zr_out = nullptr) {
+  float* red = lds;
+  float* fin = lds + 4 * DL_ROWS * DL_COLS;
+  unsigned* flag = reinterpret_cast<unsigned*>(fin + 16 * 32);
+  const int tid = threadIdx.x, c = tid & 31, s = tid >> 5;
+  const int j = bxi * DL_COLS + c;
+  const int jc = j < a.C ? j : a.C - 1;
+  const int kbeg = ks * a.split_len, kend = min(a.K, kbeg + a.split_len);
+  const bool single = a.nsplit == 1;
+  const bool small = a.R <= DL_ROWS;
+  float own[DL_ROWS / DL_SLICES];
+  float pf_g = 1.f, pf_b = 0.f, pf_mm = 0.f, pf_mv = 1.f;
+  const float pf_bias = a.bias ? a.bias[jc] : 0.f;
+  unsigned char pf_kb[DL_ROWS / DL_SLICES] = {1, 1, 1, 1};
+  if (a.bn_mode) { pf_g = a.gamma[jc]; pf_b = a.beta[jc]; pf_mm = a.mm[jc]; pf_mv = a.mv[jc]; }
+  if (a.keep && a.a_out && a.R <= DL_ROWS) {
+#pragma unroll
+    for (int i = 0; i < DL_ROWS / DL_SLICES; ++i) pf_kb[i] = a.keep[(long long)min(s + DL_SLICES * i, a.R - 1) * a.C + jc];
+  }
+  float bt_zz[DL_ROWS / DL_SLICES], bt_mu = 0.f, bt_is = 1.f, bt_g = 1.f, bt_b = 0.f;
+  unsigned char bt_kb[DL_ROWS / DL_SLICES] = {1, 1, 1, 1};
+  if (TRANS && a.bt_dz) {
+#pragma unroll
+    for (int i = 0; i < DL_ROWS / DL_SLICES; ++i) bt_zz[i] = a.bt_z[(long long)min(s + DL_SLICES * i, a.R - 1) * a.C + jc];
+    if (a.bt_keep) {
+#pragma unroll
+      for (int i = 0; i < DL_ROWS / DL_SLICES; ++i) bt_kb[i] = a.bt_keep[(long long)min(s + DL_SLICES * i, a.R - 1) * a.C + jc];
+    }
+    if (a.bt_mode) { bt_mu = a.bt_mean[jc]; bt_is = a.bt_invstd[jc]; bt_g = a.bt_gamma[jc]; bt_b = a.bt_beta[jc]; }
+  }
+
+  const int lane = tid & 63, wv = tid >> 6;
+  const int lr = lane & 31, lg = lane >> 5;
+  const int jw = bxi * DL_COLS + lr;
+  const int jwc = jw < a.C ? jw : a.C - 1;
+  for (int rc = 0; rc < a.R; rc += DL_ROWS) {
+    const int nr = min(DL_ROWS, a.R - rc);
+    f32x16 acc;
+#pragma unroll
+    for (int e = 0; e < 16; ++e) acc[e] = 0.f;
+    const int xr = rc + (lr < nr ? lr : nr - 1);
+    float xa[DEPTH][8], wb[DEPTH][8];
+    auto issue = [&](float (&xv)[8], float (&wv_)[8], int k0) {
+      const int kk = k0 + 8 * lg;
+      if constexpr (VEC) {
+        const int kc = min(kk, kend - 8);
+        const float4 t0 = *reinterpret_cast<const float4*>(a.x + (long long)xr * a.ldx + kc);
+        const float4 t1 = *reinterpret_cast<const float4*>(a.x + (long long)xr * a.ldx + kc + 4);
+        xv[0] = t0.x; xv[1] = t0.y; xv[2] = t0.z; xv[3] = t0.w; xv[4] = t1.x; xv[5] = t1.y; xv[6] = t1.z; xv[7] = t1.w;
+        if constexpr (TRANS) {
+          const float4 u0 = *reinterpret_cast<const float4*>(a.w + (long long)jwc * a.ldw + kc);
+          const float4 u1 = *reinterpret_cast<const float4*>(a.w + (long long)jwc * a.ldw + kc + 4);
+          wv_[0] = u0.x; wv_[1] = u0.y; wv_[2] = u0.z; wv_[3] = u0.w; wv_[4] = u1.x; wv_[5] = u1.y; wv_[6] = u1.z; wv_[7] = u1.w;
+        } else {
+#pragma unroll
+          for (int e = 0; e < 8; ++e) wv_[e] = a.w[(long long)(kc + e) * a.ldw + jwc];
+        }
+      } else {
+#pragma unroll
+        for (int e = 0; e < 8; ++e) {
+          const int k = kk + e;
+          const long long kc = k < kend ? k : kend - 1;
+          xv[e] = a.x[(long long)xr * a.ldx + kc];
+          wv_[e] = TRANS ? a.w[(long long)jwc * a.ldw + kc] : a.w[kc * a.ldw + jwc];
+        }
+      }
+    };
+    const int kw = kbeg + 16 * wv;
+    const int nsteps = kw < kend ? (kend - kw + 63) / 64 : 0;
+    for (int base = 0; base < nsteps; base += DEPTH) {
+#pragma unroll
+      for (int d = 0; d < DEPTH; ++d)
+        if (base + d < nsteps) issue(xa[d], wb[d], kw + 64 * (base + d));
+#pragma unroll
+      for (int d = 0; d < DEPTH; ++d) {
+        const int i = base + d;
+        if (i >= nsteps) break;
+        const int k0 = kw + 64 * i;
+        bf16x8 ah, al, bh, bl;
+#pragma unroll
+        for (int e = 0; e < 8; ++e) {
+          const bool kv = k0 + 8 * lg + e < kend;
+          const float xv = (kv && lr < nr) ? xa[d][e] : 0.f;
+          const float wvv = (kv && jw < a.C) ? wb[d][e] : 0.f;
+          ah[e] = (__bf16)xv;
+          al[e] = (__bf16)(xv - (float)ah[e]);
+          bh[e] = (__bf16)wvv;
+          bl[e] = (__bf16)(wvv - (float)bh[e]);
+        }
+        acc = __builtin_amdgcn_mfma_f32_32x32x16_bf16(al, bh, acc, 0, 0, 0);
+        acc = __builtin_amdgcn_mfma_f32_32x32x16_bf16(ah, bl, acc, 0, 0, 0);
+        acc = __builtin_amdgcn_mfma_f32_32x32x16_bf16(ah, bh, acc, 0, 0, 0);
+      }
+    }
+    __syncthreads();
+#pragma unroll
+    for (int e = 0; e < 16; ++e) red[(wv * DL_ROWS + (e & 3) + 8 * (e >> 2) + 4 * lg) * DL_COLS + lr] = acc[e];
+    __syncthreads();
+#pragma unroll
+    for (int i = 0; i < DL_ROWS / DL_SLICES; ++i) {
+      const int r = s + DL_SLICES * i;
+      const float t = (red[(0 * DL_ROWS + r) * DL_COLS + c] + red[(1 * DL_ROWS + r) * DL_COLS + c]) +
+                      (red[(2 * DL_ROWS + r) * DL_COLS + c] + red[(3 * DL_ROWS + r) * DL_COLS + c]);
+      own[i] = t;
+      if (!(single && small) && r < nr && j < a.C)
+        __hip_atomic_store(&a.partial[((long long)ks * a.R + rc + r) * a.C + j], t, __ATOMIC_RELAXED, __HIP_MEMORY_SCOPE_AGENT);
+    }
+  }
+
+  if (!single) {
+    asm volatile("s_waitcnt vmcnt(0)" ::: "memory");
+    __syncthreads();
+    if (tid == 0) {
+      const unsigned t = __hip_atomic_fetch_add(a.counters + bxi, 1u, __ATOMIC_RELAXED, __HIP_MEMORY_SCOPE_AGENT);
+      const unsigned last = (t == (unsigned)a.nsplit - 1u) ? 1u : 0u;
+      if (last) __hip_atomic_store(a.counters + bxi, 0u, __ATOMIC_RELAXED, __HIP_MEMORY_SCOPE_AGENT);
+      *flag = last;
+    }
+    __syncthreads();
+    if (*flag == 0u) return false;
+  } else {
+    __syncthreads();
+  }
+
+  const int R = a.R, C = a.C, nks = a.nsplit;
+  const int tx = c, ty = s;
+  constexpr int RP = DL_SLICES;
+  const bool jv = j < C;
+  const float b = jv ? pf_bias : 0.f;
+  float zr[DL_ROWS / RP];
+  float s1 = 0.f;
+  if (small && single) {
+#pragma unroll
+    for (int i = 0; i < DL_ROWS / RP; ++i) {
+      const int r = ty + RP * i;
+      const float z = own[i] + b;
+      zr[i] = z;
+      if (jv && r < R) {
+        a.z_out[(long long)r * C + j] = z;
+        s1 += z;
+      }
+    }
+  } else if (small) {
+    float pv[DL_ROWS / RP][DL_MAX_SPLITS];
+#pragma unroll
+    for (int i = 0; i < DL_ROWS / RP; ++i) {
+      const int r = min(ty + RP * i, R - 1);
+#pragma unroll
+      for (int q = 0; q < DL_MAX_SPLITS; ++q)
+        pv[i][q] = __hip_atomic_load(&a.partial[((long long)min(q, nks - 1) * R + r) * C + jc], __ATOMIC_RELAXED, __HIP_MEMORY_SCOPE_AGENT);
+    }
+#pragma unroll
+    for (int i = 0; i < DL_ROWS / RP; ++i) {
+      float z0 = 0.f, z1 = 0.f;
+#pragma unroll
+      for (int q = 0; q < DL_MAX_SPLITS; q += 2) {
+        z0 += (q < nks) ? pv[i][q] : 0.f;
+        z1 += (q + 1 < nks) ? pv[i][q + 1] : 0.f;
+      }
+      const int r = ty + RP * i;
+      const float z = (z0 + z1) + b;
+      zr[i] = z;
+      if (jv && r < R) {
+        a.z_out[(long long)r * C + j] = z;
+        s1 += z;
+      }
+    }
+  } else if (jv) {
+    for (int r = ty; r < R; r += RP) {
+      float z0 = 0.f, z1 = 0.f;
+      int q = 0;
+      for (; q + 1 < nks; q += 2) {
+        z0 += __hip_atomic_load(&a.partial[((long long)q * R + r) * C + j], __ATOMIC_RELAXED, __HIP_MEMORY_SCOPE_AGENT);
+        z1 += __hip_atomic_load(&a.partial[((long long)(q + 1) * R + r) * C + j], __ATOMIC_RELAXED, __HIP_MEMORY_SCOPE_AGENT);
+      }
+      if (q < nks) z0 += __hip_atomic_load(&a.partial[((long long)q * R + r) * C + j], __ATOMIC_RELAXED, __HIP_MEMORY_SCOPE_AGENT);
+      const float z = (z0 + z1) + b;
+      a.z_out[(long long)r * C + j] = z;
+      s1 += z;
+    }
+  }
+  float sc = 1.f, sh = 0.f;
+  if (a.bn_mode) {
+    float mean = 0.f, var = 1.f;
+    if (a.bn_mode == 1) {
+      __syncthreads();
+      fin[ty * 32 + tx] = s1;
+      __syncthreads();
+      float t = 0.f;
+      for (int q = 0; q < RP; ++q) t += fin[q * 32 + tx];
+      mean = t / (float)R;
+      float s2 = 0.f;
+      if (small) {
+#pragma unroll
+        for (int i = 0; i < DL_ROWS / RP; ++i) {
+          const float d = zr[i] - mean;
+          s2 = (jv && ty + RP * i < R) ? fmaf(d, d, s2) : s2;
+        }
+      } else if (jv) {
+        for (int r = ty; r < R; r += RP) {
+          const float d = a.z_out[(long long)r * C + j] - mean;
+          s2 = fmaf(d, d, s2);
+        }
+      }
+      fin[(8 + ty) * 32 + tx] = s2;
+      __syncthreads();
+      t = 0.f;
+      for (int q = 0; q < RP; ++q) t += fin[(8 + q) * 32 + tx];
+      var = t / (float)R;
+      if (ty == 0 && jv) {
+        a.mm[j] = pf_mm * a.momentum + mean * (1.f - a.momentum);
+        a.mv[j] = pf_mv * a.momentum + var * (1.f - a.momentum);
+      }
+    } else if (jv) {
+      mean = pf_mm;
+      var = pf_mv;
+    }
+    const float invstd = 1.0f / sqrtf(var + a.eps);
+    if (jv) {
+      sc = pf_g * invstd;
+      sh = pf_b - mean * sc;
+      if (ty == 0) {
+        if (a.mean_o) a.mean_o[j] = mean;
+        if (a.invstd_o) a.invstd_o[j] = invstd;
+      }
+    }
+  }
+  if (TRANS && a.bt_dz) {
+    float bsc = 1.f, bsh = 0.f;
+    const float mu = bt_mu, is = bt_is;
+    if (a.bt_mode) {
+      bsc = bt_g * is;
+      bsh = bt_b - mu * bsc;
+    }
+    const float kscale = a.bt_keep ? a.bt_keep_scale : 1.f;
+    float v[DL_ROWS / RP], zh[DL_ROWS / RP];
+    const float (&zz)[DL_ROWS / DL_SLICES] = bt_zz;
+    float S1 = 0.f, S2 = 0.f;
+#pragma unroll
+    for (int i = 0; i < DL_ROWS / RP; ++i) {
+      const int r = ty + RP * i;
+      float d = bt_kb[i] ? zr[i] * kscale : 0.f;
+      if (a.bt_act == 1 && !(fmaf(bsc, zz[i], bsh) > 0.f)) d = 0.f;
+      if (r >= R || !jv) d = 0.f;
+      zh[i] = (zz[i] - mu) * is;
+      v[i] = d;
+      S1 += d;
+      S2 = fmaf(d, zh[i], S2);
+    }
+    __syncthreads();
+    fin[ty * 32 + tx] = S1;
+    fin[(8 + ty) * 32 + tx] = S2;
+    __syncthreads();
+    S1 = 0.f; S2 = 0.f;
+#pragma unroll
+    for (int q = 0; q < RP; ++q) { S1 += fin[q * 32 + tx]; S2 += fin[(8 + q) * 32 + tx]; }
+    const float invR = 1.f / (float)R;
+    const float m1 = S1 * invR, m2 = S2 * invR;
+#pragma unroll
+    for (int i = 0; i < DL_ROWS / RP; ++i) {
+      const int r = ty + RP * i;
+      float d = v[i];
+      if (a.bt_mode == 1) d = bsc * (d - m1 - zh[i] * m2);
+      else if (a.bt_mode == 2) d *= bsc;
+      if (jv && r < R) a.bt_dz[(long long)r * C + j] = d;
+    }
+    if (ty == 0 && jv) {
+      if (a.bt_mode == 1) {
+        if (a.bt_dgamma) a.bt_dgamma[j] = S2;
+        if (a.bt_dbeta) a.bt_dbeta[j] = S1;
+      } else if (a.bt_mode == 0 && a.bt_dbias) {
+        a.bt_dbias[j] = S1;
+      }
+    }
+  }
+  if (a.a_out && jv) {
+    if (small) {
+#pragma unroll
+      for (int i = 0; i < DL_ROWS / RP; ++i) {
+        const int r = ty + RP * i;
+        if (r < R) {
+          float y = fmaf(sc, zr[i], sh);
+          if (a.act == 1) y = clamp_lo(y, 0.f);
+          if (a.keep) y = pf_kb[i] ? y * a.keep_scale : 0.f;
+          a.a_out[(long long)r * C + j] = y;
+        }
+      }
+    } else {
+      for (int r = ty; r < R; r += RP) {
+        float y = fmaf(sc, a.z_out[(long long)r * C + j], sh);
+        if (a.act == 1) y = clamp_lo(y, 0.f);
+        if (a.keep) y = a.keep[(long long)r * C + j] ? y * a.keep_scale : 0.f;
+        a.a_out[(long long)r * C + j] = y;
+      }
+    }
+  }
+  if constexpr (CARRY) {
+#pragma unroll
+    for (int i = 0; i < DL_ROWS / RP; ++i) zr_out[i] = zr[i];
+  }
+  return true;
+}
+
+int dense_call_args(const DenseCall& d, DenseArgs& a, int* depth, bool* vec);
+
+}
diff --git a/pointcloudprocessing_amd/csrc/pn_internal.h b/pointcloudprocessing_amd/csrc/pn_internal.h
--- a/pointcloudprocessing_amd/csrc/pn_internal.h
+++ b/pointcloudprocessing_amd/csrc/pn_internal.h
@@ -123,9 +123,10 @@
   int prec;
   const int* argq; int N; int* arg;
   float* pm_slabs;
+  const struct WgradDesc* gram;
 };
 int dense_trans_prep_carry(const float* dz, int lddz, const float* w, int ldw, int R, int K, int C, float* partial, unsigned* counters, float* dx,
-                           const PrepCarry* pc, hipStream_t st, bool* carried);
+                           const PrepCarry* pc, hipStream_t st, bool* carried, bool* gram_rode = nullptr);
 struct LossCarry {
   const int* labels; float grad_scale; float *probs, *dlogits, *loss_sum, *correct;
   const float* part; int n, stride, n_sum; float* sum_out;
@@ -150,10 +151,17 @@
 int seg_out_fwd(const pn_operand* x, const float* w, const float* bias, long long M, int K, int C, const int* labels,
                 float grad_scale, float* probs, float* dlogits, float* part, hipStream_t st);
 int seg_head_fused_rows();
+struct DenseCall {
+  const float* x; int ldx; const float* w; int ldw; int R, K, C; float* partial; unsigned* counters;
+  const float *bias, *gamma, *beta; float *mm, *mv; float momentum, eps; int bn_mode, act; const unsigned char* keep; float keep_scale;
+  float *z_out, *a_out, *mean_o, *invstd_o;
+};
+struct SegFill { DenseCall dense; int tile0, ntiles; };
+bool seg_head_fill_fits(const DenseCall& d);
 int seg_head_fused(const pn_operand* x, const float* gb, const void* w1t, const void* w2t, const void* w3t, const void* w4t, const float* sc1,
                    const float* sh1, const float* sc2, const float* sh2, const float* sc3, const float* sh3, const float* sc4, const float* sh4,
                    const float* w5, const float* b5, int B, int N, int C, int s16, const int* labels, float grad_scale, float* probs,
-                   float* dlogits, float* part, hipStream_t st);
+                   float* dlogits, float* part, hipStream_t st, const SegFill* fill = nullptr);
 int seg_out_part_stride();
 int seg_out_part_rows();
 int seg_out_bwd(const pn_operand* x, const float* w, const float* dlogits, int B, int N, int K, int C, float* dyhat, float* stat_part,
diff --git a/pointcloudprocessing_amd/csrc/pn_model.hip b/pointcloudprocessing_amd/csrc/pn_model.hip
--- a/pointcloudprocessing_amd/csrc/pn_model.hip
+++ b/pointcloudprocessing_amd/csrc/pn_model.hip
@@ -10,6 +10,9 @@
 namespace pn {
 
 static std::atomic<long long> g_plan_count[3];
+static std::atomic<long long> g_fill_count[4];
+constexpr int PN_SEG_FILL_DEFAULT = 0;
+constexpr int PN_GRAM_FILL_DEFAULT = 0;
 static std::atomic<long long> g_wgrad_fused_count;
 
 enum { BLK_IT = 0, BLK_M11, BLK_M12, BLK_FT, BLK_M21, BLK_M22, BLK_M23, BLK_C1, BLK_C2, BLK_C3, BLK_S1, BLK_S2, BLK_S3, BLK_S4,
@@ -123,6 +126,9 @@
   float *pmax, *sumsq, *g, *zstar, *hs, *e, *nege, *f, *a1part, *a1, *gram, *GW, *Pm, *q, *D, *Wt, *We, *dG;
   float* gram_slabs = nullptr;
   int gram_rows = 0, gram_spc = 0;
+  float* fill_slabs = nullptr;
+  int fill_rows = 0, fill_spc = 0;
+  bool fill_rode = false;
   int *pq, *argq, *arg;
   unsigned short *wb_hi, *wb_lo;
   int T64, tpc64, rows;
@@ -585,6 +591,19 @@
     return on && training && G && io.zero_grads_in_forward && io.labels_cls && io.loss_weights[0] != 0.f && W == 1 && chain_ok() &&
            dense_loss_carry_fits(w.c2.a, L.c3.cin, Bd, L.c3.cin, d.ccls, L.c2.cout);
   }
+  static int seg_fill() {
+    static const int v = getenv("PN_SEG_FILL") ? atoi(getenv("PN_SEG_FILL")) : PN_SEG_FILL_DEFAULT;
+    return (v == 1 || v == 2) ? v : 0;
+  }
+  static int seg_fill_split() {
+    static const int v = (getenv("PN_SEG_FILL_SPLIT") && atoi(getenv("PN_SEG_FILL_SPLIT")) >= 0) ? atoi(getenv("PN_SEG_FILL_SPLIT")) : -1;
+    return v;
+  }
+  DenseCall dense_call(DLs& dl, const LRef& r, const float* x, int act, const unsigned char* keep) const {
+    const int mode = r.has_bn ? (bn_batch(r.block) ? 1 : 2) : 0;
+    return DenseCall{x, r.cin, p(r.kernel), r.cout, Bd, r.cin, r.cout, w.dense_part, w.dcount, p(r.bias), p(r.gamma), p(r.beta), p(r.mm), p(r.mv),
+                     d.bn_momentum, d.bn_eps, mode, act, keep, 1.f / (1.f - d.dropout_rate), dl.z, dl.a, dl.mean, dl.invstd};
+  }
   struct ChainLayer { DLs* dl; const LRef* r; const float* xin; int act; const unsigned char* keep; };
   DenseTail chain_tail(const ChainLayer& cl) const {
     const DLs& dl = *cl.dl;
@@ -712,9 +731,34 @@
       if (!lcar) PN_TRY(dense_plain(w.c2.a, 256, p(L.c3.kernel), d.ccls, false, 256, d.ccls, p(L.c3.bias), w.cls_logits));
       return PN_OK;
     };
-    if (!lcar) PN_TRY(cls_rest());
-
-    if (fused_seg_head()) {
+    const int sfill = (fused_seg_head() && !lcar) ? seg_fill() : 0;
+    const DenseCall dc2 = dense_call(w.c2, L.c2, w.c1.a, 1, training ? io.keep2 : nullptr);
+    const DenseCall dc3{w.c2.a, 256, p(L.c3.kernel), d.ccls, Bd, 256, d.ccls, w.dense_part, w.dcount, p(L.c3.bias), nullptr, nullptr, nullptr, nullptr,
+                        0.f, 0.f, 0, 0, nullptr, 1.f, w.cls_logits, nullptr, nullptr, nullptr};
+    const bool filled = sfill && seg_head_fill_fits(dc2) && (sfill == 1 || seg_head_fill_fits(dc3));
+    if (filled) {
+      const int tiles = B * cdiv(N, seg_head_fused_rows());
+      const int first = sfill == 1 ? tiles : std::min(tiles, seg_fill_split() >= 0 ? seg_fill_split() : (tiles + 1) / 2);
+      seg_parts = tiles;
+      auto head = [&](const SegFill& f) -> int {
+        return seg_head_fused(&x64, loc(w.gb, 512), w.s1.wt16, w.s2.wt16, w.s3.wt16, w.s4.wt16, w.s1.scale, w.s1.shift, w.s2.scale, w.s2.shift,
+                              w.s3.scale, w.s3.shift, w.s4.scale, w.s4.shift, p(L.s5.kernel), p(L.s5.bias), B, N, d.cseg, s16, io.labels_seg,
+                              fseg ? io.loss_weights[1] / (float)M : 0.f, io.out_seg, nullptr, fseg ? w.seg_part : nullptr, st, &f);
+      };
+      PN_TRY(head(SegFill{dc2, 0, first}));
+      ++g_fill_count[0];
+      g_fill_count[2] += first;
+      if (sfill == 2) {
+        PN_TRY(head(SegFill{dc3, first, tiles - first}));
+        ++g_fill_count[0];
+        g_fill_count[3] += tiles - first;
+      } else {
+        PN_TRY(dense_plain(w.c2.a, 256, p(L.c3.kernel), d.ccls, false, 256, d.ccls, p(L.c3.bias), w.cls_logits));
+      }
+    } else if (!lcar) PN_TRY(cls_rest());
+
+    if (filled) {
+    } else if (fused_seg_head()) {
       seg_parts = B * cdiv(N, seg_head_fused_rows());
       PN_TRY(seg_head_fused(&x64, loc(w.gb, 512), w.s1.wt16, w.s2.wt16, w.s3.wt16, w.s4.wt16, w.s1.scale, w.s1.shift, w.s2.scale, w.s2.shift, w.s3.scale,
                             w.s3.shift, w.s4.scale, w.s4.shift, p(L.s5.kernel), p(L.s5.bias), B, N, d.cseg, s16, io.labels_seg,
@@ -781,10 +825,13 @@
     PN_TRY(conv3_wgrad(w.pcn, &dz, B, N, 64, cur_slabs(), st));
     return slab_reduce(cur_slabs(), T, T, 3 * 64, out, st);
   }
+  static int gram_target() {
+    static const int t_gram = getenv("PN_WGRAD_TARGET_GRAM") ? atoi(getenv("PN_WGRAD_TARGET_GRAM")) : 128;
+    return t_gram;
+  }
   int wgrad_general(const pn_operand& a, const pn_operand& b, int Bq, int Nq, int Ci, int Cj, float* out, bool per_cloud, int pr,
                     bool colsum = false, bool deferrable = false) {
-    static const int t_gram = getenv("PN_WGRAD_TARGET_GRAM") ? atoi(getenv("PN_WGRAD_TARGET_GRAM")) : 128;
-    const int t_over = (deferrable && colsum) ? t_gram : 0;
+    const int t_over = (deferrable && colsum) ? gram_target() : 0;
     int spc;
     const int rows = (int)wgrad_slab_rows(Bq, Nq, Ci, Cj, &spc, t_over);
     const size_t elems = (size_t)Ci * Cj + (colsum ? Ci : 0);
@@ -856,6 +903,23 @@
     static const bool on = !(getenv("PN_PREP_CARRY") && atoi(getenv("PN_PREP_CARRY")) == 0);
     return on && training && W == 1 && chain_ok() && r.cin == 128 && pm_slabs_of(r.cin, r.cout) != nullptr;
   }
+  bool gram_fills(const ML& m, const LRef& r) const {
+    static const bool on = getenv("PN_GRAM_FILL") ? atoi(getenv("PN_GRAM_FILL")) == 1 : PN_GRAM_FILL_DEFAULT == 1;
+    return on && prep_carries(r) && tr(r.block) && G && !aux && B <= 32 && !gram_rides(m, r) && s16 && prec == (PN_PREC_BF16 | PN_STORE_BF16);
+  }
+  const WgradDesc* gram_fill_take(ML& m, const LRef& r, const pn_operand& xop, WgradDesc& gd) {
+    m.fill_slabs = nullptr;
+    m.fill_rode = false;
+    if (!gram_fills(m, r)) return nullptr;
+    const int K = r.cin;
+    int spc;
+    const int rows = (int)wgrad_slab_rows(B, N, K, K, &spc, gram_target());
+    float* ps = pool_take((size_t)B * spc * ((size_t)K * K + K));
+    if (!ps) return nullptr;
+    m.fill_slabs = ps; m.fill_rows = rows; m.fill_spc = spc;
+    gd = WgradDesc{xop, xop, B, N, K, K, rows, ps, prec, 1, 0};
+    return &gd;
+  }
   PrepCarry prep_carry(const CL& l, const ML& m, const LRef& r, const pn_operand& xop, const float* dG2) const {
     const bool wg = tr(r.block) && G;
     PrepCarry c;
@@ -892,6 +956,14 @@
       PN_TRY(side([=] {
         if (gram_rides(mm, r)) {
           jobs.push_back(SlabJob{mm.gram_slabs, mm.gram, (long long)K * K + K, B * mm.gram_spc});
+          last_deferred = true;
+        } else if (mm.fill_slabs) {
+          const WgradDesc gd{xop, xop, B, N, K, K, mm.fill_rows, mm.fill_slabs, prec, 1, 0};
+          static const bool batch_gemm = !(getenv("PN_WGRAD_BATCH") && atoi(getenv("PN_WGRAD_BATCH")) == 0);
+          if (mm.fill_rode) ++g_fill_count[1];
+          else if (batch_gemm) wg_jobs.push_back(gd);
+          else PN_TRY(conv_wgrad(&gd.a, &gd.b, B, N, K, K, gd.slab_rows, gd.slabs, prec, st, 1));
+          jobs.push_back(SlabJob{mm.fill_slabs, mm.gram, (long long)K * K + K, B * mm.fill_spc});
           last_deferred = true;
         } else
         PN_TRY(wgrad_general(xop, xop, B, N, K, K, mm.gram, false, prec, true, true));
@@ -962,7 +1034,8 @@
   }
   bool chain_ok() const { return Bd <= 32; }
   int bwd_chain(const float* dtop, int Ctop, const float* Wtop, const float* a_below_top, float* dWtop, float* dbtop, float* da_top,
-                ChainLayer* ls, int n, float* dx_out, const PrepCarry* carry = nullptr, bool* carried = nullptr, bool top_done = false) {
+                ChainLayer* ls, int n, float* dx_out, const PrepCarry* carry = nullptr, bool* carried = nullptr, bool top_done = false,
+                bool* gram_rode = nullptr) {
     if (dWtop) dense_jobs.push_back(DenseWgradJob{a_below_top, ls[0].r->cout, dtop, Bd, ls[0].r->cout, Ctop, dWtop, dbtop});
     const float* dz_above = dtop;
     int c_above = Ctop;
@@ -979,7 +1052,8 @@
       dz_above = dl.dz; c_above = r.cout; w_above = p(r.kernel); dx_above = dl.din;
     }
     if (carry)
-      return dense_trans_prep_carry(dz_above, c_above, w_above, c_above, Bd, c_above, ls[n - 1].r->cin, w.dense_part, w.dcount, dx_out, carry, st, carried);
+      return dense_trans_prep_carry(dz_above, c_above, w_above, c_above, Bd, c_above, ls[n - 1].r->cin, w.dense_part, w.dcount, dx_out, carry, st, carried,
+                                    gram_rode);
     return dense_trans_tail(dz_above, c_above, w_above, c_above, Bd, c_above, ls[n - 1].r->cin, w.dense_part, w.dcount, dx_out, nullptr, st);
   }
   int bwd_tnet(TN& t, const TRef& r, const pn_operand* x, WgradFuse* wf = nullptr, bool* fused = nullptr) {
@@ -991,8 +1065,11 @@
     if (chain_ok()) {
       ChainLayer ls[2] = {{&t.d2, &r.d2, t.d1.a, 1, nullptr}, {&t.d1, &r.d1, pooled(t.m3), 1, nullptr}};
       const bool pcar = prep_carries(r.c3);
-      const PrepCarry pc = prep_carry(t.c3, t.m3, r.c3, lazy(t.c2), nullptr);
-      PN_TRY(bwd_chain(t.dR, KK, p(r.w), t.d2.a, wg ? gr(r.w) : nullptr, wg ? gr(r.b) : nullptr, t.da2, ls, 2, t.m3.dG, pcar ? &pc : nullptr, &prep_carried));
+      PrepCarry pc = prep_carry(t.c3, t.m3, r.c3, lazy(t.c2), nullptr);
+      WgradDesc gd;
+      pc.gram = gram_fill_take(t.m3, r.c3, lazy(t.c2), gd);
+      PN_TRY(bwd_chain(t.dR, KK, p(r.w), t.d2.a, wg ? gr(r.w) : nullptr, wg ? gr(r.b) : nullptr, t.da2, ls, 2, t.m3.dG, pcar ? &pc : nullptr, &prep_carried,
+                       false, &t.m3.fill_rode));
     } else {
     if (wg) {
       const float *dR = t.dR, *a2 = t.d2.a;
@@ -1096,9 +1173,11 @@
         const bool wg3 = tr(BLK_C3) && G;
         ChainLayer ls[2] = {{&w.c2, &L.c2, w.c1.a, 1, io.keep2}, {&w.c1, &L.c1, pooled(w.mm23), 1, io.keep1}};
         const bool pcar = prep_carries(L.m23);
-        const PrepCarry pc = prep_carry(w.m23, w.mm23, L.m23, lazy(w.m22), have_dGseg ? w.dGseg : nullptr);
+        PrepCarry pc = prep_carry(w.m23, w.mm23, L.m23, lazy(w.m22), have_dGseg ? w.dGseg : nullptr);
+        WgradDesc gd;
+        pc.gram = gram_fill_take(w.mm23, L.m23, lazy(w.m22), gd);
         PN_TRY(bwd_chain(w.cls_dlogits, d.ccls, p(L.c3.kernel), w.c2.a, wg3 ? gr(L.c3.kernel) : nullptr, wg3 ? gr(L.c3.bias) : nullptr,
-                         w.c3.din, ls, 2, w.dGcls, pcar ? &pc : nullptr, &cls_prep_carried, loss_carries() && !d_cls));
+                         w.c3.din, ls, 2, w.dGcls, pcar ? &pc : nullptr, &cls_prep_carried, loss_carries() && !d_cls, &w.mm23.fill_rode));
       } else {
       PN_TRY(bwd_dense(w.c3, L.c3, w.c2.a, w.cls_dlogits, 0, nullptr, w.c3.din));
       PN_TRY(bwd_dense(w.c2, L.c2, w.c1.a, w.c3.din, 1, io.keep2, w.c2.din));
@@ -1304,6 +1383,7 @@
 }
 int64_t pn_model_wgrad_fused_count(void) { return (int64_t)g_wgrad_fused_count.load(); }
 int64_t pn_model_plan_count(int which) { return (which >= 0 && which < 3) ? (int64_t)g_plan_count[which].load() : -1; }
+int64_t pn_model_fill_count(int which) { return (which >= 0 && which < 4) ? (int64_t)g_fill_count[which].load() : -1; }
 int pn_model_forward(const pn_model_desc* d, const pn_model_io* io, pn_stream stream) {
   Run* r = nullptr;
   PN_TRY(make_run(d, io, reinterpret_cast<hipStream_t>(stream), r));
diff --git a/pointcloudprocessing_amd/csrc/pn_segout.hip b/pointcloudprocessing_amd/csrc/pn_segout.hip
--- a/pointcloudprocessing_amd/csrc/pn_segout.hip
+++ b/pointcloudprocessing_amd/csrc/pn_segout.hip
@@ -1,4 +1,5 @@
 #include "pn_common.h"
+#include "pn_dense_body.h"
 #include "pn_loss_bodies.h"
 
 namespace pn {
@@ -300,11 +301,10 @@
 constexpr int sh_lds_bytes(int rows) { return sh_region_a(rows) + sh_region_b(rows) + sh_region_c(rows) + sh_region_d(); }
 static_assert(sh_lds_bytes(128) <= 160 * 1024 && 2 * sh_lds_bytes(64) <= 160 * 1024, "one 128-row workgroup or two 64-row workgroups per CU");
 template <int MB, bool S16, bool DBG = false>
-__global__ __launch_bounds__(256, MB == 2 ? 2 : 1) void seg_head_fused_kernel(const SegHeadArgs a) {
+__device__ __forceinline__ void seg_head_tile_body(const SegHeadArgs& a, const int tile, unsigned char* sh_sm) {
   constexpr int ROWS = 32 * MB, SH_REGION_A = sh_region_a(ROWS), SH_REGION_B = sh_region_b(ROWS), SH_REGION_C = sh_region_c(ROWS);
   unsigned stamp[DBG ? 24 : 1];
   SH_STAMP(0);
-  extern __shared__ __attribute__((aligned(16))) unsigned char sh_sm[];
   __bf16* Ain = reinterpret_cast<__bf16*>(sh_sm);
   __bf16* S1c = Ain + ROWS * SH_P64;
   __bf16* S3 = reinterpret_cast<__bf16*>(sh_sm);
@@ -317,7 +317,7 @@
   float* coef = reinterpret_cast<float*>(sh_sm + SH_REGION_A + SH_REGION_B + SH_REGION_C);
   const int tid = threadIdx.x, lane = tid & 63, wave = tid >> 6;
   const int r = lane & 31, h = lane >> 5;
-  const int cloud = blockIdx.x / a.tiles_per_cloud, tin = blockIdx.x - cloud * a.tiles_per_cloud;
+  const int cloud = tile / a.tiles_per_cloud, tin = tile - cloud * a.tiles_per_cloud;
   const int r0 = tin * ROWS, nrows = min(ROWS, a.N - r0);
   const long long row0 = (long long)cloud * a.N + r0;
 
@@ -607,14 +607,48 @@
     }
   }
 }
+template <int MB, bool S16, bool DBG = false>
+__global__ __launch_bounds__(256, MB == 2 ? 2 : 1) void seg_head_fused_kernel(const SegHeadArgs a) {
+  extern __shared__ __attribute__((aligned(16))) unsigned char sh_sm[];
+  seg_head_tile_body<MB, S16, DBG>(a, (int)blockIdx.x, sh_sm);
+}
+static_assert(DL_LDS_FLOATS * 4 <= sh_lds_bytes(64), "the dense body's LDS fits the front of a tile's region");
+template <int DEPTH, bool S16>
+__global__ __launch_bounds__(256, 2) void seg_fill_kernel(const DenseArgs d, int ncb, int n_dense, const SegHeadArgs a, int tile0) {
+  extern __shared__ __attribute__((aligned(16))) unsigned char sh_sm[];
+  const int lin = (int)blockIdx.x;
+  if (lin < n_dense) {
+    const int ks = lin / ncb, bx = lin - ks * ncb;
+    (void)dense_layer_body<false, DEPTH, true>(d, (unsigned)bx, ks, reinterpret_cast<float*>(sh_sm));
+    return;
+  }
+  seg_head_tile_body<2, S16>(a, tile0 + lin - n_dense, sh_sm);
+}
 #undef SH_STAMP
 #undef SH_KEEP_ABOVE
 #undef SH_BARRIER
 int seg_head_fused_rows() { return SH_ROWS; }
+static int seg_head_force_mb() {
+  static const int v = getenv("PN_SEGHEAD_MB") ? atoi(getenv("PN_SEGHEAD_MB")) : 0;
+  return v;
+}
+static bool seg_head_dbg() {
+  static const bool v = getenv("PN_SEGHEAD_DBG") && atoi(getenv("PN_SEGHEAD_DBG")) == 16;
+  return v;
+}
+bool seg_head_fill_fits(const DenseCall& d) {
+  if (seg_head_force_mb() == 4 || seg_head_dbg()) return false;
+  if (!d.x || !d.w || !d.partial || !d.counters || !d.z_out || d.R <= 0 || d.K <= 0 || d.C <= 0 || cdiv(d.C, DL_COLS) > DENSE_MAX_COUNTERS) return false;
+  if (d.bn_mode && !(d.gamma && d.beta && d.mm && d.mv)) return false;
+  DenseArgs a;
+  int depth = 0;
+  bool vec = false;
+  return dense_call_args(d, a, &depth, &vec) == PN_OK && vec && (depth == 2 || depth == 4);
+}
 int seg_head_fused(const pn_operand* x, const float* gb, const void* w1t, const void* w2t, const void* w3t, const void* w4t, const float* sc1,
                    const float* sh1, const float* sc2, const float* sh2, const float* sc3, const float* sh3, const float* sc4, const float* sh4,
                    const float* w5, const float* b5, int B, int N, int C, int s16, const int* labels, float grad_scale, float* probs,
-                   float* dlogits, float* part, hipStream_t st) {
+                   float* dlogits, float* part, hipStream_t st, const SegFill* fill) {
   PN_CHECK_ARG(x && x->s1 && !x->s2 && gb && w1t && w2t && w3t && w4t && sc1 && sh1 && sc2 && sh2 && sc3 && sh3 && sc4 && sh4 && w5,
                "seg_head_fused: null pointer");
   PN_CHECK_ARG(B > 0 && N > 0 && C >= 1 && C <= SEG_CM, "seg_head_fused: bad sizes (B=%d N=%d C=%d)", B, N, C);
@@ -627,8 +661,32 @@
   a.sc1 = sc1; a.sh1 = sh1; a.sc2 = sc2; a.sh2 = sh2; a.sc3 = sc3; a.sh3 = sh3; a.sc4 = sc4; a.sh4 = sh4;
   a.w5 = w5; a.b5 = b5; a.N = N; a.C = C; a.s16 = s16;
   a.labels = labels; a.grad_scale = grad_scale; a.probs = probs; a.dlogits = dlogits; a.part = part;
-  static const int force_mb = getenv("PN_SEGHEAD_MB") ? atoi(getenv("PN_SEGHEAD_MB")) : 0;
-  static const bool dbg = getenv("PN_SEGHEAD_DBG") && atoi(getenv("PN_SEGHEAD_DBG")) == 16;
+  const int force_mb = seg_head_force_mb();
+  const bool dbg = seg_head_dbg();
+  if (fill) {
+    a.tiles_per_cloud = cdiv(N, 64);
+    PN_CHECK_ARG(seg_head_fill_fits(fill->dense), "seg_head_fused: the dense layer does not fit the carried launch");
+    PN_CHECK_ARG(fill->tile0 >= 0 && fill->ntiles >= 0 && (long long)fill->tile0 + fill->ntiles <= (long long)B * a.tiles_per_cloud,
+                 "seg_head_fused: tiles [%d, %d + %d) of %lld", fill->tile0, fill->tile0, fill->ntiles, (long long)B * a.tiles_per_cloud);
+    DenseArgs da;
+    int depth = 0;
+    bool vec = false;
+    PN_TRY(dense_call_args(fill->dense, da, &depth, &vec));
+    const int ncb = cdiv(da.C, DL_COLS), n_dense = ncb * da.nsplit;
+    const dim3 grid(n_dense + fill->ntiles);
+#define PN_FILL_CASE(D, S)                                                                                                                   \
+  do {                                                                                                                                       \
+    static const hipError_t attr = hipFuncSetAttribute(reinterpret_cast<const void*>(&seg_fill_kernel<D, S>),                               \
+                                                       hipFuncAttributeMaxDynamicSharedMemorySize, sh_lds_bytes(64));                        \
+    PN_CHECK_ARG(attr == hipSuccess, "seg_head_fused: dynamic LDS attribute");                                                               \
+    hipLaunchKernelGGL((seg_fill_kernel<D, S>), grid, dim3(256), sh_lds_bytes(64), st, da, ncb, n_dense, a, fill->tile0);                    \
+  } while (0)
+    if (depth == 2) { if (s16) PN_FILL_CASE(2, true); else PN_FILL_CASE(2, false); }
+    else { if (s16) PN_FILL_CASE(4, true); else PN_FILL_CASE(4, false); }
+#undef PN_FILL_CASE
+    PN_CHECK_LAUNCH();
+    return PN_OK;
+  }
   const bool tall = force_mb == 4;
   if (tall) {
     static const hipError_t attr1 = hipFuncSetAttribute(reinterpret_cast<const void*>(&seg_head_fused_kernel<4, true>), hipFuncAttributeMaxDynamicSharedMemorySize,
```

New measurement: 47.44 million points/s. 0.987x the previous value.
